# wasiahmad/context_attentive_ir

Measured on AMD Instinct MI355X. Metric: ranked (query,doc) pairs/sec, higher is better.
Workload: dtype f32; 1 GPU; cars, batch=16 sessions x session_len 7 x 10 candidates, q_len=4, doc_len=64, emb_dim=300, vocab=100000, f32, full-length Zipf ids; macro_batch=8, lanes=4, batches_in_flight=32, hipgraph=True, parallelism=single GPU, world_size=1

## Files before the change

### context_attentive_ir_amd/csrc/cars_session.hip

```cpp
#include "split2.hpp"
#include <algorithm>
#include <mutex>

namespace nir {

int launch_linear(const float* a, int64_t lda, const int64_t* ids, const float* table, int E, int64_t rows_per_seq,
                  int64_t seq_stride, const float* w, int64_t ldw, const float* bias, const float* bias2, float* c,
                  int64_t ldc, int64_t M, int N, int K, int act, hipStream_t st);
int launch_linear_ex(const float* a, int64_t lda, const int64_t* ids, const float* table, int E, int64_t rows_per_seq,
                     int64_t seq_stride, const float* w, int64_t ldw, const float* bias, const float* bias2, float* c,
                     int64_t ldc, int64_t M, int N, int K, int act, const float* add, int64_t ldadd, hipStream_t st);
constexpr int ACT_MAXOUT2 = 16;
constexpr int ACT_BOUNDED = 0x100;
constexpr int ACT_TANH_ROWDOT16 = 17;


__global__ __launch_bounds__(256) void click_pool2_kernel(const float* __restrict__ docs, const float* __restrict__ epart, int NP,
                                                          const float* __restrict__ b3, const float* __restrict__ labels,
                                                          const float* __restrict__ labels_all, int rows_all,
                                                          const int* __restrict__ mg, int rpg,
                                                          int rows, int N, int D, float* __restrict__ clicks) {
    __shared__ int part[4];
    const int lane = threadIdx.x & 63, wave = threadIdx.x >> 6;
    if (!mg) {
        int best = 0;
        for (int r0 = wave; r0 < rows_all; r0 += 4 * 16) {
            float lv[16];
#pragma unroll
            for (int j = 0; j < 16; ++j) {
                const int r = r0 + 4 * j;
                lv[j] = labels_all[(int64_t)(r < rows_all ? r : 0) * N + (lane < N ? lane : 0)];
            }
#pragma unroll
            for (int j = 0; j < 16; ++j) best = max(best, (int)__popcll(__ballot(lv[j] != 0.f && lane < N && r0 + 4 * j < rows_all)));
        }
        if (lane == 0) part[wave] = best;
    }
    __syncthreads();
    const int r = blockIdx.x * 4 + wave;
    if (r >= rows) return;
    const int m = mg ? mg[r / rpg] : max(max(part[0], part[1]), max(part[2], part[3]));
    const float lab = lane < N ? labels[(int64_t)r * N + lane] : -INFINITY;
    int rank = 0;
#pragma unroll 8
    for (int k = 0; k < N; ++k) {
        const float lk = __uint_as_float(__builtin_amdgcn_readlane(__float_as_uint(lab), k));
        rank += (lk > lab) || (lk == lab && k < lane);
    }
    const int count = (int)wave_sum((lane < N && lab != 0.f) ? 1.f : 0.f);
    const bool keep = lane < N && (rank < count || rank >= m);
    float lg = -INFINITY;
    if (keep) {
        const float* lp = epart + ((int64_t)r * N + lane) * NP;
        float s = b3[0];
        for (int j = 0; j < NP; j += 4) {
            const float4 v = *reinterpret_cast<const float4*>(lp + j);
            s += (v.x + v.y) + (v.z + v.w);
        }
        lg = s;
    }
    const float mx = wave_max(lg);
    const float ex = keep ? expf(lg - mx) : 0.f;
    const float p = ex / wave_sum(ex);
    const int nch = D >> 2;
    for (int c0 = 0; c0 < nch; c0 += 64) {
        const int c = c0 + lane < nch ? c0 + lane : 0;
        float4 acc = make_float4(0.f, 0.f, 0.f, 0.f);
#pragma unroll 8
        for (int k = 0; k < N; ++k) {
            const float pk = __uint_as_float(__builtin_amdgcn_readlane(__float_as_uint(p), k));
            const float4 v = *reinterpret_cast<const float4*>(docs + ((int64_t)r * N + k) * D + 4 * c);
            acc.x = fmaf(pk, v.x, acc.x); acc.y = fmaf(pk, v.y, acc.y); acc.z = fmaf(pk, v.z, acc.z); acc.w = fmaf(pk, v.w, acc.w);
        }
        if (c0 + lane < nch) *reinterpret_cast<float4*>(clicks + (int64_t)r * D + 4 * c) = acc;
    }
}

__global__ __launch_bounds__(256) void click_max_kernel(const float* __restrict__ labels, int rows, int N, int* __restrict__ out) {
    __shared__ int part[4];
    const int lane = threadIdx.x & 63, wave = threadIdx.x >> 6;
    const float* lg = labels + (int64_t)blockIdx.x * rows * N;
    int best = 0;
    if (N <= 64) {
        for (int r0 = 0; r0 < rows; r0 += 256) {
            const int r = r0 + (int)threadIdx.x;
            const float* row = lg + (int64_t)(r < rows ? r : rows - 1) * N;
            int c = 0;
#pragma unroll 8
            for (int k = 0; k < N; ++k) c += row[k] != 0.f ? 1 : 0;
            best = max(best, r < rows ? c : 0);
        }
        best = (int)wave_max((float)best);
    } else {
        for (int r = wave; r < rows; r += 4) {
            float c = 0.f;
            for (int k = lane; k < N; k += 64) c += lg[(int64_t)r * N + k] != 0.f ? 1.f : 0.f;
            best = max(best, (int)wave_sum(c));
        }
    }
    if (lane == 0) part[wave] = best;
    __syncthreads();
    if (threadIdx.x == 0) out[blockIdx.x] = max(max(part[0], part[1]), max(part[2], part[3]));
}

__global__ __launch_bounds__(256) void click_pool_big_kernel(const float* __restrict__ docs, const float* __restrict__ epart, int NP,
                                                             const float* __restrict__ b3, const float* __restrict__ labels,
                                                             const float* __restrict__ labels_all, int rows_all,
                                                             const int* __restrict__ mg, int rpg, int rows, int N, int D,
                                                             float* __restrict__ clicks) {
    extern __shared__ float csm[];
    __shared__ int part[4];
    const int lane = threadIdx.x & 63, wave = threadIdx.x >> 6;
    if (!mg) {
        int best = 0;
        for (int r = wave; r < rows_all; r += 4) {
            float c = 0.f;
            for (int k = lane; k < N; k += 64) c += labels_all[(int64_t)r * N + k] != 0.f ? 1.f : 0.f;
            best = max(best, (int)wave_sum(c));
        }
        if (lane == 0) part[wave] = best;
    }
    __syncthreads();
    const int r = blockIdx.x * 4 + wave;
    if (r >= rows) return;
    const int m = mg ? mg[r / rpg] : max(max(part[0], part[1]), max(part[2], part[3]));
    float* lab = csm + (size_t)wave * 2 * N;
    float* pw = lab + N;
    float cnt = 0.f;
    for (int k = lane; k < N; k += 64) {
        const float v = labels[(int64_t)r * N + k];
        lab[k] = v;
        cnt += v != 0.f ? 1.f : 0.f;
    }
    const int count = (int)wave_sum(cnt);
    __builtin_amdgcn_wave_barrier();
    float mx = -INFINITY;
    for (int c0 = 0; c0 < N; c0 += 64) {
        const int c = c0 + lane;
        const float lc = c < N ? lab[c] : -INFINITY;
        int rank = 0;
        for (int k = 0; k < N; ++k) {
            const float lk = lab[k];
            rank += (lk > lc) || (lk == lc && k < c);
        }
        const bool keep = c < N && (rank < count || rank >= m);
        float lg = -INFINITY;
        if (keep) {
            const float* lp = epart + ((int64_t)r * N + c) * NP;
            float sacc = b3[0];
            for (int j = 0; j < NP; j += 4) {
                const float4 v = *reinterpret_cast<const float4*>(lp + j);
                sacc += (v.x + v.y) + (v.z + v.w);
            }
            lg = sacc;
        }
        if (c < N) pw[c] = lg;
        mx = fmaxf(mx, lg);
    }
    mx = wave_max(mx);
    float den = 0.f;
    for (int c = lane; c < N; c += 64) {
        const float lg = pw[c];
        const float ex = lg == -INFINITY ? 0.f : expf(lg - mx);
        pw[c] = ex;
        den += ex;
    }
    den = wave_sum(den);
    __builtin_amdgcn_wave_barrier();
    const int nch = D >> 2;
    for (int c = lane; c < nch; c += 64) {
        float4 acc = make_float4(0.f, 0.f, 0.f, 0.f);
#pragma unroll 4
        for (int k = 0; k < N; ++k) {
            const float pk = pw[k] / den;
            const float4 v = *reinterpret_cast<const float4*>(docs + ((int64_t)r * N + k) * D + 4 * c);
            acc.x = fmaf(pk, v.x, acc.x); acc.y = fmaf(pk, v.y, acc.y); acc.z = fmaf(pk, v.z, acc.z); acc.w = fmaf(pk, v.w, acc.w);
        }
        *reinterpret_cast<float4*>(clicks + (int64_t)r * D + 4 * c) = acc;
    }
}


template <int NB, int UG = 1>
__global__ __launch_bounds__(256) void lstm_step_kernel(LstmStepArgs p) {
    __shared__ float red[4][UG * NB][256];
    const int tid = threadIdx.x, lane = tid & 63, wave = tid >> 6;
    const int i = lane & 15, g = lane >> 4;
    const int ch = blockIdx.y + p.chain0;
    const int u0 = blockIdx.x * 4 * UG;
    const int I = p.I, H = p.H;
    const float* wi[UG];
    const float* wh[UG];
#pragma unroll
    for (int ug = 0; ug < UG; ++ug) {
        const int ua = u0 + 4 * ug + (i >> 2);
        const int arow = (i & 3) * H + (ua < H ? ua : H - 1);
        wi[ug] = p.wih[ch] + (int64_t)arow * I;
        wh[ug] = p.whh[ch] + (int64_t)arow * H;
    }
    const float* hprev = p.hprev[ch];
    const float* cprev = p.cprev[ch];
    const float* gxp = p.gx[ch];
    const int nq1 = gxp ? 0 : ((I + 15) >> 4), nq2 = hprev ? ((H + 15) >> 4) : 0;
    float bias[UG][4];
#pragma unroll
    for (int ug = 0; ug < UG; ++ug) {
        const int ud = u0 + 4 * ug + g;
#pragma unroll
        for (int r = 0; r < 4; ++r) bias[ug][r] = (ud < H && !gxp) ? p.bih[ch][r * H + ud] + p.bhh[ch][r * H + ud] : 0.f;
    }
    for (int b0 = blockIdx.z * 16 * NB; b0 < p.B; b0 += gridDim.z * 16 * NB) {
        const float* xr[NB];
        const float* hr[NB];
        float bm[NB];
#pragma unroll
        for (int t = 0; t < NB; ++t) {
            const int b = b0 + 16 * t + i;
            const bool bv = b < p.B;
            bm[t] = bv ? 1.f : 0.f;
            const int bc = bv ? b : p.B - 1;
            const int64_t xr_i = p.xid[ch] ? p.xid[ch][bc] : (int64_t)bc;
            xr[t] = p.x[ch] + xr_i * p.xstride[ch];
            hr[t] = hprev ? hprev + (int64_t)bc * H : nullptr;
        }
        f32x4 acc[UG][NB];
#pragma unroll
        for (int ug = 0; ug < UG; ++ug)
#pragma unroll
            for (int t = 0; t < NB; ++t) acc[ug][t] = (f32x4){0.f, 0.f, 0.f, 0.f};
        constexpr int CH = NB == 1 ? 12 : (NB == 2 ? 8 : (UG == 1 ? 6 : 4));
        const int nqt = nq1 + nq2;
        for (int q0 = wave; q0 < nqt; q0 += 4 * CH) {
            float4 a4[CH][UG], b4[CH][NB];
#pragma unroll
            for (int c = 0; c < CH; ++c) {
                const int q = q0 + 4 * c;
                const bool second = q >= nq1;
                const int K = second ? H : I;
                const int k = 16 * (second ? q - nq1 : q) + 4 * g;
                const float km = (q < nqt && k < K) ? 1.f : 0.f;
                const int kc = (q < nqt && k < K) ? k : 0;
#pragma unroll
                for (int ug = 0; ug < UG; ++ug) {
                    a4[c][ug] = *reinterpret_cast<const float4*>((second ? wh[ug] : wi[ug]) + kc);
                    a4[c][ug].x *= km; a4[c][ug].y *= km; a4[c][ug].z *= km; a4[c][ug].w *= km;
                }
#pragma unroll
                for (int t = 0; t < NB; ++t) {
                    b4[c][t] = *reinterpret_cast<const float4*>(((second && hr[t]) ? hr[t] : xr[t]) + kc);
                    b4[c][t].x *= bm[t]; b4[c][t].y *= bm[t]; b4[c][t].z *= bm[t]; b4[c][t].w *= bm[t];
                }
            }
            __builtin_amdgcn_sched_barrier(0);
#pragma unroll
            for (int c = 0; c < CH; ++c)
#pragma unroll
                for (int ug = 0; ug < UG; ++ug)
#pragma unroll
                    for (int t = 0; t < NB; ++t) {
                        acc[ug][t] = __builtin_amdgcn_mfma_f32_16x16x4f32(a4[c][ug].x, b4[c][t].x, acc[ug][t], 0, 0, 0);
                        acc[ug][t] = __builtin_amdgcn_mfma_f32_16x16x4f32(a4[c][ug].y, b4[c][t].y, acc[ug][t], 0, 0, 0);
// ... 232 lines not shown
                                                              const float* __restrict__ Ds, const float* __restrict__ q,
                                                              int B, int S, int D, int HS, int q_on, int d_on,
                                                              float* __restrict__ xcat) {
    extern __shared__ float lgs[];
    float* lg[2] = {lgs, lgs + S};
    const int bt = blockIdx.x, b = bt / S, t = bt % S;
    const int lane = threadIdx.x & 63, wave = threadIdx.x >> 6;
    const int nch = q_on + d_on;
    const int HSQ = q_on ? HS : 0;
    const float* ur = U + (int64_t)bt * NU;
    const float* qv = q + (int64_t)bt * D;
    float* orow = xcat + (int64_t)bt * (D + nch * HS);
    for (int e = wave; e < nch * t; e += 4) {
        const int c = e / t, k = e % t + 1;
        const float* st = (c == 0 && q_on) ? Qs : Ds;
        const float* sv = st + ((int64_t)k * B + b) * HS;
        const float* uv = ur + c * HS;
        float sacc = 0.f;
        for (int f = 4 * lane; f < HS; f += 256) {
            const float4 a = *reinterpret_cast<const float4*>(sv + f), w = *reinterpret_cast<const float4*>(uv + f);
            sacc += (a.x * w.x + a.y * w.y) + (a.z * w.z + a.w * w.w);
        }
        sacc = wave_sum(sacc);
        if (lane == 0) lg[c][k] = sacc + ur[nch * HS + c];
    }
    if (threadIdx.x < nch) lg[threadIdx.x][0] = ur[nch * HS + threadIdx.x];
    for (int f = threadIdx.x; f < D; f += 256) orow[f] = qv[f];
    __syncthreads();
    for (int c = 0; c < nch; ++c) {
        const float* st = (c == 0 && q_on) ? Qs : Ds;
        float mx = -INFINITY;
        for (int k = 0; k <= t; ++k) mx = fmaxf(mx, lg[c][k]);
        float den = 0.f;
        for (int k = 0; k <= t; ++k) den += expf(lg[c][k] - mx);
        for (int f = threadIdx.x; f < HS; f += 256) {
            float acc = 0.f;
            for (int k = 1; k <= t; ++k) acc = fmaf(expf(lg[c][k] - mx) / den, st[((int64_t)k * B + b) * HS + f], acc);
            orow[D + c * HS + f] = acc;
        }
    }
    (void)HSQ;
}

__global__ void session_pack_kernel(const float* wq, const float* wshared, const float* wpriv, const float* sqw, const float* sqb,
                                    const float* sdw, const float* sdb, int D, int HS, int q_on, int d_on, float* wrank, float* ut) {
    const int nch = q_on + d_on, KS = nch * HS, KR = D + KS;
    const int64_t i = (int64_t)blockIdx.x * blockDim.x + threadIdx.x;
    if (i < (int64_t)D * KR) {
        const int o = (int)(i / KR), k = (int)(i % KR);
        float v;
        if (k < D) v = wq[(int64_t)o * D + k];
        else v = wshared[(int64_t)o * KS + (k - D)] + wpriv[(int64_t)o * KS + (k - D)];
        wrank[i] = v;
    }
    if (i < (int64_t)(KS + nch) * D) {
        const int j = (int)(i / D), f = (int)(i % D);
        float v;
        if (j < KS) {
            const int c = j / HS, jj = j % HS;
            const float* w = (c == 0 && q_on) ? sqw : sdw;
            v = w[(int64_t)f * HS + jj];
        } else {
            const int c = j - KS;
            v = ((c == 0 && q_on) ? sqb : sdb)[f];
        }
        ut[i] = v;
    }
}

__global__ void rank_feats_kernel(const float* qp, const float* docs, int N, int D, int64_t rows, float* feats) {
    const int64_t i = ((int64_t)blockIdx.x * blockDim.x + threadIdx.x) * 4;
    if (i < rows * D) {
        const int64_t r = i / D;
        const int f = (int)(i % D);
        const float4 q = *reinterpret_cast<const float4*>(qp + (r / N) * D + f), d = *reinterpret_cast<const float4*>(docs + r * D + f);
        float* o = feats + r * 4 * D + f;
        *reinterpret_cast<float4*>(o) = q;
        *reinterpret_cast<float4*>(o + D) = d;
        *reinterpret_cast<float4*>(o + 2 * D) = make_float4(fabsf(q.x - d.x), fabsf(q.y - d.y), fabsf(q.z - d.z), fabsf(q.w - d.w));
        *reinterpret_cast<float4*>(o + 3 * D) = make_float4(q.x * d.x, q.y * d.y, q.z * d.z, q.w * d.w);
    }
}

__global__ __launch_bounds__(256) void session_inner_pool_kernel(const float* __restrict__ states, const float* __restrict__ lpart,
                                                                 int NP, const float* __restrict__ b3, int B, int S, int HS,
                                                                 float* __restrict__ out ) {
    extern __shared__ float lg[];
    const int bt = blockIdx.x, b = bt / S, t = bt % S;
    const int n = t + 1;
    for (int k = threadIdx.x; k < n; k += 256) {
        const float* lp = lpart + ((int64_t)k * B + b) * NP;
        float s = b3[0];
        for (int j = 0; j < NP; ++j) s += lp[j];
        lg[k] = s;
    }
    __syncthreads();
    float mx = -INFINITY;
    for (int k = 0; k < n; ++k) mx = fmaxf(mx, lg[k]);
    float den = 0.f;
    for (int k = 0; k < n; ++k) den += expf(lg[k] - mx);
    for (int f = threadIdx.x; f < HS; f += 256) {
        float acc = 0.f;
        for (int k = 0; k < n; ++k) acc = fmaf(expf(lg[k] - mx) / den, states[((int64_t)k * B + b) * HS + f], acc);
        out[(int64_t)bt * HS + f] = acc;
    }
}

__global__ void session_cat_states_kernel(const float* a, const float* b2, int rows, int HSa, int HSb, float* out) {
    const int64_t i = (int64_t)blockIdx.x * blockDim.x + threadIdx.x;
    const int W = HSa + HSb;
    if (i < (int64_t)rows * W) {
        const int r = (int)(i / W), f = (int)(i % W);
        out[i] = f < HSa ? a[(int64_t)r * HSa + f] : b2[(int64_t)r * HSb + (f - HSa)];
    }
}

struct SessPlan {
    float *epart, *clicks, *Qs, *Ds, *Cq, *Cd, *U, *xcat, *qp, *feats, *y0, *y1, *lin, *cat, *gx, *Qs16, *Ds16;
    size_t bytes;
};
static SessPlan sess_plan(void* ws, size_t cap, int B, int S, int N, int D, int HS, int nch, bool rank_on, bool want_states) {
    Workspace a(ws, cap);
    SessPlan p;
    const size_t R = (size_t)B * S * N, BS = (size_t)B * S;
    p.epart = a.take<float>(R * (D / 16));
    p.clicks = a.take<float>(BS * D);
    p.Qs = a.take<float>((size_t)(S + 1) * B * HS);
    p.Ds = a.take<float>((size_t)(S + 1) * B * HS);
    p.Cq = a.take<float>((size_t)(S + 1) * B * HS);
    p.Cd = a.take<float>((size_t)(S + 1) * B * HS);
    p.U = a.take<float>(BS * (size_t)(nch * HS + nch + 4));
    p.xcat = a.take<float>(BS * (size_t)(D + nch * HS));
    p.qp = a.take<float>(BS * D);
    p.feats = a.take<float>(rank_on ? R * 4 * D : 0);
    p.y0 = a.take<float>(rank_on ? R * 256 : 0);
    p.y1 = a.take<float>(rank_on ? R * 128 : 0);
    p.lin = a.take<float>(want_states ? (size_t)(S + 1) * B * (HS / 16) : 0);
    p.cat = a.take<float>(want_states ? (size_t)S * B * nch * HS : 0);
    p.gx = a.take<float>((size_t)nch * BS * 4 * HS);
    p.Qs16 = a.take<float>((size_t)(S + 1) * B * HS);
    p.Ds16 = a.take<float>((size_t)(S + 1) * B * HS);
    p.bytes = align_up(a.off, 256);
    return p;
}

}

extern "C" size_t nir_lstm_step_whh_frag_bytes(int H) { return (H > 0 && H % 32 == 0) ? (size_t)4 * H * H * 2 * sizeof(_Float16) : 0; }

extern "C" int nir_lstm_step_pack_whh_frag(const float* w_hh, int H, void* frag, int* err_flag, nir_stream_t stream) {
    using namespace nir;
    NIR_REQUIRE(w_hh && frag && H > 0 && H % 32 == 0, "lstm_step_pack_whh_frag: H must be a positive multiple of 32");
    hipLaunchKernelGGL(lstm_step_whh_frag_kernel, dim3((unsigned)(H / 4), (unsigned)(H / 32)), dim3(64), 0, (hipStream_t)stream, w_hh, H, (_Float16*)frag, err_flag);
    NIR_CHECK_LAUNCH("lstm_step_whh_frag_kernel");
    return 0;
}

extern "C" size_t nir_cars_session_pack_floats(const nir_cars_session_weights* w, size_t* wrank_floats, size_t* ut_floats) {
    if (!w) return 0;
    const int nch = (w->q_on ? 1 : 0) + (w->d_on ? 1 : 0);
    const size_t a = (size_t)w->D * (w->D + nch * w->HS), b = (size_t)(nch * w->HS + nch) * w->D;
    if (wrank_floats) *wrank_floats = a;
    if (ut_floats) *ut_floats = b;
    return a + b;
}

extern "C" int nir_cars_session_pack(const nir_cars_session_weights* w, float* wrank, float* ut, nir_stream_t stream) {
    using namespace nir;
    NIR_REQUIRE(w && wrank && ut, "cars_session_pack: null pointer");
    const int q_on = w->q_on ? 1 : 0, d_on = w->d_on ? 1 : 0, nch = q_on + d_on;
    NIR_REQUIRE(w->qproj_w, "cars_session_pack: q_projection missing (ranker off?)");
    NIR_REQUIRE(nch == 0 || (w->shared_w && w->priv1_w), "cars_session_pack: session projectors missing");
    const int64_t n = std::max((int64_t)w->D * (w->D + nch * w->HS), (int64_t)(nch * w->HS + nch) * w->D);
    hipLaunchKernelGGL(session_pack_kernel, g1(n), dim3(256), 0, (hipStream_t)stream, w->qproj_w, w->shared_w, w->priv1_w, w->sq_attn_w,
                       w->sq_attn_b, w->sd_attn_w, w->sd_attn_b, w->D, w->HS, q_on, d_on, wrank, ut);
    NIR_CHECK_LAUNCH("session_pack_kernel");
    return 0;
}

extern "C" size_t nir_cars_session_workspace_bytes(int B, int S, int N, const nir_cars_session_weights* w) {
    if (!w || B < 0 || S <= 0 || N <= 0) return 0;
    const int nch = (w->q_on ? 1 : 0) + (w->d_on ? 1 : 0);
    return nir::sess_plan(nullptr, 0, B, S, N, w->D, w->HS, nch, true, true).bytes;
}

extern "C" int nir_cars_rank_session(const float* pooled_q, const float* pooled_docs, const float* labels, int B, int S, int N,
                                     const nir_cars_session_weights* w, void* workspace, size_t workspace_bytes,
                                     float* click_scores, float* clicks_out, const nir_cars_session_outputs* extra,
                                     nir_stream_t stream) {
    return nir_cars_rank_session_rows(pooled_q, pooled_docs, labels, B, S, N, w, workspace, workspace_bytes, click_scores, clicks_out, extra,
                                      nullptr, 0, nullptr, 0, nullptr, 0, stream);
}

extern "C" int nir_cars_rank_session_shard(const float* pooled_q, const float* pooled_docs, const float* labels, int B, int S, int N,
                                           const nir_cars_session_weights* w, void* workspace, size_t workspace_bytes,
                                           float* click_scores, float* clicks_out, const nir_cars_session_outputs* extra,
                                           const float* rank_docs, int NR, nir_stream_t stream) {
    return nir_cars_rank_session_rows(pooled_q, pooled_docs, labels, B, S, N, w, workspace, workspace_bytes, click_scores, clicks_out, extra,
                                      rank_docs, NR, nullptr, 0, nullptr, 0, stream);
}

extern "C" int nir_cars_click_max(const float* labels, int groups, int rows, int N, int* m_out, nir_stream_t stream) {
    using namespace nir;
    NIR_REQUIRE(labels && m_out && groups > 0 && rows > 0 && N > 0, "cars_click_max: bad args");
    hipLaunchKernelGGL(click_max_kernel, dim3((unsigned)groups), dim3(256), 0, (hipStream_t)stream, labels, rows, N, m_out);
    NIR_CHECK_LAUNCH("click_max_kernel");
    return 0;
}

extern "C" int nir_cars_rank_session_rows(const float* pooled_q, const float* pooled_docs, const float* labels, int B, int S, int N,
                                          const nir_cars_session_weights* w, void* workspace, size_t workspace_bytes,
                                          float* click_scores, float* clicks_out, const nir_cars_session_outputs* extra,
                                          const float* rank_docs, int NR, const float* labels_all, int64_t rows_all, const int* m_groups,
                                          int sessions_per_group, nir_stream_t stream) {
    return nir_cars_rank_session_pre(pooled_q, pooled_docs, labels, B, S, N, w, workspace, workspace_bytes, click_scores, clicks_out, extra, rank_docs, NR,
                                     labels_all, rows_all, m_groups, sessions_per_group, nullptr, nullptr, stream);
}

extern "C" int nir_cars_session_query_side(const float* pooled_q, int B, int S, const nir_cars_session_weights* w, float* U, float* gq,
                                           nir_stream_t stream) {
    using namespace nir;
    hipStream_t st = (hipStream_t)stream;
    NIR_REQUIRE(pooled_q && w && B >= 0 && S > 0, "cars_session_query_side: bad arguments");
    if (B == 0) return 0;
    const bool q_on = w->q_on != 0, d_on = w->d_on != 0, rank_on = w->rank_on != 0;
    const int nch = (q_on ? 1 : 0) + (d_on ? 1 : 0), D = w->D, HS = w->HS, NU = nch * HS + nch;
    const int64_t BS = (int64_t)B * S;
    const int bnd = (w->rank_bounded & 8) ? ACT_BOUNDED : 0;
    NIR_REQUIRE(!(nch && rank_on) || (U && w->attn_ut), "cars_session_query_side: U / packed attention weights missing");
    NIR_REQUIRE(!(nch && q_on) || gq, "cars_session_query_side: gq missing");
    if (nch && rank_on)
        NIR_PROPAGATE(launch_linear(pooled_q, D, nullptr, nullptr, 0, 0, 0, w->attn_ut, D, nullptr, nullptr, U, NU, BS, NU, D, NIR_ACT_NONE, st));
    if (nch && q_on)
        NIR_PROPAGATE(launch_linear_ex(pooled_q, D, nullptr, nullptr, 0, 0, 0, w->sq_wih, D, w->sq_bih, w->sq_bhh, gq, 4 * HS, BS, 4 * HS, D, NIR_ACT_NONE | bnd, nullptr, 0, st));
    return 0;
}

extern "C" int nir_cars_rank_session_pre(const float* pooled_q, const float* pooled_docs, const float* labels, int B, int S, int N,
                                         const nir_cars_session_weights* w, void* workspace, size_t workspace_bytes,
                                         float* click_scores, float* clicks_out, const nir_cars_session_outputs* extra,
                                         const float* rank_docs, int NR, const float* labels_all, int64_t rows_all, const int* m_groups,
                                         int sessions_per_group, const float* pre_U, const float* pre_gq, nir_stream_t stream) {
    using namespace nir;
    hipStream_t st = (hipStream_t)stream;
    NIR_REQUIRE(pooled_q && w, "cars_rank_session: null pointer");
    const bool q_on = w->q_on != 0, d_on = w->d_on != 0, rank_on = w->rank_on != 0;
    const int nch = (q_on ? 1 : 0) + (d_on ? 1 : 0);
    NIR_REQUIRE(!rank_on || (pooled_docs && click_scores && w->wrank), "cars_rank_session: ranker on needs documents, scores and packed weights");
    NIR_REQUIRE(!d_on || (pooled_docs && labels), "cars_rank_session: the document session needs documents and labels");
    NIR_REQUIRE(nch == 0 || !rank_on || w->attn_ut, "cars_rank_session: packed attention weights missing (nir_cars_session_pack)");
    NIR_REQUIRE(B >= 0 && S > 0 && N > 0, "cars_rank_session: bad dims");
    NIR_REQUIRE(N <= 2048, "cars_rank_session: %d candidates > 2048 unsupported", N);
    NIR_REQUIRE(!labels_all || (rows_all >= (int64_t)B * S && rows_all < (1 << 30)), "cars_rank_session: labels_all must hold at least the B*S rows of this call");
    NIR_REQUIRE(!rank_docs || (NR > 0 && NR <= N), "cars_rank_session: the ranked candidate slice must hold 1..N candidates (got %d)", NR);
    NIR_REQUIRE(S <= 4096, "cars_rank_session: session length %d > 4096 unsupported", S);
    NIR_REQUIRE(!m_groups || (sessions_per_group > 0 && !labels_all), "cars_rank_session: m_groups needs sessions_per_group > 0 and excludes labels_all");
    NIR_REQUIRE(!m_groups || B % sessions_per_group == 0, "cars_rank_session: B = %d is not a whole number of blocks of %d sessions", B, sessions_per_group);
    NIR_REQUIRE(!extra || nch > 0, "cars_rank_session: decoder states need at least one session encoder");
    NIR_REQUIRE(w->D % 64 == 0 && w->HS % 16 == 0 && w->D % 16 == 0, "cars_rank_session: D %% 64 / HS %% 16 required");
    if (B == 0) return 0;
    const int D = w->D, HS = w->HS, NP = D / 16;
    const bool want_states = extra != nullptr;
    SessPlan p = sess_plan(workspace, workspace_bytes, B, S, N, D, HS, nch, rank_on, want_states);
    if (!workspace || p.bytes > workspace_bytes) {
        set_error("cars_rank_session: workspace too small (%zu < %zu)", workspace_bytes, p.bytes);
        return NIR_ERR_WORKSPACE;
    }
    const int64_t BS = (int64_t)B * S, R = BS * N;
    float* clicks = clicks_out ? clicks_out : p.clicks;
    const int NU = nch * HS + nch;
    const float* gq = (pre_gq && q_on) ? pre_gq : p.gx;
    float* gd = p.gx + (q_on ? BS * 4 * (int64_t)HS : 0);
    const float* Uq = (pre_U && nch && rank_on) ? pre_U : p.U;
    const int bnd = (w->rank_bounded & 8) ? ACT_BOUNDED : 0;
    {
        hipStream_t sq_ = st;
        if (nch && rank_on && Uq == p.U)
            NIR_PROPAGATE(launch_linear(pooled_q, D, nullptr, nullptr, 0, 0, 0, w->attn_ut, D, nullptr, nullptr, p.U, NU, BS, NU, D, NIR_ACT_NONE, sq_));
        if (nch && q_on && gq == p.gx) NIR_PROPAGATE(launch_linear_ex(pooled_q, D, nullptr, nullptr, 0, 0, 0, w->sq_wih, D, w->sq_bih, w->sq_bhh, p.gx, 4 * HS, BS, 4 * HS, D, NIR_ACT_NONE | bnd, nullptr, 0, sq_));
    }
    if (d_on) {
        NIR_PROPAGATE(launch_linear_ex(pooled_docs, D, nullptr, nullptr, 0, 0, 0, w->click0_w, D, w->click0_b, nullptr, p.epart, NP, R, D, D,
                                       ACT_TANH_ROWDOT16 | ((w->rank_bounded & 4) ? ACT_BOUNDED : 0), w->click3_w, 0, st));
        {
            ProfScope ps("click_pool2_kernel", st);
            const float* lall = labels_all ? labels_all : labels;
            const int rall = labels_all ? (int)rows_all : (int)BS;
            if (N <= 64)
                hipLaunchKernelGGL(click_pool2_kernel, dim3((unsigned)((BS + 3) / 4)), dim3(256), 0, st, pooled_docs, p.epart, NP, w->click3_b, labels,
                                   lall, rall, m_groups, sessions_per_group * S, (int)BS, N, D, clicks);
            else {
                static std::once_flag once;
                std::call_once(once, [] { (void)hipFuncSetAttribute((const void*)click_pool_big_kernel, hipFuncAttributeMaxDynamicSharedMemorySize, 4 * 2 * 2048 * (int)sizeof(float)); });
                hipLaunchKernelGGL(click_pool_big_kernel, dim3((unsigned)((BS + 3) / 4)), dim3(256), (size_t)4 * 2 * N * sizeof(float), st, pooled_docs,
                                   p.epart, NP, w->click3_b, labels, lall, rall, m_groups, sessions_per_group * S, (int)BS, N, D, clicks);
            }
        }
        NIR_CHECK_LAUNCH("click_pool2_kernel");
    }
    const int nsteps = want_states ? S : S - 1;
    if (nch) {
        LstmStepArgs a;
        a.wih[0] = w->sq_wih; a.whh[0] = w->sq_whh; a.bih[0] = w->sq_bih; a.bhh[0] = w->sq_bhh;
        a.wih[1] = w->sd_wih; a.whh[1] = w->sd_whh; a.bih[1] = w->sd_bih; a.bhh[1] = w->sd_bhh;
        a.xid[0] = a.xid[1] = nullptr;
        a.xstride[0] = a.xstride[1] = (int64_t)S * D;
        a.chain0 = q_on ? 0 : 1;
        a.B = B; a.I = D; a.H = HS;
        {
            if (d_on) NIR_PROPAGATE(launch_linear_ex(clicks, D, nullptr, nullptr, 0, 0, 0, w->sd_wih, D, w->sd_bih, w->sd_bhh, gd, 4 * HS, BS, 4 * HS, D, NIR_ACT_NONE | bnd, nullptr, 0, st));
            a.gx[0] = gq; a.gx[1] = gd;
            a.gxstride = (int64_t)S * 4 * HS;
            a.whh_frag[0] = w->sq_whh_frag; a.whh_frag[1] = w->sd_whh_frag;
        }
        const float* gx0[2] = {a.gx[0], a.gx[1]};
        const int64_t slot = (int64_t)B * HS;
        for (int t = 0; t < nsteps; ++t) {
            a.gx[0] = gx0[0] + (int64_t)t * 4 * HS; a.gx[1] = gx0[1] + (int64_t)t * 4 * HS;
            a.x[0] = pooled_q + (int64_t)t * D; a.x[1] = clicks + (int64_t)t * D;
            a.hprev[0] = t ? p.Qs + t * slot : nullptr; a.cprev[0] = t ? p.Cq + t * slot : nullptr;
            a.hprev[1] = t ? p.Ds + t * slot : nullptr; a.cprev[1] = t ? p.Cd + t * slot : nullptr;
            a.hnext[0] = p.Qs + (t + 1) * slot; a.cnext[0] = p.Cq + (t + 1) * slot;
            a.hnext[1] = p.Ds + (t + 1) * slot; a.cnext[1] = p.Cd + (t + 1) * slot;
            a.h16prev[0] = t ? reinterpret_cast<const _Float16*>(p.Qs16 + t * slot) : nullptr;
            a.h16prev[1] = t ? reinterpret_cast<const _Float16*>(p.Ds16 + t * slot) : nullptr;
            a.h16next[0] = reinterpret_cast<_Float16*>(p.Qs16 + (t + 1) * slot);
            a.h16next[1] = reinterpret_cast<_Float16*>(p.Ds16 + (t + 1) * slot);
            NIR_PROPAGATE(launch_lstm_step(a, nch, st));
        }
    }
    if (rank_on) {
        const int KR = D + nch * HS;
        const float* xrows = pooled_q;
        if (nch) {
            {
                ProfScope ps("session_attend2_kernel", st);
                hipLaunchKernelGGL(session_attend2_kernel, dim3((unsigned)BS), dim3(256), 2 * S * sizeof(float), st, Uq, NU, p.Qs, p.Ds, pooled_q, B, S, D, HS,
                                   (int)q_on, (int)d_on, p.xcat);
            }
            NIR_CHECK_LAUNCH("session_attend2_kernel");
            xrows = p.xcat;
        }
        NIR_PROPAGATE(launch_linear(xrows, KR, nullptr, nullptr, 0, 0, 0, w->wrank, KR, w->qproj_b, nullptr, p.qp, D, BS, D, KR, NIR_ACT_NONE, st));
        const float* rdocs = rank_docs ? rank_docs : pooled_docs;
        const int Nr = rank_docs ? NR : N;
        const int64_t Rr = BS * Nr;
        {
            ProfScope ps("rank_feats_kernel", st);
            hipLaunchKernelGGL(rank_feats_kernel, g1(Rr * D / 4), dim3(256), 0, st, p.qp, rdocs, Nr, D, Rr, p.feats);
        }
        NIR_CHECK_LAUNCH("rank_feats_kernel");
        NIR_PROPAGATE(launch_linear_ex(p.feats, 4 * D, nullptr, nullptr, 0, 0, 0, w->mo0_w, 4 * D, w->mo0_b, nullptr, p.y0, 256, Rr, 512, 4 * D,
                                       ACT_MAXOUT2 | ((w->rank_bounded & 1) ? ACT_BOUNDED : 0), nullptr, 0, st));
        NIR_PROPAGATE(launch_linear_ex(p.y0, 256, nullptr, nullptr, 0, 0, 0, w->mo1_w, 256, w->mo1_b, nullptr, p.y1, 128, Rr, 256, 256,
                                       ACT_MAXOUT2 | ((w->rank_bounded & 2) ? ACT_BOUNDED : 0), nullptr, 0, st));
        NIR_PROPAGATE(launch_linear_ex(p.y1, 128, nullptr, nullptr, 0, 0, 0, w->mo2_w, 128, w->mo2_b, nullptr, click_scores, 1, Rr, 2, 128, ACT_MAXOUT2, nullptr, 0, st));
    }
    if (want_states) {
        const float* st_a = q_on ? p.Qs : p.Ds;
        const float* st_b = (q_on && d_on) ? p.Ds : nullptr;
        const float* c_a = q_on ? p.Cq : p.Cd;
        const float* c_b = (q_on && d_on) ? p.Cd : nullptr;
        const int HSb = st_b ? HS : 0, W = HS + HSb;
        const int rows = (S - 1) * B;
        if (extra->inner_q && q_on) {
            NIR_PROPAGATE(launch_linear_ex(p.Qs + (int64_t)B * HS, HS, nullptr, nullptr, 0, 0, 0, w->sq_inner0_w, HS, w->sq_inner0_b, nullptr, p.lin, HS / 16,
                                           (int64_t)S * B, HS, HS, ACT_TANH_ROWDOT16, w->sq_inner3_w, 0, st));
            hipLaunchKernelGGL(session_inner_pool_kernel, dim3((unsigned)BS), dim3(256), S * sizeof(float), st, p.Qs + (int64_t)B * HS, p.lin, HS / 16, w->sq_inner3_b, B, S, HS, extra->inner_q);
        }
        if (extra->inner_d && d_on) {
            NIR_PROPAGATE(launch_linear_ex(p.Ds + (int64_t)B * HS, HS, nullptr, nullptr, 0, 0, 0, w->sd_inner0_w, HS, w->sd_inner0_b, nullptr, p.lin, HS / 16,
                                           (int64_t)S * B, HS, HS, ACT_TANH_ROWDOT16, w->sd_inner3_w, 0, st));
            hipLaunchKernelGGL(session_inner_pool_kernel, dim3((unsigned)BS), dim3(256), S * sizeof(float), st, p.Ds + (int64_t)B * HS, p.lin, HS / 16, w->sd_inner3_b, B, S, HS, extra->inner_d);
        }
        NIR_CHECK_LAUNCH("session_inner_pool_kernel");
        if (rows > 0 && extra->dec_h && w->th_w) {
            hipLaunchKernelGGL(session_cat_states_kernel, g1((int64_t)rows * W), dim3(256), 0, st, st_a + (int64_t)B * HS,
                               st_b ? st_b + (int64_t)B * HS : nullptr, rows, HS, HSb, p.cat);
            NIR_PROPAGATE(launch_linear(p.cat, W, nullptr, nullptr, 0, 0, 0, w->th_w, W, w->th_b, nullptr, extra->dec_h, w->HDEC, rows, w->HDEC, W, NIR_ACT_NONE, st));
        }
        if (rows > 0 && extra->dec_c && w->tc_w) {
            hipLaunchKernelGGL(session_cat_states_kernel, g1((int64_t)rows * W), dim3(256), 0, st, c_a + (int64_t)B * HS,
                               c_b ? c_b + (int64_t)B * HS : nullptr, rows, HS, HSb, p.cat);
            NIR_PROPAGATE(launch_linear(p.cat, W, nullptr, nullptr, 0, 0, 0, w->tc_w, W, w->tc_b, nullptr, extra->dec_c, w->HDEC, rows, w->HDEC, W, NIR_ACT_NONE, st));
        }
        NIR_CHECK_LAUNCH("session_cat_states_kernel");
    }
    return 0;
}
```

### context_attentive_ir_amd/csrc/gemm.hip

```cpp
#include "split2.hpp"
#include <algorithm>
#include <mutex>
#include <stdlib.h>

namespace nir {


struct GemmArgs {
    const float* a;
    int64_t lda;
    const int64_t* ids;
    const float* table;
    int E;
    int64_t rows_per_seq, seq_stride;
    const float* w;
    int64_t ldw;
    const float* bias;
    const float* bias2;
    float* c;
    int64_t ldc;
    int64_t M;
    int N, K, act;
    const float* add;
    int64_t ldadd;
};

constexpr int ACT_MAXOUT2 = 16;
constexpr int ACT_TANH_ROWDOT16 = 17;
constexpr int ACT_BOUNDED = 0x100;

__device__ __forceinline__ void gemm_store(const GemmArgs& p, int64_t m, int n, float v, float bsum) {
    v += bsum;
    if (p.act == ACT_TANH_ROWDOT16) {
        v = n < p.N ? fast_tanh(v) * p.add[n] : 0.f;
        v += dpp_mov<0xB1>(v);
        v += dpp_mov<0x4E>(v);
        v += dpp_mov<0x141>(v);
        v += dpp_mov<0x140>(v);
        if (m < p.M && n < p.N && !(n & 15)) p.c[m * p.ldc + (n >> 4)] = v;
        return;
    }
    if (p.add && m < p.M && n < p.N) v += p.add[m * p.ldadd + n];
    if (p.act == NIR_ACT_TANH) v = fast_tanh(v);
    else if (p.act == NIR_ACT_RELU) v = fmaxf(v, 0.f);
    if (p.act == ACT_MAXOUT2) {
        const float other = dpp_mov<0xB1>(v);
        v = fmaxf(v, other);
        if (m < p.M && n < p.N && !(n & 1)) p.c[m * p.ldc + (n >> 1)] = v;
    } else if (m < p.M && n < p.N) {
        p.c[m * p.ldc + n] = v;
    }
}

#ifndef NIR_GEMM_BK
#define NIR_GEMM_BK 32
#endif
constexpr int BM = 64, BN = 64, BK = NIR_GEMM_BK, LDS_LD = BK + 4;
constexpr int TPR = BK / 4, RPP = 256 / TPR;
constexpr int LPT = BM * BK / 4 / 256;

template <bool VEC>
__global__ __launch_bounds__(256) void gemm_kernel(GemmArgs p) {
    extern __shared__ __attribute__((aligned(16))) float smem[];
    float* As = smem;
    float* Ws = smem + 2 * BM * LDS_LD;
    const int tid = threadIdx.x, lane = tid & 63, wave = tid >> 6;
    const int wm = wave >> 1, wn = wave & 1;
    const int nb = (p.N + BN - 1) / BN;
    const int64_t mb = (p.M + BM - 1) / BM;
    const int64_t bid = blockIdx.x;
    const int64_t tq = bid >> 3;
    const int64_t mblk = (tq / nb) * 8 + (bid & 7);
    if (mblk >= mb) return;
    const int64_t m0 = mblk * BM;
    const int n0 = (int)(tq % nb) * BN;
    const int lr = tid / TPR, lk = (tid % TPR) * 4;

    const float* arow[LPT];
    int64_t aidx[LPT];
    bool aval[LPT];
    const float* wrow[LPT];
    bool wval[LPT];
    const bool taps3 = p.ids && p.K > p.E && p.K <= 3 * p.E;
    const float* arow1[LPT];
    const float* arow2[LPT];
#pragma unroll
    for (int i = 0; i < LPT; ++i) {
        int64_t m = m0 + lr + RPP * i;
        aval[i] = m < p.M;
        arow[i] = arow1[i] = arow2[i] = nullptr;
        aidx[i] = 0;
        if (aval[i]) {
            if (p.ids) {
                aidx[i] = (m / p.rows_per_seq) * p.seq_stride + (m % p.rows_per_seq);
                if (p.K <= p.E) arow[i] = p.table + p.ids[aidx[i]] * (int64_t)p.E;
                if (taps3) {
                    arow[i] = p.table + p.ids[aidx[i]] * (int64_t)p.E;
                    arow1[i] = p.table + p.ids[aidx[i] + 1] * (int64_t)p.E - p.E;
                    arow2[i] = p.K > 2 * p.E ? p.table + p.ids[aidx[i] + 2] * (int64_t)p.E - 2 * p.E : arow1[i];
                }
            } else {
                arow[i] = p.a + m * p.lda;
            }
        }
        int n = n0 + lr + RPP * i;
        wval[i] = n < p.N;
        wrow[i] = p.w + (int64_t)(wval[i] ? n : 0) * p.ldw;
    }

    float4 ra[LPT], rw[LPT];
    auto load_tile = [&](int k0) {
        const int k = k0 + lk;
#pragma unroll
        for (int i = 0; i < LPT; ++i) {
            ra[i] = make_float4(0.f, 0.f, 0.f, 0.f);
            rw[i] = make_float4(0.f, 0.f, 0.f, 0.f);
            if (VEC) {
                if (k < p.K) {
                    if (aval[i]) {
                        const float* src;
                        if (taps3) {
                            src = (k < p.E ? arow[i] : (k < 2 * p.E ? arow1[i] : arow2[i])) + k;
                        } else if (p.ids && p.K > p.E) {
                            int seg = k / p.E;
                            src = p.table + p.ids[aidx[i] + seg] * (int64_t)p.E + (k - seg * p.E);
                        } else {
                            src = arow[i] + k;
                        }
                        ra[i] = *reinterpret_cast<const float4*>(src);
                    }
                    if (wval[i]) rw[i] = *reinterpret_cast<const float4*>(wrow[i] + k);
                }
            } else {
                float ta[4] = {0.f, 0.f, 0.f, 0.f}, tw[4] = {0.f, 0.f, 0.f, 0.f};
// ... 546 lines not shown
            G3_TERM(2, 0) G3_TERM(1, 1) G3_TERM(0, 2) G3_TERM(1, 0) G3_TERM(0, 1) G3_TERM(0, 0)
#undef G3_TERM
        }
      }
    };
#ifdef NIR_G3_NOLOAD
#define G3_LOAD(...)
#else
#define G3_LOAD(...) load_tile(__VA_ARGS__)
#endif
#ifdef NIR_G3_NOMMA
#define G3_MMA(b)
#else
#define G3_MMA(b) mma_tile(b)
#endif
#ifdef NIR_G3_NOSTORE
#define G3_STORE(...)
#else
#define G3_STORE(...) store_tile(__VA_ARGS__)
#endif
    int kt = 0;
    for (; kt + 4 < nk; kt += 2) {
        G3_LOAD(R0, (kt + 2) * KSTEP, false);
        __builtin_amdgcn_sched_barrier(0);
        G3_MMA(0);
        __builtin_amdgcn_sched_barrier(0);
        G3_STORE(R1, 1);
        lds_barrier();
        G3_LOAD(R1, (kt + 3) * KSTEP, false);
        __builtin_amdgcn_sched_barrier(0);
        G3_MMA(1);
        __builtin_amdgcn_sched_barrier(0);
        G3_STORE(R0, 0);
        lds_barrier();
    }
#undef G3_LOAD
#undef G3_MMA
#undef G3_STORE
    for (; kt < nk; ++kt) {
        const bool odd = (kt & 1) != 0;
        if (kt + 2 < nk) {
            if (odd) load_tile(R1, (kt + 2) * KSTEP, (kt + 2 == nk - 1) && ktail);
            else load_tile(R0, (kt + 2) * KSTEP, (kt + 2 == nk - 1) && ktail);
        }
        __builtin_amdgcn_sched_barrier(0);
        mma_tile(kt & 1);
        __builtin_amdgcn_sched_barrier(0);
        if (kt + 1 < nk) {
            if (odd) store_tile(R0, 0);
            else store_tile(R1, 1);
            lds_barrier();
        }
    }
#pragma unroll
    for (int b = 0; b < 2; ++b) {
        const int n = n0 + wn * 64 + b * 32 + (lane & 31);
        float bsum = 0.f;
        if (n < p.N) {
            if (p.bias) bsum += p.bias[n];
            if (p.bias2) bsum += p.bias2[n];
        }
#pragma unroll
        for (int a = 0; a < 2; ++a)
#pragma unroll
            for (int r = 0; r < 16; ++r) {
                const int64_t m = m0 + wm * 64 + a * 32 + (r & 3) + 8 * (r >> 2) + 4 * (lane >> 5);
                float v = acc[a][b][r];
                if (H2) v = split2_combine(v, acx[a][b][r]);
                gemm_store(p, m, n, v, bsum);
            }
    }
}

struct GemmPlaneArgs {
    const _Float16 *a1, *a2;
    int64_t lda;
    const int64_t* ids;
    int64_t rows_per_seq, seq_stride;
    int EP, taps;
    const _Float16 *w1, *w2;
    int64_t ldw;
    GemmArgs ep;
    int K;
};
constexpr int GP_BK = 32;
constexpr int GP_CHUNK = 128 * 8 + 32;
constexpr int GP_PLANE = 4 * GP_CHUNK;

template <int MODE>
__global__ __launch_bounds__(256, 2) void gemm_h2p_kernel(GemmPlaneArgs q) {
    extern __shared__ __attribute__((aligned(16))) unsigned short smemp[];
    unsigned short* As = smemp;
    unsigned short* Ws = smemp + 2 * 2 * GP_PLANE;
    const GemmArgs& p = q.ep;
    const int tid = threadIdx.x, lane = tid & 63, wave = tid >> 6;
    const int wm = wave >> 1, wn = wave & 1;
    const int nb = (p.N + G3_BN - 1) / G3_BN;
    const int64_t mb = (p.M + G3_BM - 1) / G3_BM;
    const int64_t bid = blockIdx.x;
    const int64_t tq = bid >> 3;
    const int64_t mblk = (tq / nb) * 8 + (bid & 7);
    if (mblk >= mb) return;
    const int64_t m0 = mblk * G3_BM;
    const int n0 = (int)(tq % nb) * G3_BN;
    const int lr = tid >> 1, hs = tid & 1;

    int64_t m = m0 + lr;
    m = m < p.M ? m : p.M - 1;
    int64_t arow[3] = {0, 0, 0};
    if (MODE == 0) {
        arow[0] = m * q.lda;
    } else {
        const int64_t ai = (m / q.rows_per_seq) * q.seq_stride + (m % q.rows_per_seq);
#pragma unroll
        for (int t = 0; t < 3; ++t) arow[t] = (t < q.taps ? q.ids[ai + t] : q.ids[ai]) * q.lda - (int64_t)t * q.EP;
    }
    int n = n0 + lr;
    n = n < p.N ? n : p.N - 1;
    const int64_t wrow = (int64_t)n * q.ldw;

    uint4 ra[2][2], rw[2][2];
    auto load_tile = [&](int k0, bool tail) {
        int k = k0 + 16 * hs;
        bool kv = true, kv2 = true;
        if (tail) {
            kv = k < q.K;
            k = kv ? k : 0;
            kv2 = kv && k + 8 < q.K;
        }
        int64_t ao = arow[0];
        if (MODE == 2) ao = k < q.EP ? arow[0] : (k < 2 * q.EP ? arow[1] : arow[2]);
        const int k2 = kv2 ? k + 8 : k;
        int64_t ao2 = ao;
        if (MODE == 2) ao2 = k2 < q.EP ? arow[0] : (k2 < 2 * q.EP ? arow[1] : arow[2]);
        ra[0][0] = *reinterpret_cast<const uint4*>(q.a1 + ao + k);
        ra[1][0] = *reinterpret_cast<const uint4*>(q.a2 + ao + k);
        ra[0][1] = *reinterpret_cast<const uint4*>(q.a1 + ao2 + k2);
        ra[1][1] = *reinterpret_cast<const uint4*>(q.a2 + ao2 + k2);
        rw[0][0] = *reinterpret_cast<const uint4*>(q.w1 + wrow + k);
        rw[1][0] = *reinterpret_cast<const uint4*>(q.w2 + wrow + k);
        rw[0][1] = *reinterpret_cast<const uint4*>(q.w1 + wrow + k2);
        rw[1][1] = *reinterpret_cast<const uint4*>(q.w2 + wrow + k2);
        if (tail) {
            const uint4 z = make_uint4(0u, 0u, 0u, 0u);
            if (!kv) { ra[0][0] = z; ra[1][0] = z; rw[0][0] = z; rw[1][0] = z; }
            if (!kv2) { ra[0][1] = z; ra[1][1] = z; rw[0][1] = z; rw[1][1] = z; }
        }
    };
    auto store_tile = [&](int buf) {
#pragma unroll
        for (int t = 0; t < 2; ++t)
#pragma unroll
            for (int c = 0; c < 2; ++c) {
                const int off = (buf * 2 + t) * GP_PLANE + (hs * 2 + c) * GP_CHUNK + lr * 8;
                *reinterpret_cast<uint4*>(As + off) = ra[t][c];
                *reinterpret_cast<uint4*>(Ws + off) = rw[t][c];
            }
    };
    f32x16 acc[2][2], acx[2][2];
#pragma unroll
    for (int a = 0; a < 2; ++a)
#pragma unroll
        for (int b = 0; b < 2; ++b)
#pragma unroll
            for (int r = 0; r < 16; ++r) { acc[a][b][r] = 0.0f; acx[a][b][r] = 0.0f; }

    const int nk = (q.K + GP_BK - 1) / GP_BK;
    const bool ktail = (q.K % GP_BK) != 0;
    if (nk == 1 && ktail) load_tile(0, true);
    else load_tile(0, false);
    store_tile(0);
    __syncthreads();
    const int foff_a = (lane >> 5) * GP_CHUNK + (wm * 64 + (lane & 31)) * 8;
    const int foff_w = (lane >> 5) * GP_CHUNK + (wn * 64 + (lane & 31)) * 8;
    auto mma_tile = [&](int buf) {
#pragma unroll
        for (int kb = 0; kb < 2; ++kb) {
            const unsigned short* ab = As + buf * 2 * GP_PLANE + kb * 2 * GP_CHUNK + foff_a;
            const unsigned short* wb = Ws + buf * 2 * GP_PLANE + kb * 2 * GP_CHUNK + foff_w;
            f16x8 af[2][2], wf[2][2];
#pragma unroll
            for (int t = 0; t < 2; ++t)
#pragma unroll
                for (int i = 0; i < 2; ++i) {
                    af[i][t] = *reinterpret_cast<const f16x8*>(ab + t * GP_PLANE + i * 32 * 8);
                    wf[i][t] = *reinterpret_cast<const f16x8*>(wb + t * GP_PLANE + i * 32 * 8);
                }
#define GP_T(ACC, TA, TW)                                                                                        \
            ACC[0][0] = __builtin_amdgcn_mfma_f32_32x32x16_f16(af[0][TA], wf[0][TW], ACC[0][0], 0, 0, 0);        \
            ACC[0][1] = __builtin_amdgcn_mfma_f32_32x32x16_f16(af[0][TA], wf[1][TW], ACC[0][1], 0, 0, 0);        \
            ACC[1][0] = __builtin_amdgcn_mfma_f32_32x32x16_f16(af[1][TA], wf[0][TW], ACC[1][0], 0, 0, 0);        \
            ACC[1][1] = __builtin_amdgcn_mfma_f32_32x32x16_f16(af[1][TA], wf[1][TW], ACC[1][1], 0, 0, 0);
            GP_T(acx, 1, 0) GP_T(acx, 0, 1) GP_T(acc, 0, 0)
#undef GP_T
        }
    };
    for (int kt = 0; kt + 2 < nk; ++kt) {
        load_tile((kt + 1) * GP_BK, false);
        __builtin_amdgcn_sched_barrier(0);
        mma_tile(kt & 1);
        __builtin_amdgcn_sched_barrier(0);
        store_tile((kt & 1) ^ 1);
        __syncthreads();
    }
    if (nk >= 2) {
        const int kt = nk - 2;
        if (ktail) load_tile((kt + 1) * GP_BK, true);
        else load_tile((kt + 1) * GP_BK, false);
        __builtin_amdgcn_sched_barrier(0);
        mma_tile(kt & 1);
        __builtin_amdgcn_sched_barrier(0);
        store_tile((kt & 1) ^ 1);
        __syncthreads();
    }
    mma_tile((nk - 1) & 1);
#pragma unroll
    for (int b = 0; b < 2; ++b) {
        const int nn = n0 + wn * 64 + b * 32 + (lane & 31);
        float bsum = 0.f;
        if (nn < p.N) {
            if (p.bias) bsum += p.bias[nn];
            if (p.bias2) bsum += p.bias2[nn];
        }
#pragma unroll
        for (int a = 0; a < 2; ++a)
#pragma unroll
            for (int r = 0; r < 16; ++r) {
                const int64_t mm = m0 + wm * 64 + a * 32 + (r & 3) + 8 * (r >> 2) + 4 * (lane >> 5);
                gemm_store(p, mm, nn, split2_combine(acc[a][b][r], acx[a][b][r]), bsum);
            }
    }
}

__global__ void split_f16x2_kernel(const float* __restrict__ x, int64_t rows, int cols, int64_t ld, int cols_pad, _Float16* __restrict__ p1,
                                   _Float16* __restrict__ p2) {
    const int64_t i = (int64_t)blockIdx.x * blockDim.x + threadIdx.x;
    if (i >= rows * cols_pad) return;
    const int64_t r = i / cols_pad;
    const int c = (int)(i % cols_pad);
    const float v = c < cols ? x[r * ld + c] : 0.f;
    const _Float16 a = split2_hi1_rtz(v);
    p1[i] = a;
    p2[i] = split2_lo1(v, a);
}

int launch_split_f16x2(const float* x, int64_t rows, int cols, int64_t ld, int cols_pad, void* p1, void* p2, hipStream_t st) {
    NIR_REQUIRE(x && p1 && p2 && rows >= 0 && cols > 0 && cols_pad >= cols && cols_pad % 8 == 0, "split_f16x2: bad args (cols_pad %% 8 == 0)");
    if (rows == 0) return 0;
    const int64_t n = rows * cols_pad;
    hipLaunchKernelGGL(split_f16x2_kernel, dim3((unsigned)((n + 255) / 256)), dim3(256), 0, st, x, rows, cols, ld, cols_pad, (_Float16*)p1, (_Float16*)p2);
    NIR_CHECK_LAUNCH("split_f16x2_kernel");
    return 0;
}

int launch_linear_planes(const void* a1, const void* a2, int64_t lda, const int64_t* ids, int64_t rows_per_seq, int64_t seq_stride, int EP,
                         int taps, const void* w1, const void* w2, int64_t ldw, const float* bias, float* c, int64_t ldc, int64_t M, int N, int K,
                         int act, const float* add, int64_t ldadd, hipStream_t st) {
    NIR_REQUIRE(a1 && a2 && w1 && w2 && c && M >= 0 && N > 0 && K > 0, "linear_planes: bad args");
    NIR_REQUIRE(K % 8 == 0 && lda % 8 == 0 && ldw % 8 == 0, "linear_planes: K and the row strides must be multiples of 8");
    NIR_REQUIRE(!ids || (taps >= 1 && taps <= 3 && EP % 8 == 0 && K == taps * EP), "linear_planes: gathered A needs K == taps*EP, EP %% 8 == 0");
    if (M == 0) return 0;
    GemmPlaneArgs q;
    q.a1 = (const _Float16*)a1; q.a2 = (const _Float16*)a2; q.lda = lda; q.ids = ids; q.rows_per_seq = rows_per_seq; q.seq_stride = seq_stride;
    q.EP = EP; q.taps = taps; q.w1 = (const _Float16*)w1; q.w2 = (const _Float16*)w2; q.ldw = ldw; q.K = K;
    q.ep = GemmArgs{nullptr, 0, nullptr, nullptr, 0, 0, 0, nullptr, 0, bias, nullptr, c, ldc, M, N, K, act, add, ldadd};
    const int64_t mb3 = (M + G3_BM - 1) / G3_BM;
    const int nb3 = (N + G3_BN - 1) / G3_BN;
    constexpr size_t lds = (size_t)2 * 2 * 2 * GP_PLANE * 2;
    static std::once_flag once;
    std::call_once(once, [] {
        (void)hipFuncSetAttribute((const void*)gemm_h2p_kernel<0>, hipFuncAttributeMaxDynamicSharedMemorySize, (int)lds);
        (void)hipFuncSetAttribute((const void*)gemm_h2p_kernel<2>, hipFuncAttributeMaxDynamicSharedMemorySize, (int)lds);
    });
    ProfScope ps(prof_shape_name(ids ? "gemm_h2p_kernel[gather]" : "gemm_h2p_kernel", M, N, K), st);
    dim3 grid((unsigned)(8 * nb3 * ((mb3 + 7) / 8)));
    if (ids) hipLaunchKernelGGL(gemm_h2p_kernel<2>, grid, dim3(256), lds, st, q);
    else hipLaunchKernelGGL(gemm_h2p_kernel<0>, grid, dim3(256), lds, st, q);
    NIR_CHECK_LAUNCH("gemm_h2p_kernel");
    return 0;
}

template <int NT>
static void launch_skinny(const GemmArgs& p, int G, size_t lds, hipStream_t st) {
    static std::once_flag once;
    std::call_once(once, [] { (void)hipFuncSetAttribute((const void*)gemm_skinny_kernel<NT>, hipFuncAttributeMaxDynamicSharedMemorySize, 128 * 1024); });
    const int64_t ntiles = (p.M + 15) / 16;
    const unsigned grid = (unsigned)std::min<int64_t>((ntiles + SK_WAVES - 1) / SK_WAVES, 512);
    hipLaunchKernelGGL(gemm_skinny_kernel<NT>, dim3(grid), dim3(64 * SK_WAVES), lds, st, p, G);
}

__global__ __launch_bounds__(256) void rowdot_kernel(const float* x, int64_t ldx, const float* w, const float* b,
                                                     float* out, int64_t M, int K, int act) {
    const int lane = threadIdx.x & 63;
    const int64_t m = (int64_t)blockIdx.x * 4 + (threadIdx.x >> 6);
    if (m >= M) return;
    const float* xr = x + m * ldx;
    float s = 0.f;
    for (int k = lane; k < K; k += 64) s += xr[k] * w[k];
    s = wave_sum(s);
    if (lane == 0) {
        float v = s + (b ? b[0] : 0.f);
        if (act == NIR_ACT_TANH) v = fast_tanh(v);
        else if (act == NIR_ACT_RELU) v = fmaxf(v, 0.f);
        out[m] = v;
    }
}

int launch_linear_ex(const float* a, int64_t lda, const int64_t* ids, const float* table, int E, int64_t rows_per_seq,
                     int64_t seq_stride, const float* w, int64_t ldw, const float* bias, const float* bias2, float* c,
                     int64_t ldc, int64_t M, int N, int K, int act, const float* add, int64_t ldadd, hipStream_t st) {
    const bool bounded = (act & ACT_BOUNDED) != 0;
    act &= ~ACT_BOUNDED;
    NIR_REQUIRE(M >= 0 && N > 0 && K > 0, "linear: bad dims M=%lld N=%d K=%d", (long long)M, N, K);
    NIR_REQUIRE(w && c, "linear: null weight/output");
    NIR_REQUIRE(ids ? (table != nullptr && E > 0 && rows_per_seq > 0) : (a != nullptr), "linear: null A operand");
    if (M == 0) return 0;
    NIR_REQUIRE(act != ACT_MAXOUT2 || (N % 2 == 0), "linear: maxout epilogue needs an even N");
    NIR_REQUIRE(act != ACT_TANH_ROWDOT16 || (N % 16 == 0 && add != nullptr), "linear: tanh-rowdot epilogue needs N %% 16 == 0 and the weight row");
    GemmArgs p{a, lda, ids, table, E, rows_per_seq, seq_stride, w, ldw, bias, bias2, c, ldc, M, N, K, act, add, ldadd};
    bool vec = (K % 4 == 0) && (ldw % 4 == 0) && (((uintptr_t)w & 15) == 0);
    if (ids) vec = vec && (E % 4 == 0) && (((uintptr_t)table & 15) == 0);
    else vec = vec && (lda % 4 == 0) && (((uintptr_t)a & 15) == 0);
    const int64_t mb = (M + BM - 1) / BM;
    const int nb = (N + BN - 1) / BN;
    const int skG = (K + 15) / 16, skNT = (N + 15) / 16;
    const size_t sk_lds = (size_t)16 * skNT * (skG * 16 + 4) * 4;
    const bool exact_f32 = tun(g_tun.exact_f32) != 0;
    const int64_t mb3 = (M + G3_BM - 1) / G3_BM;
    const int nb3 = (N + G3_BN - 1) / G3_BN;
    const int mode3 = !ids ? 0 : (K <= E ? 1 : (K <= 3 * E ? 2 : -1));
    if (vec && !exact_f32 && mode3 >= 0 && N >= 96 && K >= 32 && mb3 * nb3 >= 96) {
        ProfScope ps(prof_shape_name(bounded ? (ids ? "gemm3h_kernel[gather]" : "gemm3h_kernel") : (ids ? "gemm3_kernel[gather]" : "gemm3_kernel"), M, N, K), st);
        dim3 grid((unsigned)(8 * nb3 * ((mb3 + 7) / 8)));
        if (bounded && K >= 64) {
            constexpr size_t lds2 = (size_t)2 * 2 * 2 * 2 * G3_PLANE * 2;
            static std::once_flag once;
            std::call_once(once, [] {
                (void)hipFuncSetAttribute((const void*)gemm3_kernel<0, true, 2>, hipFuncAttributeMaxDynamicSharedMemorySize, (int)lds2);
                (void)hipFuncSetAttribute((const void*)gemm3_kernel<1, true, 2>, hipFuncAttributeMaxDynamicSharedMemorySize, (int)lds2);
            });
            if (mode3 == 0) { hipLaunchKernelGGL((gemm3_kernel<0, true, 2>), grid, dim3(256), lds2, st, p); NIR_CHECK_LAUNCH("gemm3h ks2"); return 0; }
            if (mode3 == 1) { hipLaunchKernelGGL((gemm3_kernel<1, true, 2>), grid, dim3(256), lds2, st, p); NIR_CHECK_LAUNCH("gemm3h ks2"); return 0; }
        }
        if (bounded) {
            constexpr size_t lds = (size_t)2 * 2 * 2 * G3_PLANE * 2;
            if (mode3 == 0) hipLaunchKernelGGL((gemm3_kernel<0, true>), grid, dim3(256), lds, st, p);
            else if (mode3 == 1) hipLaunchKernelGGL((gemm3_kernel<1, true>), grid, dim3(256), lds, st, p);
            else hipLaunchKernelGGL((gemm3_kernel<2, true>), grid, dim3(256), lds, st, p);
        } else {
            constexpr size_t lds = (size_t)2 * 2 * 3 * G3_PLANE * 2;
            if (mode3 == 0) hipLaunchKernelGGL((gemm3_kernel<0, false>), grid, dim3(256), lds, st, p);
            else if (mode3 == 1) hipLaunchKernelGGL((gemm3_kernel<1, false>), grid, dim3(256), lds, st, p);
            else hipLaunchKernelGGL((gemm3_kernel<2, false>), grid, dim3(256), lds, st, p);
        }
        NIR_CHECK_LAUNCH("nir_linear_f32[bf16x3]");
        return 0;
    }
    if (N <= 64 && vec && M >= 4096 && (!ids || K <= E) && sk_lds <= 128 * 1024 && act != ACT_MAXOUT2 && act != ACT_TANH_ROWDOT16) {
        ProfScope ps(prof_shape_name(ids ? "gemm_skinny_kernel[gather]" : "gemm_skinny_kernel", M, N, K), st);
        if (skNT == 1) launch_skinny<1>(p, skG, sk_lds, st);
// ... 18 lines not shown
        }
        const dim3 grid((unsigned)((M + 16 * best - 1) / (16 * best)), (unsigned)ncol);
        switch (best) {
            case 2: hipLaunchKernelGGL(gemm32_kernel<2>, grid, dim3(256), 0, st, p); break;
            case 3: hipLaunchKernelGGL(gemm32_kernel<3>, grid, dim3(256), 0, st, p); break;
            case 4: hipLaunchKernelGGL(gemm32_kernel<4>, grid, dim3(256), 0, st, p); break;
            case 5: hipLaunchKernelGGL(gemm32_kernel<5>, grid, dim3(256), 0, st, p); break;
            default: hipLaunchKernelGGL(gemm32_kernel<6>, grid, dim3(256), 0, st, p); break;
        }
    } else if (mb * nb < 160) {
        ProfScope ps(prof_shape_name(ids ? "gemm16_kernel[gather]" : "gemm16_kernel", M, N, K), st);
        dim3 grid((unsigned)((M + 15) / 16), (unsigned)((N + 15) / 16));
        if (vec) hipLaunchKernelGGL(gemm16_kernel<true>, grid, dim3(256), 0, st, p);
        else hipLaunchKernelGGL(gemm16_kernel<false>, grid, dim3(256), 0, st, p);
    } else {
        ProfScope ps(prof_shape_name(ids ? "gemm_kernel[gather]" : "gemm_kernel", M, N, K), st);
        constexpr size_t lds = (size_t)2 * (BM + BN) * LDS_LD * 4;
        static std::once_flag once;
        std::call_once(once, [] {
            (void)hipFuncSetAttribute((const void*)gemm_kernel<true>, hipFuncAttributeMaxDynamicSharedMemorySize, (int)lds);
            (void)hipFuncSetAttribute((const void*)gemm_kernel<false>, hipFuncAttributeMaxDynamicSharedMemorySize, (int)lds);
        });
        dim3 grid((unsigned)(8 * nb * ((mb + 7) / 8)));
        if (vec) hipLaunchKernelGGL(gemm_kernel<true>, grid, dim3(256), lds, st, p);
        else hipLaunchKernelGGL(gemm_kernel<false>, grid, dim3(256), lds, st, p);
    }
    NIR_CHECK_LAUNCH("nir_linear_f32");
    return 0;
}

int launch_linear(const float* a, int64_t lda, const int64_t* ids, const float* table, int E, int64_t rows_per_seq,
                  int64_t seq_stride, const float* w, int64_t ldw, const float* bias, const float* bias2, float* c,
                  int64_t ldc, int64_t M, int N, int K, int act, hipStream_t st) {
    return launch_linear_ex(a, lda, ids, table, E, rows_per_seq, seq_stride, w, ldw, bias, bias2, c, ldc, M, N, K, act,
                            nullptr, 0, st);
}

int launch_rowdot(const float* x, int64_t ldx, const float* w, const float* b, float* out, int64_t M, int K, int act,
                  hipStream_t st) {
    NIR_REQUIRE(x && w && out && K > 0, "rowdot: bad args");
    if (M == 0) return 0;
    {
        ProfScope ps("rowdot_kernel", st);
        hipLaunchKernelGGL(rowdot_kernel, dim3((unsigned)((M + 3) / 4)), dim3(256), 0, st, x, ldx, w, b, out, M, K, act);
    }
    NIR_CHECK_LAUNCH("nir_rowdot_f32");
    return 0;
}

}

extern "C" int nir_linear_f32(const float* a, int64_t lda, const int64_t* ids, const float* table, int E,
                              int64_t rows_per_seq, int64_t seq_stride, const float* w, int64_t ldw,
                              const float* bias, const float* bias2, float* c, int64_t ldc, int64_t M, int N, int K,
                              int act, nir_stream_t stream) {
    return nir::launch_linear(a, lda, ids, table, E, rows_per_seq, seq_stride, w, ldw, bias, bias2, c, ldc, M, N, K,
                              act, (hipStream_t)stream);
}

extern "C" int nir_linear_ex_f32(const float* a, int64_t lda, const int64_t* ids, const float* table, int E,
                                 int64_t rows_per_seq, int64_t seq_stride, const float* w, int64_t ldw,
                                 const float* bias, const float* bias2, float* c, int64_t ldc, int64_t M, int N, int K,
                                 int act, const float* add, int64_t ldadd, nir_stream_t stream) {
    return nir::launch_linear_ex(a, lda, ids, table, E, rows_per_seq, seq_stride, w, ldw, bias, bias2, c, ldc, M, N, K,
                                 act, add, ldadd, (hipStream_t)stream);
}

extern "C" int nir_rowdot_f32(const float* x, int64_t ldx, const float* w, const float* b, float* out, int64_t M,
                              int K, int act, nir_stream_t stream) {
    return nir::launch_rowdot(x, ldx, w, b, out, M, K, act, (hipStream_t)stream);
}

namespace nir { int launch_split_f16x2(const float* x, int64_t rows, int cols, int64_t ld, int cols_pad, void* p1, void* p2, hipStream_t st); }
extern "C" int nir_split_f16x2(const float* x, int64_t rows, int cols, int64_t ld, int cols_pad, void* p1, void* p2, nir_stream_t stream) {
    return nir::launch_split_f16x2(x, rows, cols, ld, cols_pad, p1, p2, (hipStream_t)stream);
}

extern "C" int nir_linear_planes_f32(const void* a1, const void* a2, int64_t lda, const int64_t* ids, int64_t rows_per_seq, int64_t seq_stride,
                                     int EP, int taps, const void* w1, const void* w2, int64_t ldw, const float* bias, float* c, int64_t ldc,
                                     int64_t M, int N, int K, int act, nir_stream_t stream) {
    return nir::launch_linear_planes(a1, a2, lda, ids, rows_per_seq, seq_stride, EP, taps, w1, w2, ldw, bias, c, ldc, M, N, K, act, nullptr, 0,
                                     (hipStream_t)stream);
}
```

### context_attentive_ir_amd/lib.py

```python
import ctypes as C
import os

import torch

_HERE = os.path.dirname(os.path.abspath(__file__))
LIB_PATH = os.path.join(_HERE, "libneuroir_hip.so")

c_fp = C.c_void_p
c_ip = C.c_void_p
c_st = C.c_void_p


def _struct(name, float_fields, int_fields=()):
    fields = [(f, c_fp) for f in float_fields] + [(f, C.c_int) for f in int_fields]
    return type(name, (C.Structure,), {"_fields_": fields})


DrmmWeights = _struct("nir_drmm_weights",
                      ["gate_w", "gate_b", "ffnn0_w", "ffnn0_b", "ffnn1_w", "ffnn1_b", "out_w", "out_b"], ["snap_one"])
DrmmWeights = type("nir_drmm_weights", (C.Structure,), {"_fields_": list(DrmmWeights._fields_) + [("self_bin", C.c_void_p)]})
MatchTensorWeights = _struct(
    "nir_matchtensor_weights",
    ["proj_w", "proj_b", "q_wih", "q_whh", "q_bih", "q_bhh", "d_wih", "d_whh", "d_bih", "d_bhh",
     "qproj_w", "qproj_b", "dproj_w", "dproj_b", "alpha", "conv1_w", "conv1_b", "conv2_w", "conv2_b",
     "conv3_w", "conv3_b", "conv_w", "conv_b", "out_w", "out_b"],
    ["F", "Hq", "Hd", "C", "NF", "MF", "bounded"])
MatchTensorWeights = type("nir_matchtensor_weights", (C.Structure,), {"_fields_": list(MatchTensorWeights._fields_) + [("dproj_frag", C.c_void_p)]})
DuetWeights = _struct(
    "nir_duet_weights",
    ["l_conv_w", "l_conv_b", "l_fc1_w", "l_fc1_b", "l_fc2_w", "l_fc2_b", "l_fc3_w", "l_fc3_b",
     "convq_w", "convq_b", "convd1_w", "convd1_b", "convd2_w", "convd2_b", "fc1_w", "fc1_b", "fc2_w", "fc2_b",
     "fc3_w", "fc3_b", "fc4_w", "fc4_b"],
    ["NF", "pool", "bounded"])
DuetWeights = type("nir_duet_weights", (C.Structure,), {"_fields_": list(DuetWeights._fields_) + [
    (f, C.c_void_p) for f in ("table_h1", "table_h2", "convd1_h1", "convd1_h2", "convd2_h1", "convd2_h2")] + [("EP", C.c_int)] + [
    ("fw1", C.c_void_p), ("fw2", C.c_void_p), ("K1P", C.c_int), ("ftable", C.c_void_p), ("fw1c", C.c_void_p), ("EPT", C.c_int)]})
DssmWeights = _struct("nir_dssm_weights", ["q_w1t", "q_b1", "q_w2t", "q_b2", "d_w1t", "d_b1", "d_w2t", "d_b2"], ["NH", "NO"])
CdssmWeights = _struct("nir_cdssm_weights", ["q_w5t", "q_b", "q_semt", "q_semb", "d_w5t", "d_b", "d_semt", "d_semb"], ["NH", "NO"])
CONV1D_SPLIT, CONV1D_FP32, ARCI_MAX_LAYERS = 0, 1, 8


class Conv1dLayer(C.Structure):
    _fields_ = [("planes", C.c_void_p), ("wt", c_fp), ("bias", c_fp)] + [(f, C.c_int) for f in ("C_in", "F", "k", "p", "path")]


class ArciWeights(C.Structure):
    _fields_ = [("q", Conv1dLayer * ARCI_MAX_LAYERS), ("d", Conv1dLayer * ARCI_MAX_LAYERS), ("head_wq", c_fp), ("head_wd", c_fp), ("head_b", c_fp),
                ("n_layers", C.c_int), ("q_feats", C.c_int), ("d_feats", C.c_int)]


ARCII_MAX_LAYERS = 8


class Conv2dLayer(C.Structure):
    _fields_ = [("planes", C.c_void_p), ("wt", c_fp), ("bias", c_fp)] + [(f, C.c_int) for f in ("C_in", "F", "kh", "kw", "ph", "pw", "path")]


class ArciiWeights(C.Structure):
    _fields_ = [("q", Conv1dLayer), ("d", Conv1dLayer), ("l", Conv2dLayer * ARCII_MAX_LAYERS), ("head_w", c_fp), ("head_b", c_fp),
                ("n_layers", C.c_int), ("feats", C.c_int)]


CarsEncoderWeights = _struct(
    "nir_cars_encoder_weights",
    ["wih", "whh", "bih", "bhh", "attn0_w", "attn0_b", "attn3_w", "attn3_b"], ["H", "bounded"])
CarsEncoderWeights = type("nir_cars_encoder_weights", (C.Structure,), {"_fields_": list(CarsEncoderWeights._fields_) + [("attn_frag", C.c_void_p),
                                                                                                   ("whh_frag", C.c_void_p)]})
CarsSessionWeights = _struct(
    "nir_cars_session_weights",
    ["click0_w", "click0_b", "click3_w", "click3_b", "sq_attn_w", "sq_attn_b", "sd_attn_w", "sd_attn_b",
     "sq_wih", "sq_whh", "sq_bih", "sq_bhh", "sd_wih", "sd_whh", "sd_bih", "sd_bhh", "qproj_w", "qproj_b",
     "shared_w", "priv1_w", "mo0_w", "mo0_b", "mo1_w", "mo1_b", "mo2_w", "mo2_b", "wrank", "attn_ut",
     "sq_inner0_w", "sq_inner0_b", "sq_inner3_w", "sq_inner3_b", "sd_inner0_w", "sd_inner0_b", "sd_inner3_w", "sd_inner3_b",
     "th_w", "th_b", "tc_w", "tc_b"],
    ["D", "HS", "HDEC", "q_on", "d_on", "rank_on", "rank_bounded"])
CarsSessionWeights = type("nir_cars_session_weights", (C.Structure,), {"_fields_": list(CarsSessionWeights._fields_) + [("sq_whh_frag", C.c_void_p),
                                                                                                   ("sd_whh_frag", C.c_void_p)]})
class CarsDecoderWeights(C.Structure):
    _fields_ = [(f, c_fp) for f in ("rnn_wih", "rnn_whh", "rnn_bih", "rnn_bhh", "attn_in_w", "attn_out_w", "dec_attn_w", "pred1_w",
                                    "pred2_w", "sess_w")] + [(f, C.c_int) for f in ("HD", "DQ", "P", "KS")] + [("VT", C.c_int64), ("pred2_frag", C.c_void_p), ("rnn_gate_fold", C.c_void_p),
                                                                                                           ("rnn_whh_frag", C.c_void_p), ("attn_q_w", C.c_void_p)]


S2S_ATTN = {"general": 0, "dot": 1, "mlp": 2}


class Seq2seqDecoderWeights(C.Structure):
    _fields_ = [(f, c_fp) for f in ("rnn_wih", "rnn_whh", "rnn_bih", "rnn_bhh", "attn_in_wt", "attn_ctx_w", "attn_query_w", "attn_query_b", "attn_v",
                                    "attn_out_w", "attn_out_b", "gen_w", "gen_b")] + [("H", C.c_int), ("attn_type", C.c_int), ("VT", C.c_int64),
                                                                                     ("rnn_gate_fold", C.c_void_p), ("rnn_whh_frag", C.c_void_p),
                                                                                     ("gen_frag", C.c_void_p)]


class AcgCopyWeights(C.Structure):
    _fields_ = [("copy_w", c_fp), ("copy_b", c_fp), ("reuse_copy_attn", C.c_int)] + [(f, c_fp) for f in ("attn_in_wt", "attn_ctx_w", "attn_query_w",
                                                                                                    "attn_query_b", "attn_v")]


class HredqsDecoderWeights(C.Structure):
    _fields_ = [(f, c_fp) for f in ("rnn_wih", "rnn_whh", "rnn_bih", "rnn_bhh", "gen_w", "gen_b")] + [("H", C.c_int), ("VT", C.c_int64),
                                                                                                     ("rnn_gate_fold", C.c_void_p),
                                                                                                     ("rnn_whh_frag", C.c_void_p),
                                                                                                     ("gen_frag", C.c_void_p)]


CarsSessionOutputs = _struct("nir_cars_session_outputs", ["inner_q", "inner_d", "dec_h", "dec_c"])

MnsrfWeights = _struct(
    "nir_mnsrf_weights",
    ["q_wih", "q_whh", "q_bih", "q_bhh", "d_wih", "d_whh", "d_bih", "d_bhh", "s_wih", "s_whh", "s_bih", "s_bhh",
     "proj_w", "proj_b"], ["Hq", "Hd", "HS"])
MnsrfWeights = type("nir_mnsrf_weights", (C.Structure,), {"_fields_": list(MnsrfWeights._fields_) + [
    ("q_fold", C.c_void_p), ("d_fold", C.c_void_p), ("q_whh_frag", C.c_void_p), ("d_whh_frag", C.c_void_p), ("s_whh_frag", C.c_void_p), ("err", C.c_void_p)]})

_i, _l, _z = C.c_int, C.c_int64, C.c_size_t
SIGNATURES = {
    "nir_version": (_i, []),
    "nir_last_error_string": (C.c_char_p, []),
    "nir_debug_clock_probe": (_i, [C.c_void_p, _i, _i, C.c_void_p, c_st]),
    "nir_debug_set_buffer": (_i, [C.c_void_p]),
    "nir_set_stream_batches_in_flight": (_i, [c_st, _i]),
    "nir_debug_set_tunable": (_i, [C.c_char_p, _i]),
    "nir_profile_enable": (_i, [_i]),
    "nir_profile_report": (_i, [C.c_char_p, _z]),
    "nir_split_f16x2": (_i, [c_fp, _l, _i, _l, _i, C.c_void_p, C.c_void_p, c_st]),
    "nir_linear_planes_f32": (_i, [C.c_void_p, C.c_void_p, _l, c_ip, _l, _l, _i, _i, C.c_void_p, C.c_void_p, _l, c_fp, c_fp, _l, _l, _i, _i, _i, c_st]),
    "nir_sanitize_ids": (_i, [c_ip, _l, c_ip, _l, _l, c_ip, c_ip, C.c_void_p, c_st]),
    "nir_flag_publish": (_i, [C.c_void_p, C.c_void_p, c_st]),
    "nir_gather_fields": (_i, [C.c_void_p, _i, C.c_void_p, _l, c_st]),
    "nir_host_device_pointer": (_i, [C.c_void_p, C.POINTER(C.c_void_p)]),
    "nir_softmax_rows_publish": (_i, [c_fp, c_fp, _l, _i, C.c_void_p, C.c_void_p, c_st]),
    "nir_host_rank_metric": (C.c_double, [_i, C.c_void_p, C.c_void_p, _i, _l, _i, _i]),
    "nir_widen_ids_i32": (_i, [C.c_void_p, C.c_void_p, _l, c_st]),
    "nir_linear_f32": (_i, [c_fp, _l, c_ip, c_fp, _i, _l, _l, c_fp, _l, c_fp, c_fp, c_fp, _l, _l, _i, _i, _i, c_st]),
    "nir_linear_ex_f32": (_i, [c_fp, _l, c_ip, c_fp, _i, _l, _l, c_fp, _l, c_fp, c_fp, c_fp, _l, _l, _i, _i, _i, c_fp, _l, c_st]),
    "nir_rowdot_f32": (_i, [c_fp, _l, c_fp, c_fp, c_fp, _l, _i, _i, c_st]),
    "nir_attn_pool_workspace_bytes": (_z, [_l, _i, _i]),
    "nir_attn_pool_f32": (_i, [C.c_void_p, _i, C.POINTER(CarsEncoderWeights), c_ip, _l, _i, _i, _i, C.c_void_p, _z, c_fp, c_st]),
    "nir_bilstm_fwd": (_i, [c_fp, c_ip, c_fp, c_fp, c_fp, c_fp, c_fp, c_fp, _l, _i, _i, _i, c_st]),
    "nir_bilstm_supported": (_i, [_i]),
    "nir_bilstm_fused_fwd": (_i, [c_fp, _i, c_fp, c_fp, c_fp, c_ip, c_fp, c_fp, c_fp, c_fp, c_fp, c_fp, _l, _i, _i, _i, c_st]),
    "nir_bilstm_steps_workspace_bytes": (_z, [_l, _i]),
    "nir_bilstm_steps_fwd": (_i, [c_fp, c_ip, c_fp, c_fp, c_fp, c_fp, c_fp, c_fp, _l, _i, _i, _i, C.c_void_p, _z, c_st]),
    "nir_birnn_steps_fwd": (_i, [_i, c_fp, c_ip, c_fp, c_fp, c_fp, c_fp, c_fp, c_fp, c_fp, c_fp, _l, _i, _i, _i, C.c_void_p, _z, c_st]),
    "nir_maxpool_time_f32": (_i, [c_fp, _l, _i, _i, c_fp, c_st]),
    "nir_lstm256_whh_frag_bytes": (_z, [_i]),
    "nir_lstm256_pack_whh_frag": (_i, [c_fp, _i, C.c_void_p, C.c_void_p, c_st]),
    "nir_lstm256_workspace_bytes": (_z, [_l, _i]),
    "nir_lstm256_rows_fwd": (_i, [c_fp, c_ip, c_ip, C.c_void_p, c_fp, _i, C.c_void_p, _l, _l, _i, _i, C.c_void_p, _z, c_st]),
    "nir_lstm256_train_fwd": (_i, [c_fp, c_ip, C.c_void_p, c_fp, c_fp, c_fp, C.c_void_p, _l, _i, _i, C.c_void_p, C.c_size_t, c_st]),
    "nir_lstm256_bptt_workspace_bytes": (_z, [_l, _i]),
    "nir_lstm256_bptt": (_i, [c_fp, c_fp, c_fp, c_ip, c_fp, c_fp, _l, _i, _i, C.c_void_p, C.c_size_t, c_st]),
    "nir_decode_greedy_plain_workspace_bytes": (_z, [_l, _i, _l]),
    "nir_decode_greedy_plain": (_i, [c_fp, c_fp, _l, _i, c_fp, _l, _i, c_fp, c_fp, c_fp, c_fp, c_fp, c_fp, _l, c_ip, _l, _i, C.c_void_p, _z, c_ip,
                                     c_st]),
    "nir_decode_greedy_plain_folded": (_i, [c_fp, c_fp, _l, _i, c_fp, _l, _i, c_fp, c_fp, c_fp, c_fp, c_fp, c_fp, _l, c_ip, _l, _i, c_fp, C.c_void_p,
                                            C.c_void_p, _z, c_ip, c_st]),
    "nir_mnsrf_workspace_bytes": (_z, [_l, _i, _i, _i, _i, C.POINTER(MnsrfWeights)]),
    "nir_mnsrf_encode": (_i, [c_ip, c_ip, _l, _i, _i, c_fp, _l, _i, C.POINTER(MnsrfWeights), C.c_void_p, _z, c_fp, c_fp, c_st]),
    "nir_mnsrf_encode_states": (_i, [c_ip, c_ip, _l, _i, _i, c_fp, _l, _i, C.POINTER(MnsrfWeights), C.c_void_p, _z, c_fp, c_fp, c_fp, c_fp, c_st]),
    "nir_mnsrf_rank": (_i, [c_fp, c_fp, c_ip, c_ip, _l, _i, _i, _i, c_fp, _l, _i, C.POINTER(MnsrfWeights), C.c_void_p, _z, c_fp, c_st]),
    "nir_mnsrf_score": (_i, [c_ip, c_ip, c_ip, c_ip, _l, _i, _i, _i, _i, c_fp, _l, _i, C.POINTER(MnsrfWeights), C.c_void_p, _z,
                            c_fp, c_st]),
    "nir_softmax_rows": (_i, [c_fp, c_fp, _l, _i, c_st]),
    "nir_softmax_gathered": (_i, [c_fp, c_fp, c_fp, _i, _l, _i, _i, c_st]),
    "nir_rank_loss_bce": (_i, [c_fp, c_fp, _l, _i, c_fp, c_st]),
    "nir_rank_loss_softmax_nll": (_i, [c_fp, c_fp, _l, _i, c_fp, c_st]),
    "nir_esm_score": (_i, [c_ip, c_ip, _i, _i, _i, _i, c_fp, _l, _i, c_fp, c_st]),
    "nir_drmm_score": (_i, [c_ip, c_ip, _i, _i, _i, _i, c_fp, _l, _i, C.POINTER(DrmmWeights), c_fp, c_fp, c_st]),
    "nir_matchtensor_workspace_bytes": (_z, [_i, _i, _i, _i, C.POINTER(MatchTensorWeights)]),
    "nir_matchtensor_score": (_i, [c_ip, c_ip, c_ip, c_ip, _i, _i, _i, _i, c_fp, _l, _i,
                                   C.POINTER(MatchTensorWeights), C.c_void_p, _z, c_fp, c_fp, c_fp, c_fp, c_fp, c_st]),
    "nir_matchtensor_score_encoded": (_i, [c_ip, c_ip, c_fp, c_fp, _i, _i, _i, _i, C.POINTER(MatchTensorWeights), C.c_void_p, _z, c_fp, c_fp, c_fp,
                                           c_st]),
    "nir_matchtensor_score_folded": (_i, [c_ip, c_ip, c_ip, c_ip, _i, _i, _i, _i, C.c_void_p, C.c_void_p, _i, _l,
                                          C.POINTER(MatchTensorWeights), C.c_void_p, _z, c_fp, c_fp, c_fp, c_fp, c_fp, C.c_void_p, c_st]),
    "nir_duet_workspace_bytes": (_z, [_i, _i, _i, _i, _i, C.POINTER(DuetWeights)]),
    "nir_duet_score": (_i, [c_ip, c_ip, _i, _i, _i, _i, c_fp, _l, _i, C.POINTER(DuetWeights), C.c_void_p, _z,
                            c_fp, c_fp, c_fp, c_st]),
    "nir_dssm_workspace_bytes": (_z, [_i, _i, _i]),
    "nir_dssm_score": (_i, [c_ip, c_ip, _i, _i, _i, _i, c_fp, _l, _i, _l, C.POINTER(DssmWeights), C.c_void_p, _z, c_fp, c_fp, c_fp, c_st]),
    "nir_cdssm_workspace_bytes": (_z, [_i, _i, _i, _i, _i]),
    "nir_cdssm_score": (_i, [c_ip, c_ip, _i, _i, _i, _i, c_fp, _l, _i, _l, C.POINTER(CdssmWeights), C.c_void_p, _z, c_fp, c_fp, c_fp, c_st]),
    "nir_conv1d_planes_bytes": (_z, [_i, _i, _i]),
    "nir_conv1d_pack": (_i, [c_fp, _i, _i, _i, C.c_void_p, c_fp, C.c_void_p, c_st]),
    "nir_conv1d_pool_out_floats": (_z, [_l, _i, _i, _i, _i]),
    "nir_conv1d_pool_f32": (_i, [c_ip, c_fp, _l, _i, C.POINTER(Conv1dLayer), _i, c_fp, c_fp, c_st]),
    "nir_arci_workspace_bytes": (_z, [_i, _i, _i, _i, C.POINTER(ArciWeights)]),
    "nir_arci_score": (_i, [c_ip, c_ip, _i, _i, _i, _i, c_fp, _l, _i, C.POINTER(ArciWeights), C.c_void_p, _z, c_fp, c_st]),
    "nir_conv2d_planes_bytes": (_z, [_i, _i, _i, _i]),
    "nir_conv2d_pack": (_i, [c_fp, _i, _i, _i, _i, C.c_void_p, c_fp, C.c_void_p, c_st]),
    "nir_conv2d_pool_out_floats": (_z, [_l, _i, _i, _i, _i, _i, _i]),
    "nir_conv2d_pool_f32": (_i, [c_fp, c_fp, c_fp, _l, _i, _i, _i, C.POINTER(Conv2dLayer), _i, c_fp, c_fp, c_st]),
    "nir_arcii_workspace_bytes": (_z, [_i, _i, _i, _i, C.POINTER(ArciiWeights)]),
    "nir_arcii_score": (_i, [c_ip, c_ip, _i, _i, _i, _i, c_fp, _l, _i, C.POINTER(ArciiWeights), C.c_void_p, _z, c_fp, c_st]),
    "nir_maxpool_arg_f32": (_i, [c_fp, _l, _i, _i, c_fp, C.c_void_p, c_st]),
    "nir_maxpool_arg_bwd_f32": (_i, [c_fp, C.c_void_p, _l, _i, _i, c_fp, c_st]),
    "nir_cosine_bcast_f32": (_i, [c_fp, c_fp, _l, _i, _i, c_fp, c_st]),
    "nir_cosine_bcast_bwd_f32": (_i, [c_fp, c_fp, c_fp, _l, _i, _i, c_fp, c_fp, c_st]),
    "nir_rank_loss_softmax_nll_bwd": (_i, [c_fp, c_fp, c_fp, _l, _i, c_fp, c_st]),
    "nir_cars_encode_workspace_bytes": (_z, [_l, _i, _i, C.POINTER(CarsEncoderWeights)]),
    "nir_cars_encode": (_i, [c_ip, c_ip, _l, _i, c_fp, _l, _i, C.POINTER(CarsEncoderWeights), C.c_void_p, _z,
                             c_fp, c_fp, c_st]),
    "nir_lstm_whh_frag_bytes": (_z, [_i, _i]),
    "nir_lstm_pack_whh_frag": (_i, [c_fp, _i, _i, C.c_void_p, C.c_void_p, c_st]),
    "nir_lstm_fold_table_bytes": (_z, [_l, _i, _i, _i]),
    "nir_lstm_fold_table_workspace_bytes": (_z, [_l, _i, _i, _i, _i]),
    "nir_lstm_fold_table": (_i, [c_fp, _l, _i, c_fp, c_fp, c_fp, _i, _i, C.c_void_p, _i, C.c_void_p, _z, c_st]),
    "nir_bilstm_folded_fwd": (_i, [C.c_void_p, _i, c_ip, c_ip, c_fp, c_fp, C.c_void_p, _l, _l, _i, _i, _i, c_st]),
    "nir_cars_encode_folded_workspace_bytes": (_z, [_l, _i, C.POINTER(CarsEncoderWeights)]),
    "nir_cars_encode_folded": (_i, [c_ip, c_ip, _l, _i, C.c_void_p, _i, _l, C.POINTER(CarsEncoderWeights), C.c_void_p, _z,
                                    c_fp, c_fp, C.c_void_p, c_st]),
    "nir_cars_session_workspace_bytes": (_z, [_i, _i, _i, C.POINTER(CarsSessionWeights)]),
    "nir_linear_wgrad_f32": (_i, [c_fp, _l, c_fp, _l, c_ip, c_fp, _i, c_fp, _l, _l, _i, _i, c_st]),
    "nir_colsum_f32": (_i, [c_fp, _l, _l, _i, c_fp, c_st]),
    "nir_linear_wgrad_set_f32": (_i, [c_fp, _l, c_fp, _l, c_ip, c_fp, _i, c_fp, _l, _l, _i, _i, c_st]),
    "nir_linear_wgrad_bias_f32": (_i, [c_fp, _l, c_fp, _l, c_ip, c_fp, _i, c_fp, _l, c_fp, _l, _i, _i, c_st]),
    "nir_linear_wgrad_group_f32": (_i, [_i] + [C.c_void_p] * 10 + [c_st]),
    "nir_linear_wgrad_bias_set_f32": (_i, [c_fp, _l, c_fp, _l, c_ip, c_fp, _i, c_fp, _l, c_fp, _l, _i, _i, c_st]),
    "nir_colsum_set_f32": (_i, [c_fp, _l, _l, _i, c_fp, c_st]),
    "nir_seq_rows": (_i, [c_ip, _l, _i, _i, C.c_void_p, C.c_void_p, c_st]),
    "nir_linear_wgrad_rows_set_f32": (_i, [c_fp, _l, _l, c_fp, _l, _l, C.c_void_p, C.c_void_p, _l, _i, _i, c_fp, _l, c_fp, _i, _i, c_st]),
    "nir_transpose_f32": (_i, [c_fp, _i, _i, c_fp, c_st]),
    "nir_transpose_group_f32": (_i, [_i, C.c_void_p, C.c_void_p, C.c_void_p, C.c_void_p, c_st]),
    "nir_lstm_train_fwd": (_i, [c_fp, c_ip, c_fp, c_fp, c_fp, c_fp, c_fp, c_fp, c_fp, c_fp, _l, _i, _i, _i, c_st]),
    "nir_lstm_perm_weights": (_i, [c_fp, c_fp, c_fp, c_fp, c_fp, c_fp, _i, _i, _i, c_fp, c_fp, c_st]),
    "nir_lstm_train_fwd_split": (_i, [c_fp, c_ip, c_ip, c_fp, c_fp, c_fp, c_fp, C.c_void_p, _l, _i, _i, _i, c_st]),
    "nir_lstm_train_bwd": (_i, [c_fp, c_fp, c_fp, c_fp, c_fp, c_fp, c_fp, c_ip, c_fp, c_fp, c_fp, c_fp, _l, _i, _i, _i, c_st]),
    "nir_lstm_cell_fwd": (_i, [c_fp, c_fp, c_fp, c_fp, c_fp, _l, _i, c_st]),
    "nir_lstm_cell_bwd": (_i, [c_fp, c_fp, c_fp, c_fp, c_fp, c_fp, c_fp, _l, _i, c_st]),
    "nir_lstm_cell_seq_fwd": (_i, [c_fp, _l, c_fp, c_fp, c_fp, _l, c_fp, _l, c_fp, _l, c_fp, _l, _l, _i, c_st]),
    "nir_lstm_cell_seq_bwd": (_i, [c_fp, _l, c_fp, c_fp, _l, c_fp, c_fp, _l, c_fp, _l, c_fp, _l, c_fp, _l, c_fp, _l, _i, c_st]),
    "nir_gru_train_mfma_supported": (_i, [_i]),
    "nir_gru_train_fwd": (_i, [c_fp, c_ip, c_fp, c_fp, c_fp, c_fp, c_fp, _l, _i, _i, _i, c_st]),
    "nir_gru_train_bwd": (_i, [c_fp, c_fp, c_fp, c_fp, c_ip, c_fp, c_fp, c_fp, _l, _i, _i, _i, _i, c_st]),
    "nir_gru_cell_seq_fwd": (_i, [c_fp, _l, c_fp, c_fp, c_fp, _l, c_fp, _l, c_fp, _l, _l, _i, c_st]),
    "nir_gru_cell_seq_bwd": (_i, [c_fp, _l, c_fp, c_fp, c_fp, _l, c_fp, _l, c_fp, _l, c_fp, _l, c_fp, _l, _i, c_st]),
    "nir_dropout_f32": (_i, [c_fp, c_fp, C.c_void_p, _l, C.c_float, C.c_uint64, c_st]),
    "nir_dropout_dev_f32": (_i, [c_fp, c_fp, C.c_void_p, _l, C.c_float, C.c_void_p, C.c_uint64, c_st]),
    "nir_mask_scale_f32": (_i, [c_fp, C.c_void_p, C.c_float, c_fp, _l, c_st]),
    "nir_act_bwd_f32": (_i, [c_fp, c_fp, c_fp, _l, _i, c_st]),
    "nir_im2col_rows_f32": (_i, [c_fp, _l, _i, _i, _i, _i, _i, _i, _i, c_fp, c_st]),
    "nir_mt_conv3_supported": (_i, [_i, _i, _i, _i]),
    "nir_mt_conv3_fwd": (_i, [c_fp, c_fp, c_fp, c_fp, c_fp, c_fp, c_fp, _l, _i, _i, _i, _i, c_fp, c_st]),
    "nir_mt_conv3_wt_floats": (C.c_size_t, [_i, _i]),
    "nir_mt_conv3_partial_floats": (C.c_size_t, [_l, _i, _i]),
    "nir_mt_conv3_bwd": (_i, [c_fp, c_fp, c_fp, c_fp, c_fp, _l, _i, _i, _i, _i, c_fp, c_fp, c_fp, c_st]),
    "nir_col2im_rows_f32": (_i, [c_fp, _l, _i, _i, _i, _i, _i, _i, _i, c_fp, c_st]),
    "nir_rank_loss_bce_bwd": (_i, [c_fp, c_fp, c_fp, c_fp, _l, c_st]),
    "nir_softmax_nll_ent_fwd": (_i, [c_fp, _l, c_ip, _l, _l, _i, c_fp, c_fp, c_fp, C.c_void_p, c_st]),
    "nir_softmax_nll_ent_bwd": (_i, [c_fp, _l, c_ip, _l, c_fp, c_fp, c_fp, c_fp, _l, _i, c_fp, c_st]),
    "nir_softmax_pool_fwd": (_i, [c_fp, C.c_void_p, _l, _l, c_fp, _l, _i, _i, _i, c_fp, c_fp, c_st]),
    "nir_softmax_pool_bwd": (_i, [c_fp, c_fp, c_fp, _l, _i, _i, _i, c_fp, c_fp, c_st]),
    "nir_embed_f32": (_i, [c_ip, c_fp, _l, _i, _l, c_fp, C.c_void_p, c_st]),
    "nir_embed_bwd_f32": (_i, [c_ip, c_fp, _l, _i, _l, c_fp, _l, c_st]),
    "nir_add_f32": (_i, [c_fp, c_fp, c_fp, _l, c_st]),
    "nir_cars_decode_workspace_bytes": (_z, [_l, _l, _i, C.POINTER(CarsDecoderWeights)]),
    "nir_cars_decode_greedy": (_i, [c_fp, c_fp, c_fp, c_ip, _l, _i, c_ip, _l, c_fp, c_fp, _l, _i, c_ip, _l, _i,
                                    C.POINTER(CarsDecoderWeights), C.c_void_p, _z, c_ip, c_st]),
    "nir_cars_session_pack_floats": (_z, [C.POINTER(CarsSessionWeights), C.POINTER(_z), C.POINTER(_z)]),
    "nir_cars_session_pack": (_i, [C.POINTER(CarsSessionWeights), c_fp, c_fp, c_st]),
    "nir_cars_rank_session": (_i, [c_fp, c_fp, c_fp, _i, _i, _i, C.POINTER(CarsSessionWeights), C.c_void_p, _z,
                                   c_fp, c_fp, C.POINTER(CarsSessionOutputs), c_st]),
    "nir_cars_rank_session_shard": (_i, [c_fp, c_fp, c_fp, _i, _i, _i, C.POINTER(CarsSessionWeights), C.c_void_p, _z,
                                         c_fp, c_fp, C.POINTER(CarsSessionOutputs), c_fp, _i, c_st]),
    "nir_cars_rank_session_rows": (_i, [c_fp, c_fp, c_fp, _i, _i, _i, C.POINTER(CarsSessionWeights), C.c_void_p, _z,
                                        c_fp, c_fp, C.POINTER(CarsSessionOutputs), c_fp, _i, c_fp, _l, C.c_void_p, _i, c_st]),
    "nir_cars_session_query_side": (_i, [c_fp, _i, _i, C.POINTER(CarsSessionWeights), c_fp, c_fp, c_st]),
    "nir_cars_rank_session_pre": (_i, [c_fp, c_fp, c_fp, _i, _i, _i, C.POINTER(CarsSessionWeights), C.c_void_p, _z,
                                       c_fp, c_fp, C.POINTER(CarsSessionOutputs), c_fp, _i, c_fp, _l, C.c_void_p, _i, c_fp, c_fp, c_st]),
    "nir_cars_click_max": (_i, [c_fp, _i, _i, _i, C.c_void_p, c_st]),
    "nir_lstm_step_whh_frag_bytes": (_z, [_i]),
    "nir_lstm_step_pack_whh_frag": (_i, [c_fp, _i, C.c_void_p, C.c_void_p, c_st]),
    "nir_seq2seq_gen_frag_bytes": (_z, [_l, _i]),
    "nir_seq2seq_pack_gen_frag": (_i, [c_fp, _l, _i, C.c_void_p, C.c_void_p, c_st]),
    "nir_seq2seq_gen_argmax_workspace_bytes": (_z, [_l, _i, _l, _i]),
    "nir_seq2seq_gen_argmax": (_i, [c_fp, _l, _i, c_fp, c_fp, C.c_void_p, _l, c_ip, _l, C.c_void_p, _z, c_ip, _l, c_ip, c_st]),
    "nir_seq2seq_attend": (_i, [c_fp, c_fp, c_fp, c_fp, c_fp, c_ip, _l, _i, _i, _i, c_fp, c_fp, _l, c_st]),
    "nir_seq2seq_decode_workspace_bytes": (_z, [_l, _i, C.POINTER(Seq2seqDecoderWeights)]),
    "nir_seq2seq_decode_greedy": (_i, [c_fp, c_fp, c_fp, c_ip, _l, _i, c_fp, _l, _i, c_ip, _l, _i, C.POINTER(Seq2seqDecoderWeights), C.c_void_p, _z,
                                       c_ip, c_fp, c_st]),
    "nir_hredqs_gen_argmax_workspace_bytes": (_z, [_l]),
    "nir_hredqs_gen_argmax": (_i, [C.c_void_p, _l, _i, c_fp, C.c_void_p, _l, c_ip, _l, C.c_void_p, _z, c_ip, _l, c_ip, c_st]),
    "nir_hredqs_decode_workspace_bytes": (_z, [_l, _l, _i, C.POINTER(HredqsDecoderWeights)]),
    "nir_hredqs_decode_greedy": (_i, [c_fp, c_fp, _l, _l, c_fp, _l, _i, c_ip, _l, _i, C.POINTER(HredqsDecoderWeights), C.c_void_p, _z, c_ip, c_st]),
    "nir_acg_gen_select_workspace_bytes": (_z, [_l, _i, _l, _i]),
    "nir_acg_gen_select": (_i, [c_fp, _l, _i, c_fp, c_fp, C.c_void_p, _l, c_fp, c_fp, c_fp, _l, c_ip, _i, c_ip, c_ip, c_ip, _i, c_ip, _l, C.c_void_p, _z,
                                c_ip, _l, c_ip, c_fp, c_fp, c_ip, c_st]),
    "nir_acg_decode_workspace_bytes": (_z, [_l, _i, _i, C.POINTER(Seq2seqDecoderWeights), C.POINTER(AcgCopyWeights)]),
    "nir_acg_decode_greedy": (_i, [c_fp, c_fp, c_fp, c_ip, _l, _i, c_fp, _l, _i, c_ip, _l, _i, C.POINTER(Seq2seqDecoderWeights),
                                   C.POINTER(AcgCopyWeights), c_ip, c_ip, c_ip, _i, C.c_void_p, _z, c_ip, c_fp, c_st]),
    "nir_acg_copy_loss_fwd": (_i, [c_fp, _l, c_fp, c_fp, c_ip, c_ip, _i, _l, _i, c_fp, c_fp, C.c_void_p, c_st]),
    "nir_acg_copy_loss_bwd": (_i, [c_fp, _l, c_fp, c_fp, c_ip, c_ip, _i, c_fp, c_fp, _l, _i, c_fp, c_fp, c_fp, c_st]),
}

# ... 386 lines not shown
```

### context_attentive_ir_amd/multitask/cars.py

```python
from collections import OrderedDict

import torch
import torch.nn as nn

from .. import autograd as A
from .. import lib
from ..constants import BOS, PAD
from ..encoders.rnn_encoder import lstm_cat_weights
from ..modules import Maxout
from . import suggest
from .layers import Embedder, Encoder


def _attn_mlp(n, p):
    return nn.Sequential(nn.Linear(n, n), nn.Tanh(), nn.Dropout(p=p), nn.Linear(n, 1))


def _projector(i, o, p, bias):
    return nn.Sequential(OrderedDict([("dropout", nn.Dropout(p=p)), ("linear", nn.Linear(i, o, bias=bias))]))


class _RNNDecoderParams(nn.Module):

    def __init__(self, emsize, nhid):
        super().__init__()
        self.rnn = nn.LSTM(emsize, nhid, 1, batch_first=True)
        self.attn = nn.Module()
        self.attn.linear_in = nn.Linear(nhid, nhid, bias=False)
        self.attn.linear_out = nn.Linear(2 * nhid, nhid, bias=False)


def _wsum(x, w):
    return (x * w.unsqueeze(2)).sum(1)


class CARS(nn.Module, lib.IdCheck):
    def __init__(self, args):
        super().__init__()
        if args.rnn_type != "LSTM" or not args.bidirection or args.nlayers != 1 or args.pool_type != "attn":
            raise NotImplementedError("HIP CARS supports the reference configuration (hyparam.py:197-225): LSTM, bidirectional, 1 layer, "
                                      "pool_type='attn' (GRU / stacked layers fail in the reference's own session loop too)")
        if getattr(args, "attn_type", "general") != "general":
            raise NotImplementedError("HIP CARS decoder supports attn_type='general' (hyparam.py:206)")
        p = args.dropout
        self.no_ranker = bool(args.turn_ranker_off)
        self.no_recommender = bool(args.turn_recommender_off)
        self.no_query_session_encoding = bool(args.query_session_off)
        self.no_document_session_encoding = bool(args.doc_session_off)
        q_on, d_on = not self.no_query_session_encoding, not self.no_document_session_encoding
        need_docs = not (self.no_ranker and self.no_document_session_encoding)
        if (q_on and d_on and args.nhid_session_query != args.nhid_session_document) or args.nhid_query != args.nhid_document:
            raise NotImplementedError("HIP CARS expects nhid_query == nhid_document and equal session sizes")
        self.embedder = Embedder(args.emsize, args.src_vocab_size, args.dropout_emb)
        self.query_encoder = Encoder(args.rnn_type, args.emsize, True, 1, args.nhid_query, args.dropout_rnn)
        self.q_attn = _attn_mlp(args.nhid_query, p)
        if need_docs:
            self.document_encoder = Encoder(args.rnn_type, args.emsize, True, 1, args.nhid_document, args.dropout_rnn)
            self.d_attn = _attn_mlp(args.nhid_document, p)
        sess = 0
        if q_on:
            self.nhid_session_query = args.nhid_session_query
            self.session_query_encoder = Encoder(args.rnn_type, args.nhid_query, False, 1, args.nhid_session_query, args.dropout_rnn)
            self.session_query_attn = nn.Linear(args.nhid_session_query, args.nhid_query)
            self.session_query_inner_attn = _attn_mlp(args.nhid_session_query, p)
            sess += args.nhid_session_query
        if d_on:
            self.click_attn = _attn_mlp(args.nhid_document, p)
            self.nhid_session_document = args.nhid_session_document
            self.session_doc_encoder = Encoder(args.rnn_type, args.nhid_document, False, 1, args.nhid_session_document, args.dropout_rnn)
            self.session_doc_attn = nn.Linear(args.nhid_session_document, args.nhid_document)
            self.session_doc_inner_attn = _attn_mlp(args.nhid_session_document, p)
            sess += args.nhid_session_document
        self.session_rep_size = sess
        if sess > 0:
            self.shared_session_projector = _projector(sess, args.nhid_document, p, False)
        if not self.no_ranker:
            self.q_projection = _projector(args.nhid_query, args.nhid_document, p, True)
            if sess > 0:
                self.private_session_projector1 = _projector(sess, args.nhid_document, p, False)
            self.ranknet = Maxout(args.nhid_document * 4, 3, [256, 128, 1], [2, 2, 2])
        if not self.no_recommender:
            if sess == 0:
                raise ValueError("Both session-level RNNs cannot be off!")
            self.private_session_projector2 = _projector(sess, args.nhid_document, p, False)
            self.transform_hid = _projector(sess, args.nhid_decoder, p, True)
            self.transform_cell = _projector(sess, args.nhid_decoder, p, True)
            self.decoder = nn.Module()
            self.decoder.decoder = _RNNDecoderParams(args.emsize, args.nhid_decoder)
            self.dec_attn = nn.Linear(args.nhid_query, args.nhid_decoder, bias=False)
            pred_in = args.nhid_document if need_docs else args.emsize
            self.token_prob_predictor1 = nn.Linear(args.nhid_decoder, pred_in, bias=False)
            self.token_prob_predictor2 = nn.Linear(pred_in, args.tgt_vocab_size, bias=False)
        self.dropout = nn.Dropout(args.dropout)
        self.dec_dropout_p = float(args.dropout_rnn)
        self.regularize_coeff = args.regularize_coeff
        self.pool_type = args.pool_type
        self.lambda1, self.lambda2 = args.lambda1, args.lambda2
        hs = args.nhid_session_query if q_on else args.nhid_session_document
        self._dims = dict(D=args.nhid_document, HS=hs, HDEC=args.nhid_decoder, q_on=int(q_on), d_on=int(d_on),
                          rank_on=int(not self.no_ranker))
        self._pq, self._pd, self._ps, self._pdec = lib.PackCache(), lib.PackCache(), lib.PackCache(), lib.PackCache()
        self.fold_embeddings = getattr(args, "fold_embeddings", True)
        self.fuse_attention_pooling = True
        self.fuse_generator_topk = True
        self.fuse_decoder_argmax = True
        self.fold_decoder_step = True
        self.fold_decoder_query = True
        self.fold_budget_bytes = 64 << 30
        self.compute_dtype = getattr(args, "compute_dtype", "f32")
        self._fq, self._fd = lib.PackCache(retain=1), lib.PackCache(retain=1)

    def _enc_weights(self, which):
        enc = (self.query_encoder if which == "q" else self.document_encoder).encoder
        attn = self.q_attn if which == "q" else self.d_attn
        cache = self._pq if which == "q" else self._pd

        def build():
            wih, whh, bih, bhh = lstm_cat_weights(enc.rnns[0])
            bounded = float(attn[0].weight.detach().abs().max()) < 32768.0
            table = self.embedder.word_embeddings.table
            gb = float(table.detach().abs().max()) < 32768.0 and float(wih.detach().abs().max()) < 32768.0
            rec_ok = float(whh.detach().abs().max()) < 32768.0
            pk = lib.Packed(lib.CarsEncoderWeights,
                            dict(wih=wih, whh=whh, bih=bih, bhh=bhh, attn0_w=attn[0].weight, attn0_b=attn[0].bias,
                                 attn3_w=attn[3].weight, attn3_b=attn[3].bias),
                            dict(H=enc.hidden, bounded=int(bounded) | (int(gb) << 1) | (int(rec_ok) << 2)))
            pk.rec_ok = rec_ok
            L = lib.load()
            nb = L.nir_lstm_whh_frag_bytes(enc.hidden, 2)
            if nb and pk.rec_ok and whh.is_cuda:
                pk.keep["whh_frag"] = torch.empty(nb, dtype=torch.uint8, device=whh.device)
                lib.check(L.nir_lstm_pack_whh_frag(lib.ptr(pk.keep["whh"]), enc.hidden, 2, lib.ptr(pk.keep["whh_frag"]), None, lib.stream()),
                          "nir_lstm_pack_whh_frag")
                pk.struct.whh_frag = pk.keep["whh_frag"].data_ptr()
            if bounded and 2 * enc.hidden == 256 and self.fuse_attention_pooling and attn[0].weight.is_cuda:
                planes = torch.stack(lib.split_f16x2(pk.keep["attn0_w"], 256))
                pk.keep["attn_frag"] = planes.view(2, 16, 16, 8, 4, 8).permute(3, 1, 0, 4, 2, 5).contiguous()
                pk.struct.attn_frag = pk.keep["attn_frag"].data_ptr()
            return pk
        return cache.get(list(enc.parameters()) + list(attn.parameters()) + [self.embedder.word_embeddings.table], build)

    def _session_modules(self):
        names = ["click_attn", "session_query_attn", "session_doc_attn", "session_query_encoder", "session_doc_encoder",
                 "q_projection", "shared_session_projector", "private_session_projector1", "ranknet",
                 "session_query_inner_attn", "session_doc_inner_attn", "transform_hid", "transform_cell"]
        return [getattr(self, n) for n in names if hasattr(self, n)]

    def _session_weights(self):
        def build():
            t = {}
            if hasattr(self, "click_attn"):
                sd = self.session_doc_encoder.encoder.rnns[0]
                t.update(click0_w=self.click_attn[0].weight, click0_b=self.click_attn[0].bias,
                         click3_w=self.click_attn[3].weight, click3_b=self.click_attn[3].bias,
                         sd_attn_w=self.session_doc_attn.weight, sd_attn_b=self.session_doc_attn.bias,
                         sd_wih=sd.weight_ih_l0, sd_whh=sd.weight_hh_l0, sd_bih=sd.bias_ih_l0, sd_bhh=sd.bias_hh_l0,
                         sd_inner0_w=self.session_doc_inner_attn[0].weight, sd_inner0_b=self.session_doc_inner_attn[0].bias,
                         sd_inner3_w=self.session_doc_inner_attn[3].weight, sd_inner3_b=self.session_doc_inner_attn[3].bias)
            if hasattr(self, "session_query_encoder"):
                sq = self.session_query_encoder.encoder.rnns[0]
                t.update(sq_attn_w=self.session_query_attn.weight, sq_attn_b=self.session_query_attn.bias,
                         sq_wih=sq.weight_ih_l0, sq_whh=sq.weight_hh_l0, sq_bih=sq.bias_ih_l0, sq_bhh=sq.bias_hh_l0,
                         sq_inner0_w=self.session_query_inner_attn[0].weight, sq_inner0_b=self.session_query_inner_attn[0].bias,
                         sq_inner3_w=self.session_query_inner_attn[3].weight, sq_inner3_b=self.session_query_inner_attn[3].bias)
            if not self.no_ranker:
                mo = self.ranknet._linear_layers
                t.update(qproj_w=self.q_projection.linear.weight, qproj_b=self.q_projection.linear.bias,
                         mo0_w=mo[0].weight, mo0_b=mo[0].bias, mo1_w=mo[1].weight, mo1_b=mo[1].bias,
                         mo2_w=mo[2].weight, mo2_b=mo[2].bias)
                if self.session_rep_size:
                    t.update(shared_w=self.shared_session_projector.linear.weight,
                             priv1_w=self.private_session_projector1.linear.weight)
            if not self.no_recommender:
                t.update(th_w=self.transform_hid.linear.weight, th_b=self.transform_hid.linear.bias,
                         tc_w=self.transform_cell.linear.weight, tc_b=self.transform_cell.linear.bias)
            pk = lib.Packed(lib.CarsSessionWeights, t, self._dims)
            L = lib.load()
            HS_ = self._dims["HS"]
            nb = L.nir_lstm_step_whh_frag_bytes(HS_)
            for key in ("sq", "sd"):
                if nb and (key + "_whh") in pk.keep:
                    dev = pk.keep[key + "_whh"].device
                    frag, flag = torch.empty(nb, dtype=torch.uint8, device=dev), torch.zeros(1, dtype=torch.int32, device=dev)
                    lib.check(L.nir_lstm_step_pack_whh_frag(lib.ptr(pk.keep[key + "_whh"]), HS_, lib.ptr(frag), lib.ptr(flag), lib.stream()),
                              "nir_lstm_step_pack_whh_frag")
                    if int(flag.item()) == 0:
                        pk.keep[key + "_whh_frag"] = frag
                        setattr(pk.struct, key + "_whh_frag", frag.data_ptr())
            b3 = int(all(float(pk.keep[k].abs().max()) < 32768.0 for k in ("sq_wih", "sd_wih") if k in pk.keep))
            pk.struct.rank_bounded = b3 << 3
            if not self.no_ranker:
                L = lib.load()
                na, nb = lib.C.c_size_t(0), lib.C.c_size_t(0)
                L.nir_cars_session_pack_floats(pk.ref(), lib.C.byref(na), lib.C.byref(nb))
                dev = self.q_projection.linear.weight.device
                pk.keep["wrank"] = torch.empty(max(na.value, 1), device=dev)
                pk.keep["attn_ut"] = torch.empty(max(nb.value, 1), device=dev)
                lib.check(L.nir_cars_session_pack(pk.ref(), lib.ptr(pk.keep["wrank"]), lib.ptr(pk.keep["attn_ut"]), lib.stream()),
                          "nir_cars_session_pack")
                pk.struct.wrank = pk.keep["wrank"].data_ptr()
                pk.struct.attn_ut = pk.keep["attn_ut"].data_ptr()
                D_ = self._dims["D"]
                kr = na.value // D_ if D_ else 0
                qb = float((pk.keep["wrank"][:D_ * kr].view(D_, kr).abs().sum(1) + pk.keep["qproj_b"].abs()).max()) if kr else 0.0
                b0 = int(qb + 1.0 < 32768.0 and float(pk.keep["mo0_w"].abs().max()) < 32768.0)
                y0 = (qb + 1.0) * float(pk.keep["mo0_w"].abs().sum(1).max()) + float(pk.keep["mo0_b"].abs().max())
                b1 = int(b0 and y0 < 32768.0 and float(pk.keep["mo1_w"].abs().max()) < 32768.0)
                b2 = int("click0_w" in pk.keep and float(pk.keep["click0_w"].abs().max()) < 32768.0)
                pk.struct.rank_bounded = b0 | (b1 << 1) | (b2 << 2) | (b3 << 3)
            return pk
        return self._ps.get([p for m in self._session_modules() for p in m.parameters()], build)

    def _decoder_weights(self):
        def build():
            rnn, att = self.decoder.decoder.rnn, self.decoder.decoder.attn
            t = dict(rnn_wih=rnn.weight_ih_l0, rnn_whh=rnn.weight_hh_l0, rnn_bih=rnn.bias_ih_l0, rnn_bhh=rnn.bias_hh_l0,
                     attn_in_w=att.linear_in.weight, attn_out_w=att.linear_out.weight, dec_attn_w=self.dec_attn.weight,
                     pred1_w=self.token_prob_predictor1.weight, pred2_w=self.token_prob_predictor2.weight)
            ints = dict(HD=rnn.hidden_size, DQ=self.dec_attn.weight.shape[1], P=self.token_prob_predictor1.weight.shape[0],
                        KS=self.session_rep_size, VT=self.token_prob_predictor2.weight.shape[0])
            pk = lib.Packed(lib.CarsDecoderWeights, t, ints)
            a = self.shared_session_projector.linear.weight.detach().float().contiguous()
            b = self.private_session_projector2.linear.weight.detach().float().contiguous()
            pk.keep["sess_w"] = torch.empty_like(a)
            lib.check(lib.load().nir_add_f32(lib.ptr(a), lib.ptr(b), lib.ptr(pk.keep["sess_w"]), a.numel(), lib.stream()), "nir_add_f32")
            pk.struct.sess_w = pk.keep["sess_w"].data_ptr()
            w2 = pk.keep["pred2_w"]
            VT, P = w2.shape
            if self.fuse_decoder_argmax and P == 256 and w2.is_cuda and float(w2.abs().max()) < 32768.0:
                vp = (VT + 15) // 16 * 16
                pad = torch.zeros(vp, P, device=w2.device, dtype=torch.float32)
                pad[:VT] = w2
                planes = torch.stack(lib.split_f16x2(pad, P))
                pk.keep["pred2_frag"] = planes.view(2, vp // 16, 16, P // 32, 4, 8).permute(1, 3, 0, 4, 2, 5).contiguous()
                pk.struct.pred2_frag = pk.keep["pred2_frag"].data_ptr()
            if self.fold_decoder_query and w2.is_cuda:
                HDa, DQ = self.dec_attn.weight.shape
                a_t = pk.keep["attn_in_w"].t().contiguous()
                d_t = pk.keep["dec_attn_w"].t().contiguous()
                wq = torch.empty(HDa, DQ, device=w2.device, dtype=torch.float32)
                lib.check(lib.load().nir_linear_f32(lib.ptr(a_t), HDa, None, None, 0, 0, 0, lib.ptr(d_t), HDa, None, None, lib.ptr(wq), DQ, HDa, DQ, HDa,
                                                    0, lib.stream()), "nir_linear_f32")
                pk.keep["attn_q_w"] = wq
                pk.struct.attn_q_w = wq.data_ptr()
            table = self.embedder.word_embeddings.table
            HD = int(rnn.hidden_size)
            nb = lib.load().nir_lstm_step_whh_frag_bytes(HD)
            if (self.fold_decoder_step and self.fold_embeddings and nb and table.is_cuda and table.shape[1] == rnn.input_size
                    and table.shape[0] * 4 * HD * 4 <= self.fold_budget_bytes):
                frag, flag = torch.empty(nb, dtype=torch.uint8, device=table.device), torch.zeros(1, dtype=torch.int32, device=table.device)
                lib.check(lib.load().nir_lstm_step_pack_whh_frag(lib.ptr(pk.keep["rnn_whh"]), HD, lib.ptr(frag), lib.ptr(flag), lib.stream()),
                          "nir_lstm_step_pack_whh_frag")
                if int(flag.item()) == 0:
                    pk.keep["rnn_whh_frag"] = frag
                    pk.keep["rnn_gate_fold"] = lib.fold_lstm_table(table, pk.keep["rnn_wih"], pk.keep["rnn_bih"], pk.keep["rnn_bhh"], HD, 1, "f32")
                    pk.struct.rnn_whh_frag = frag.data_ptr()
                    pk.struct.rnn_gate_fold = pk.keep["rnn_gate_fold"].data_ptr()
            return pk
        mods = [self.decoder, self.dec_attn, self.token_prob_predictor1, self.token_prob_predictor2,
                self.shared_session_projector, self.private_session_projector2]
        return self._pdec.get([p for m in mods for p in m.parameters()] + [self.embedder.word_embeddings.table, self.fold_decoder_step,
                                                                         self.fuse_decoder_argmax, self.fold_decoder_query], build)

    def _check_eval(self):
        if self.training:
            raise RuntimeError("CARS.encode / encode_document / rank_document / decode are the inference entry points: call them in "
                               "eval mode (the train-mode path is forward(), which runs the differentiable operators with dropout)")

    def _folded_table(self, which, w):
        table = self.embedder.word_embeddings.table
        enc = (self.query_encoder if which == "q" else self.document_encoder).encoder
        cache = self._fq if which == "q" else self._fd
        dt = "bf16" if self.compute_dtype == "bf16" else "f32"
        return cache.get([table] + list(enc.parameters()) + [dt],
                         lambda: lib.fold_lstm_table(table, w.keep["wih"], w.keep["bih"], w.keep["bhh"], w.struct.H, 2, dt))

    def _use_fold(self, table, H):
        if not self.fold_embeddings or self.training:
            return False
        per = table.shape[0] * 8 * H * (2 if self.compute_dtype == "bf16" else 4)
        return 2 * per <= self.fold_budget_bytes and H >= 8 and (2 * H) % 64 == 0

    def _encode_seqs(self, which, ids, lens, want_encoded):
        table = self.embedder.word_embeddings.table
        lib.require_device(ids, lens, table)
        L = lib.load()
        ids, lens = lib.ids64(ids), lib.ids64(lens)
        M, T = ids.shape
        w = self._enc_weights(which)
        H2 = 2 * w.struct.H
        dev = ids.device
        pooled = torch.empty(M, H2, device=dev, dtype=torch.float32)
        encoded = torch.empty(M, T, H2, device=dev, dtype=torch.float32) if want_encoded else None
        if self._use_fold(table, w.struct.H) and w.rec_ok:
# ... 480 lines not shown
```

### include/neuroir_hip.h

```cpp
#ifndef NEUROIR_HIP_H
#define NEUROIR_HIP_H

#include <stddef.h>
#include <stdint.h>

#ifdef __cplusplus
extern "C" {
#endif

typedef void* nir_stream_t;

#define NIR_ERR_BAD_ARG (-1)
#define NIR_ERR_UNSUPPORTED (-2)
#define NIR_ERR_WORKSPACE (-3)

#define NIR_DTYPE_F32 0
#define NIR_DTYPE_BF16 1
#define NIR_DTYPE_F32_SPLIT2 2

int nir_version(void);
const char* nir_last_error_string(void);

int nir_set_stream_batches_in_flight(nir_stream_t stream, int n);
int nir_debug_set_tunable(const char* name , int value);

int nir_debug_clock_probe(void* out , int iters, int blocks, void* sink , nir_stream_t stream);
int nir_debug_set_buffer(void* dev_u64);
int nir_profile_enable(int on);
int nir_profile_report(char* buf , size_t cap);

int nir_split_f16x2(const float* x, int64_t rows, int cols, int64_t ld, int cols_pad, void* p1, void* p2, nir_stream_t stream);

int nir_linear_planes_f32(const void* a1, const void* a2, int64_t lda, const int64_t* ids, int64_t rows_per_seq, int64_t seq_stride, int EP,
                          int taps, const void* w1, const void* w2, int64_t ldw, const float* bias, float* c, int64_t ldc, int64_t M, int N,
                          int K, int act, nir_stream_t stream);

int nir_sanitize_ids(const int64_t* a, int64_t na, const int64_t* b, int64_t nb, int64_t V, int64_t* out_a, int64_t* out_b,
                     int* err_flag, nir_stream_t stream);

int nir_flag_publish(const int* dev_flag, int* host_flag , nir_stream_t stream);

int nir_gather_fields(const int64_t* table , int n, void* dst , int64_t total_bytes, nir_stream_t stream);
int nir_host_device_pointer(const void* host, void** device_visible );

int nir_softmax_rows_publish(const float* scores, float* probs, int64_t rows, int n, const int* dev_flag, int* host_flag, nir_stream_t stream);

double nir_host_rank_metric(int what, const int64_t* predictions , const void* target , int label_dtype, int64_t rows, int n, int k);

int nir_widen_ids_i32(const int32_t* src, int64_t* dst, int64_t n, nir_stream_t stream);


#define NIR_ACT_NONE 0
#define NIR_ACT_TANH 1
#define NIR_ACT_RELU 2

int nir_linear_f32(const float* a, int64_t lda, const int64_t* ids, const float* table, int E,
                   int64_t rows_per_seq, int64_t seq_stride, const float* w, int64_t ldw, const float* bias,
                   const float* bias2, float* c, int64_t ldc, int64_t M, int N, int K, int act,
                   nir_stream_t stream);

#define NIR_ACT_MAXOUT2 16
#define NIR_ACT_TANH_ROWDOT16 17
#define NIR_ACT_BOUNDED 0x100
int nir_linear_ex_f32(const float* a, int64_t lda, const int64_t* ids, const float* table, int E,
                      int64_t rows_per_seq, int64_t seq_stride, const float* w, int64_t ldw, const float* bias,
                      const float* bias2, float* c, int64_t ldc, int64_t M, int N, int K, int act,
                      const float* add, int64_t ldadd, nir_stream_t stream);

int nir_rowdot_f32(const float* x, int64_t ldx, const float* w, const float* b, float* out, int64_t M, int K,
                   int act, nir_stream_t stream);

int nir_bilstm_fwd(const float* gates_in, const int64_t* lengths, const float* w_hh, const float* h0,
                   const float* c0, float* out, float* hn, float* cn, int64_t M, int T, int H, int ndir,
                   nir_stream_t stream);
int nir_bilstm_supported(int H);
int nir_bilstm_fused_fwd(const float* x, int I, const float* w_ih, const float* b_ih, const float* b_hh,
                         const int64_t* lengths, const float* w_hh, const float* h0, const float* c0, float* out,
                         float* hn, float* cn, int64_t M, int T, int H, int ndir, nir_stream_t stream);

int nir_softmax_rows(const float* in, float* out, int64_t rows, int n, nir_stream_t stream);
int nir_softmax_gathered(const float* gathered, float* probs, float* scores, int world, int64_t B, int per, int N,
                         nir_stream_t stream);
int nir_rank_loss_bce(const float* scores, const float* labels, int64_t rows, int n, float* loss,
                      nir_stream_t stream);
int nir_rank_loss_softmax_nll(const float* scores, const float* labels, int64_t rows, int n, float* loss,
                              nir_stream_t stream);

int nir_esm_score(const int64_t* q_ids, const int64_t* d_ids, int B, int N, int QL, int DL,
                  const float* table, int64_t V, int E, float* scores, nir_stream_t stream);

typedef struct {
    const float* gate_w;
    const float* gate_b;
    const float* ffnn0_w;
    const float* ffnn0_b;
    const float* ffnn1_w;
    const float* ffnn1_b;
    const float* out_w;
    const float* out_b;
    int snap_one;
    const signed char* self_bin;
} nir_drmm_weights;
int nir_drmm_score(const int64_t* q_ids, const int64_t* d_ids, int B, int N, int QL, int DL,
                   const float* table, int64_t V, int E, const nir_drmm_weights* w , float* scores,
                   float* hist_out, nir_stream_t stream);

typedef struct {
    const float *proj_w, *proj_b;
    const float *q_wih, *q_whh, *q_bih, *q_bhh;
    const float *d_wih, *d_whh, *d_bih, *d_bhh;
    const float *qproj_w, *qproj_b;
    const float *dproj_w, *dproj_b;
    const float* alpha;
    const float *conv1_w, *conv1_b;
    const float *conv2_w, *conv2_b;
    const float *conv3_w, *conv3_b;
    const float *conv_w, *conv_b;
    const float *out_w, *out_b;
// ... 86 lines not shown
size_t nir_conv1d_planes_bytes(int C_in, int F, int k);
int nir_conv1d_pack(const float* w, int C_in, int F, int k, void* planes, float* wt, int* flag, nir_stream_t stream);
size_t nir_conv1d_pool_out_floats(int64_t M, int L, int F, int p, int head);
int nir_conv1d_pool_f32(const int64_t* ids, const float* x, int64_t M, int L, const nir_conv1d_layer* layer , int act, const float* head_w,
                        float* out, nir_stream_t stream);
size_t nir_arci_workspace_bytes(int B, int N, int QL, int DL, const nir_arci_weights* w );
int nir_arci_score(const int64_t* q_ids, const int64_t* d_ids, int B, int N, int QL, int DL, const float* table, int64_t V, int E,
                   const nir_arci_weights* w , void* workspace, size_t workspace_bytes, float* scores, nir_stream_t stream);

#define NIR_ARCII_MAX_LAYERS 8
typedef struct {
    const void* planes;
    const float* wt;
    const float* bias;
    int C_in, F, kh, kw, ph, pw, path;
} nir_conv2d_layer;
typedef struct {
    nir_conv1d_layer q, d;
    nir_conv2d_layer l[NIR_ARCII_MAX_LAYERS];
    const float* head_w;
    const float* head_b;
    int n_layers, feats;
} nir_arcii_weights;
size_t nir_conv2d_planes_bytes(int C_in, int F, int kh, int kw);
int nir_conv2d_pack(const float* w, int C_in, int F, int kh, int kw, void* planes, float* wt, int* flag, nir_stream_t stream);
size_t nir_conv2d_pool_out_floats(int64_t M, int H, int W, int F, int ph, int pw, int head);
int nir_conv2d_pool_f32(const float* x, const float* pd, const float* pq, int64_t M, int N, int H, int W, const nir_conv2d_layer* layer ,
                        int act, const float* head_w, float* out, nir_stream_t stream);
size_t nir_arcii_workspace_bytes(int B, int N, int QL, int DL, const nir_arcii_weights* w );
int nir_arcii_score(const int64_t* q_ids, const int64_t* d_ids, int B, int N, int QL, int DL, const float* table, int64_t V, int E,
                    const nir_arcii_weights* w , void* workspace, size_t workspace_bytes, float* scores, nir_stream_t stream);

typedef struct {
    const float *wih, *whh, *bih, *bhh;
    const float *attn0_w, *attn0_b;
    const float *attn3_w, *attn3_b;
    int H;
    int bounded;
    const void* attn_frag;
    const void* whh_frag;
} nir_cars_encoder_weights;
size_t nir_cars_encode_workspace_bytes(int64_t M, int T, int E, const nir_cars_encoder_weights* w );
int nir_cars_encode(const int64_t* ids, const int64_t* lens, int64_t M, int T, const float* table, int64_t V, int E,
                    const nir_cars_encoder_weights* w , void* workspace, size_t workspace_bytes,
                    float* pooled, float* encoded, nir_stream_t stream);

size_t nir_lstm_fold_table_bytes(int64_t V, int H, int ndir, int dtype);
size_t nir_lstm_fold_table_workspace_bytes(int64_t V, int E, int H, int ndir, int dtype);
int nir_lstm_fold_table(const float* table, int64_t V, int E, const float* w_ih, const float* b_ih, const float* b_hh, int H,
                        int ndir, void* folded, int dtype, void* workspace, size_t workspace_bytes, nir_stream_t stream);
size_t nir_lstm_whh_frag_bytes(int H, int ndir);
int nir_lstm_pack_whh_frag(const float* w_hh, int H, int ndir, void* frag, int* err_flag, nir_stream_t stream);
int nir_bilstm_folded_fwd(const void* folded, int dtype, const int64_t* ids, const int64_t* lengths, const float* w_hh,
                          float* out, int* err_flag, int64_t M, int64_t V, int T, int H, int ndir, nir_stream_t stream);
size_t nir_cars_encode_folded_workspace_bytes(int64_t M, int T, const nir_cars_encoder_weights* w );
int nir_cars_encode_folded(const int64_t* ids, const int64_t* lens, int64_t M, int T, const void* folded, int dtype, int64_t V,
                           const nir_cars_encoder_weights* w , void* workspace, size_t workspace_bytes, float* pooled,
                           float* encoded, int* err_flag, nir_stream_t stream);

#define NIR_ATTN_POOL_ONE_TERM 1
#define NIR_ATTN_POOL_PLAIN 2
size_t nir_attn_pool_workspace_bytes(int64_t M, int T, int D);
int nir_attn_pool_f32(const void* rows, int row_format, const nir_cars_encoder_weights* w , const int64_t* lens, int64_t M, int T,
                      int D, int flags, void* workspace, size_t workspace_bytes, float* pooled, nir_stream_t stream);

typedef struct {
    const float *click0_w, *click0_b, *click3_w, *click3_b;
    const float *sq_attn_w, *sq_attn_b;
    const float *sd_attn_w, *sd_attn_b;
    const float *sq_wih, *sq_whh, *sq_bih, *sq_bhh;
    const float *sd_wih, *sd_whh, *sd_bih, *sd_bhh;
    const float *qproj_w, *qproj_b;
    const float *shared_w, *priv1_w;
    const float *mo0_w, *mo0_b, *mo1_w, *mo1_b, *mo2_w, *mo2_b;
    const float *wrank;
    const float *attn_ut;
    const float *sq_inner0_w, *sq_inner0_b, *sq_inner3_w, *sq_inner3_b;
    const float *sd_inner0_w, *sd_inner0_b, *sd_inner3_w, *sd_inner3_b;
    const float *th_w, *th_b, *tc_w, *tc_b;
    int D, HS, HDEC;
    int q_on, d_on, rank_on;
    int rank_bounded;
    const void *sq_whh_frag, *sd_whh_frag;
} nir_cars_session_weights;
typedef struct {
    float* inner_q;
    float* inner_d;
    float* dec_h;
    float* dec_c;
} nir_cars_session_outputs;
size_t nir_lstm_step_whh_frag_bytes(int H);
int nir_lstm_step_pack_whh_frag(const float* w_hh, int H, void* frag, int* err_flag, nir_stream_t stream);
size_t nir_cars_session_pack_floats(const nir_cars_session_weights* w , size_t* wrank_floats , size_t* ut_floats );
int nir_cars_session_pack(const nir_cars_session_weights* w , float* wrank, float* attn_ut, nir_stream_t stream);
size_t nir_cars_session_workspace_bytes(int B, int S, int N, const nir_cars_session_weights* w );
int nir_cars_rank_session(const float* pooled_q, const float* pooled_docs, const float* labels, int B, int S, int N,
                          const nir_cars_session_weights* w , void* workspace, size_t workspace_bytes,
                          float* click_scores, float* clicks_out, const nir_cars_session_outputs* extra ,
                          nir_stream_t stream);
int nir_cars_rank_session_shard(const float* pooled_q, const float* pooled_docs, const float* labels, int B, int S, int N,
                                const nir_cars_session_weights* w , void* workspace, size_t workspace_bytes,
                                float* click_scores, float* clicks_out, const nir_cars_session_outputs* extra ,
                                const float* rank_docs, int NR, nir_stream_t stream);
int nir_cars_rank_session_rows(const float* pooled_q, const float* pooled_docs, const float* labels, int B, int S, int N,
                               const nir_cars_session_weights* w , void* workspace, size_t workspace_bytes,
                               float* click_scores, float* clicks_out, const nir_cars_session_outputs* extra ,
                               const float* rank_docs, int NR, const float* labels_all, int64_t rows_all, const int* m_groups,
                               int sessions_per_group, nir_stream_t stream);
int nir_cars_session_query_side(const float* pooled_q, int B, int S, const nir_cars_session_weights* w , float* U, float* gq,
                                nir_stream_t stream);
int nir_cars_rank_session_pre(const float* pooled_q, const float* pooled_docs, const float* labels, int B, int S, int N,
                              const nir_cars_session_weights* w , void* workspace, size_t workspace_bytes,
                              float* click_scores, float* clicks_out, const nir_cars_session_outputs* extra ,
                              const float* rank_docs, int NR, const float* labels_all, int64_t rows_all, const int* m_groups,
                              int sessions_per_group, const float* pre_U, const float* pre_gq, nir_stream_t stream);
int nir_cars_click_max(const float* labels, int groups, int rows, int N, int* m_out, nir_stream_t stream);

typedef struct {
    const float *rnn_wih, *rnn_whh, *rnn_bih, *rnn_bhh;
    const float *attn_in_w;
    const float *attn_out_w;
    const float *dec_attn_w;
    const float *pred1_w;
    const float *pred2_w;
    const float *sess_w;
    int HD, DQ, P, KS;
    int64_t VT;
    const void* pred2_frag;
    const float* rnn_gate_fold;
    const void* rnn_whh_frag;
    const float* attn_q_w;
} nir_cars_decoder_weights;
int nir_add_f32(const float* a, const float* b, float* out, int64_t n, nir_stream_t stream);
size_t nir_cars_decode_workspace_bytes(int64_t rows_src, int64_t Bd, int QL, const nir_cars_decoder_weights* w );
int nir_cars_decode_greedy(const float* dec_h, const float* dec_c, const float* encoded_source, const int64_t* source_len,
                           int64_t rows_src, int QL, const int64_t* rowmap, int64_t Bd, const float* session_cat,
                           const float* table, int64_t V, int E, const int64_t* tgt2src, int64_t bos, int max_len,
                           const nir_cars_decoder_weights* w , void* workspace, size_t workspace_bytes,
                           int64_t* predictions, nir_stream_t stream);

size_t nir_bilstm_steps_workspace_bytes(int64_t M, int H);
int nir_bilstm_steps_fwd(const float* gates_in, const int64_t* lengths, const float* w_hh, const float* h0, const float* c0,
                         float* out, float* hn, float* cn, int64_t M, int T, int H, int ndir, void* workspace,
                         size_t workspace_bytes, nir_stream_t stream);
size_t nir_lstm256_whh_frag_bytes(int ndir);
int nir_lstm256_pack_whh_frag(const float* w_hh, int ndir, void* frag, int* err_flag, nir_stream_t stream);
size_t nir_lstm256_workspace_bytes(int64_t M, int ndir);
int nir_lstm256_rows_fwd(const float* rows, const int64_t* ids, const int64_t* lengths, const void* whh_frag, float* out, int mode,
                         int* err_flag, int64_t M, int64_t R, int T, int ndir, void* workspace, size_t workspace_bytes, nir_stream_t stream);
int nir_lstm256_train_fwd(const float* gates_perm, const int64_t* lengths, const void* whh_frag, float* out, float* act, float* cst,
                          int* err_flag, int64_t M, int T, int ndir, void* workspace, size_t workspace_bytes, nir_stream_t stream);
size_t nir_lstm256_bptt_workspace_bytes(int64_t M, int ndir);
int nir_lstm256_bptt(const float* dout, const float* act, const float* cst, const int64_t* lengths, const float* w_hh, float* dgates,
                     int64_t M, int T, int ndir, void* workspace, size_t workspace_bytes, nir_stream_t stream);

#define NIR_CELL_LSTM 0
#define NIR_CELL_GRU 1
int nir_birnn_steps_fwd(int cell, const float* gates_in, const int64_t* lengths, const float* w_hh, const float* b_hh, const float* h0,
                        const float* c0, float* out, float* c_steps , float* hn,
                        float* cn, int64_t M, int T, int H, int ndir, void* workspace, size_t workspace_bytes, nir_stream_t stream);

int nir_maxpool_time_f32(const float* x, int64_t M, int T, int D, float* y, nir_stream_t stream);

size_t nir_decode_greedy_plain_workspace_bytes(int64_t Bd, int H, int64_t VT);
int nir_decode_greedy_plain(const float* dec_h, const float* dec_c, int64_t Bd, int H, const float* table, int64_t V, int E, const float* w_ih,
                            const float* w_hh, const float* b_ih, const float* b_hh, const float* gen_w, const float* gen_b, int64_t VT,
                            const int64_t* tgt2src, int64_t bos, int max_len, void* workspace, size_t workspace_bytes, int64_t* predictions,
                            nir_stream_t stream);
int nir_decode_greedy_plain_folded(const float* dec_h, const float* dec_c, int64_t Bd, int H, const float* table, int64_t V, int E,
                                   const float* w_ih, const float* w_hh, const float* b_ih, const float* b_hh, const float* gen_w,
                                   const float* gen_b, int64_t VT, const int64_t* tgt2src, int64_t bos, int max_len, const float* gate_fold,
                                   const void* whh_frag, void* workspace, size_t workspace_bytes, int64_t* predictions, nir_stream_t stream);

typedef struct {
    const float *q_wih, *q_whh, *q_bih, *q_bhh;
    const float *d_wih, *d_whh, *d_bih, *d_bhh;
    const float *s_wih, *s_whh, *s_bih, *s_bhh;
// ... 185 lines not shown
```

Before: 8.487 million pairs/s.

## Pre-split session GEMM weights into fp16 hi/lo planes and emit activation planes

Adds a one-time packing step that splits five session-model weight matrices (click0, sq/sd input projections, maxout layers) into two fp16 planes. The session GEMMs then run through a plane-based linear path that takes pre-split weights. Producer kernels (click pooling, rank feature construction, mo0 output) write fp16 hi/lo activation planes directly, so the consumer GEMMs skip the per-call f32-to-fp16 split. This aims to cut GEMM conversion and memory cost, at the price of extra plane writes, more workspace reuse, and dependence on the bounded-magnitude checks for accuracy.

Result: no change. 8.484 million pairs/s (-0.0%).

```diff
diff --git a/context_attentive_ir_amd/csrc/cars_session.hip b/context_attentive_ir_amd/csrc/cars_session.hip
--- a/context_attentive_ir_amd/csrc/cars_session.hip
+++ b/context_attentive_ir_amd/csrc/cars_session.hip
@@ -10,6 +10,11 @@
 int launch_linear_ex(const float* a, int64_t lda, const int64_t* ids, const float* table, int E, int64_t rows_per_seq,
                      int64_t seq_stride, const float* w, int64_t ldw, const float* bias, const float* bias2, float* c,
                      int64_t ldc, int64_t M, int N, int K, int act, const float* add, int64_t ldadd, hipStream_t st);
+int launch_linear_wplanes(const float* a, const void* a1, const void* a2, int64_t lda, const void* w1, const void* w2, int64_t ldw,
+                          const float* bias, const float* bias2, float* c, void* c1, void* c2, int64_t ldc, int64_t M, int N, int K, int act,
+                          const float* add, hipStream_t st);
+int launch_split_f16x2_rtz(const float* x, int64_t rows, int cols, int64_t ld, int cols_pad, void* p1, void* p2, int* err, hipStream_t st);
+bool linear_split_shape(const float* a, int64_t lda, int64_t M, int N, int K);
 constexpr int ACT_MAXOUT2 = 16;
 constexpr int ACT_BOUNDED = 0x100;
 constexpr int ACT_TANH_ROWDOT16 = 17;
@@ -19,7 +24,8 @@
                                                           const float* __restrict__ b3, const float* __restrict__ labels,
                                                           const float* __restrict__ labels_all, int rows_all,
                                                           const int* __restrict__ mg, int rpg,
-                                                          int rows, int N, int D, float* __restrict__ clicks) {
+                                                          int rows, int N, int D, float* __restrict__ clicks,
+                                                          _Float16* __restrict__ ch1, _Float16* __restrict__ ch2) {
     __shared__ int part[4];
     const int lane = threadIdx.x & 63, wave = threadIdx.x >> 6;
     if (!mg) {
@@ -72,7 +78,14 @@
             const float4 v = *reinterpret_cast<const float4*>(docs + ((int64_t)r * N + k) * D + 4 * c);
             acc.x = fmaf(pk, v.x, acc.x); acc.y = fmaf(pk, v.y, acc.y); acc.z = fmaf(pk, v.z, acc.z); acc.w = fmaf(pk, v.w, acc.w);
         }
-        if (c0 + lane < nch) *reinterpret_cast<float4*>(clicks + (int64_t)r * D + 4 * c) = acc;
+        if (c0 + lane < nch) {
+            *reinterpret_cast<float4*>(clicks + (int64_t)r * D + 4 * c) = acc;
+            if (ch1) {
+                const Split2x4 h = split2(acc);
+                *reinterpret_cast<uint2*>(ch1 + (int64_t)r * D + 4 * c) = h.hi;
+                *reinterpret_cast<uint2*>(ch2 + (int64_t)r * D + 4 * c) = h.lo;
+            }
+        }
     }
 }
 
@@ -107,7 +120,7 @@
                                                              const float* __restrict__ b3, const float* __restrict__ labels,
                                                              const float* __restrict__ labels_all, int rows_all,
                                                              const int* __restrict__ mg, int rpg, int rows, int N, int D,
-                                                             float* __restrict__ clicks) {
+                                                             float* __restrict__ clicks, _Float16* __restrict__ ch1, _Float16* __restrict__ ch2) {
     extern __shared__ float csm[];
     __shared__ int part[4];
     const int lane = threadIdx.x & 63, wave = threadIdx.x >> 6;
@@ -177,6 +190,11 @@
             acc.x = fmaf(pk, v.x, acc.x); acc.y = fmaf(pk, v.y, acc.y); acc.z = fmaf(pk, v.z, acc.z); acc.w = fmaf(pk, v.w, acc.w);
         }
         *reinterpret_cast<float4*>(clicks + (int64_t)r * D + 4 * c) = acc;
+        if (ch1) {
+            const Split2x4 h = split2(acc);
+            *reinterpret_cast<uint2*>(ch1 + (int64_t)r * D + 4 * c) = h.hi;
+            *reinterpret_cast<uint2*>(ch2 + (int64_t)r * D + 4 * c) = h.lo;
+        }
     }
 }
 
@@ -575,6 +593,25 @@
     }
 }
 
+__global__ void rank_feats_planes_kernel(const float* qp, const float* docs, int N, int D, int64_t rows, _Float16* f1, _Float16* f2) {
+    const int64_t i = ((int64_t)blockIdx.x * blockDim.x + threadIdx.x) * 4;
+    if (i < rows * D) {
+        const int64_t r = i / D;
+        const int f = (int)(i % D);
+        const float4 q = *reinterpret_cast<const float4*>(qp + (r / N) * D + f), d = *reinterpret_cast<const float4*>(docs + r * D + f);
+        const int64_t o = r * 4 * D + f;
+        const Split2x4 sq = split2(q), sd = split2(d);
+        const Split2x4 sa = split2(make_float4(fabsf(q.x - d.x), fabsf(q.y - d.y), fabsf(q.z - d.z), fabsf(q.w - d.w)));
+        float4 m = make_float4(q.x * d.x, q.y * d.y, q.z * d.z, q.w * d.w);
+        asm volatile("" : "+v"(m.x), "+v"(m.y), "+v"(m.z), "+v"(m.w));
+        const Split2x4 sm = split2(m);
+        *reinterpret_cast<uint2*>(f1 + o) = sq.hi;         *reinterpret_cast<uint2*>(f2 + o) = sq.lo;
+        *reinterpret_cast<uint2*>(f1 + o + D) = sd.hi;     *reinterpret_cast<uint2*>(f2 + o + D) = sd.lo;
+        *reinterpret_cast<uint2*>(f1 + o + 2 * D) = sa.hi; *reinterpret_cast<uint2*>(f2 + o + 2 * D) = sa.lo;
+        *reinterpret_cast<uint2*>(f1 + o + 3 * D) = sm.hi; *reinterpret_cast<uint2*>(f2 + o + 3 * D) = sm.lo;
+    }
+}
+
 __global__ __launch_bounds__(256) void session_inner_pool_kernel(const float* __restrict__ states, const float* __restrict__ lpart,
                                                                  int NP, const float* __restrict__ b3, int B, int S, int HS,
                                                                  float* __restrict__ out ) {
@@ -609,7 +646,7 @@
 }
 
 struct SessPlan {
-    float *epart, *clicks, *Qs, *Ds, *Cq, *Cd, *U, *xcat, *qp, *feats, *y0, *y1, *lin, *cat, *gx, *Qs16, *Ds16;
+    float *epart, *clicks, *Qs, *Ds, *Cq, *Cd, *U, *xcat, *qp, *feats, *y0, *y1, *lin, *cat, *gx, *Qs16, *Ds16, *clicks16;
     size_t bytes;
 };
 static SessPlan sess_plan(void* ws, size_t cap, int B, int S, int N, int D, int HS, int nch, bool rank_on, bool want_states) {
@@ -633,6 +670,7 @@
     p.gx = a.take<float>((size_t)nch * BS * 4 * HS);
     p.Qs16 = a.take<float>((size_t)(S + 1) * B * HS);
     p.Ds16 = a.take<float>((size_t)(S + 1) * B * HS);
+    p.clicks16 = a.take<float>(BS * D);
     p.bytes = align_up(a.off, 256);
     return p;
 }
@@ -671,6 +709,61 @@
     return 0;
 }
 
+namespace nir {
+struct SessPlaneLayer { const float* w; int64_t rows; int K; int bit; const void* p1; const void* p2; };
+static void sess_plane_layers(const nir_cars_session_weights* w, SessPlaneLayer (&l)[5]) {
+    const int D = w->D, HS = w->HS;
+    l[0] = {w->click0_w, D, D, 4, w->click0_w1, w->click0_w2};
+    l[1] = {w->sq_wih, 4 * (int64_t)HS, D, 8, w->sq_wih1, w->sq_wih2};
+    l[2] = {w->sd_wih, 4 * (int64_t)HS, D, 8, w->sd_wih1, w->sd_wih2};
+    l[3] = {w->mo0_w, 512, 4 * D, 1, w->mo0_w1, w->mo0_w2};
+    l[4] = {w->mo1_w, 256, 256, 2, w->mo1_w1, w->mo1_w2};
+}
+static bool sess_use_planes(const nir_cars_session_weights* w, int layer, const float* a, int64_t M) {
+    SessPlaneLayer l[5];
+    sess_plane_layers(w, l);
+    const SessPlaneLayer& y = l[layer];
+    return y.p1 && y.p2 && (w->rank_bounded & y.bit) && linear_split_shape(a, y.K, M, (int)y.rows, y.K);
+}
+static int sess_gemm(const nir_cars_session_weights* w, int layer, bool planes, const float* a, const void* a1, const void* a2, const float* bias,
+                     const float* bias2, float* c, void* c1, void* c2, int64_t ldc, int64_t M, int act, const float* add, hipStream_t st) {
+    SessPlaneLayer l[5];
+    sess_plane_layers(w, l);
+    const SessPlaneLayer& y = l[layer];
+    if (planes) return launch_linear_wplanes(a, a1, a2, y.K, y.p1, y.p2, (y.K + 7) / 8 * 8, bias, bias2, c, c1, c2, ldc, M, (int)y.rows, y.K, act, add, st);
+    return launch_linear_ex(a, y.K, nullptr, nullptr, 0, 0, 0, y.w, y.K, bias, bias2, c, ldc, M, (int)y.rows, y.K,
+                            act | ((w->rank_bounded & y.bit) ? ACT_BOUNDED : 0), add, 0, st);
+}
+}
+
+extern "C" size_t nir_cars_session_plane_bytes(const nir_cars_session_weights* w, size_t* offsets) {
+    if (!w || w->D <= 0 || w->HS <= 0) return 0;
+    nir::SessPlaneLayer l[5];
+    nir::sess_plane_layers(w, l);
+    size_t off = 0;
+    for (int i = 0; i < 5; ++i) {
+        if (offsets) offsets[i] = l[i].w ? off : (size_t)-1;
+        if (l[i].w) off = nir::align_up(off + (size_t)2 * l[i].rows * ((l[i].K + 7) / 8 * 8) * sizeof(_Float16), 256);
+    }
+    return off;
+}
+
+extern "C" int nir_cars_session_pack_planes(const nir_cars_session_weights* w, void* buffer, size_t buffer_bytes, int* err_flag, nir_stream_t stream) {
+    using namespace nir;
+    size_t offs[5];
+    const size_t need = nir_cars_session_plane_bytes(w, offs);
+    NIR_REQUIRE(w && buffer && need && buffer_bytes >= need && ((uintptr_t)buffer & 255) == 0, "cars_session_pack_planes: buffer missing, misaligned or too small");
+    SessPlaneLayer l[5];
+    sess_plane_layers(w, l);
+    for (int i = 0; i < 5; ++i) {
+        if (!l[i].w || !(w->rank_bounded & l[i].bit)) continue;
+        const int KP = (l[i].K + 7) / 8 * 8;
+        char* p1 = (char*)buffer + offs[i];
+        NIR_PROPAGATE(launch_split_f16x2_rtz(l[i].w, l[i].rows, l[i].K, l[i].K, KP, p1, p1 + (size_t)l[i].rows * KP * sizeof(_Float16), err_flag, (hipStream_t)stream));
+    }
+    return 0;
+}
+
 extern "C" size_t nir_cars_session_workspace_bytes(int B, int S, int N, const nir_cars_session_weights* w) {
     if (!w || B < 0 || S <= 0 || N <= 0) return 0;
     const int nch = (w->q_on ? 1 : 0) + (w->d_on ? 1 : 0);
@@ -719,13 +812,13 @@
     const bool q_on = w->q_on != 0, d_on = w->d_on != 0, rank_on = w->rank_on != 0;
     const int nch = (q_on ? 1 : 0) + (d_on ? 1 : 0), D = w->D, HS = w->HS, NU = nch * HS + nch;
     const int64_t BS = (int64_t)B * S;
-    const int bnd = (w->rank_bounded & 8) ? ACT_BOUNDED : 0;
     NIR_REQUIRE(!(nch && rank_on) || (U && w->attn_ut), "cars_session_query_side: U / packed attention weights missing");
     NIR_REQUIRE(!(nch && q_on) || gq, "cars_session_query_side: gq missing");
     if (nch && rank_on)
         NIR_PROPAGATE(launch_linear(pooled_q, D, nullptr, nullptr, 0, 0, 0, w->attn_ut, D, nullptr, nullptr, U, NU, BS, NU, D, NIR_ACT_NONE, st));
     if (nch && q_on)
-        NIR_PROPAGATE(launch_linear_ex(pooled_q, D, nullptr, nullptr, 0, 0, 0, w->sq_wih, D, w->sq_bih, w->sq_bhh, gq, 4 * HS, BS, 4 * HS, D, NIR_ACT_NONE | bnd, nullptr, 0, st));
+        NIR_PROPAGATE(sess_gemm(w, 1, sess_use_planes(w, 1, pooled_q, BS), pooled_q, nullptr, nullptr, w->sq_bih, w->sq_bhh, gq, nullptr, nullptr, 4 * HS, BS,
+                                NIR_ACT_NONE, nullptr, st));
     return 0;
 }
 
@@ -765,28 +858,32 @@
     const float* gq = (pre_gq && q_on) ? pre_gq : p.gx;
     float* gd = p.gx + (q_on ? BS * 4 * (int64_t)HS : 0);
     const float* Uq = (pre_U && nch && rank_on) ? pre_U : p.U;
-    const int bnd = (w->rank_bounded & 8) ? ACT_BOUNDED : 0;
+    const bool sd_planes = d_on && sess_use_planes(w, 2, clicks, BS);
+    _Float16* ch1 = sd_planes ? reinterpret_cast<_Float16*>(p.clicks16) : nullptr;
+    _Float16* ch2 = sd_planes ? ch1 + BS * D : nullptr;
     {
         hipStream_t sq_ = st;
         if (nch && rank_on && Uq == p.U)
             NIR_PROPAGATE(launch_linear(pooled_q, D, nullptr, nullptr, 0, 0, 0, w->attn_ut, D, nullptr, nullptr, p.U, NU, BS, NU, D, NIR_ACT_NONE, sq_));
-        if (nch && q_on && gq == p.gx) NIR_PROPAGATE(launch_linear_ex(pooled_q, D, nullptr, nullptr, 0, 0, 0, w->sq_wih, D, w->sq_bih, w->sq_bhh, p.gx, 4 * HS, BS, 4 * HS, D, NIR_ACT_NONE | bnd, nullptr, 0, sq_));
+        if (nch && q_on && gq == p.gx)
+            NIR_PROPAGATE(sess_gemm(w, 1, sess_use_planes(w, 1, pooled_q, BS), pooled_q, nullptr, nullptr, w->sq_bih, w->sq_bhh, p.gx, nullptr, nullptr, 4 * HS, BS,
+                                    NIR_ACT_NONE, nullptr, sq_));
     }
     if (d_on) {
-        NIR_PROPAGATE(launch_linear_ex(pooled_docs, D, nullptr, nullptr, 0, 0, 0, w->click0_w, D, w->click0_b, nullptr, p.epart, NP, R, D, D,
-                                       ACT_TANH_ROWDOT16 | ((w->rank_bounded & 4) ? ACT_BOUNDED : 0), w->click3_w, 0, st));
+        NIR_PROPAGATE(sess_gemm(w, 0, sess_use_planes(w, 0, pooled_docs, R), pooled_docs, nullptr, nullptr, w->click0_b, nullptr, p.epart, nullptr, nullptr, NP, R,
+                                ACT_TANH_ROWDOT16, w->click3_w, st));
         {
             ProfScope ps("click_pool2_kernel", st);
             const float* lall = labels_all ? labels_all : labels;
             const int rall = labels_all ? (int)rows_all : (int)BS;
             if (N <= 64)
                 hipLaunchKernelGGL(click_pool2_kernel, dim3((unsigned)((BS + 3) / 4)), dim3(256), 0, st, pooled_docs, p.epart, NP, w->click3_b, labels,
-                                   lall, rall, m_groups, sessions_per_group * S, (int)BS, N, D, clicks);
+                                   lall, rall, m_groups, sessions_per_group * S, (int)BS, N, D, clicks, ch1, ch2);
             else {
                 static std::once_flag once;
                 std::call_once(once, [] { (void)hipFuncSetAttribute((const void*)click_pool_big_kernel, hipFuncAttributeMaxDynamicSharedMemorySize, 4 * 2 * 2048 * (int)sizeof(float)); });
                 hipLaunchKernelGGL(click_pool_big_kernel, dim3((unsigned)((BS + 3) / 4)), dim3(256), (size_t)4 * 2 * N * sizeof(float), st, pooled_docs,
-                                   p.epart, NP, w->click3_b, labels, lall, rall, m_groups, sessions_per_group * S, (int)BS, N, D, clicks);
+                                   p.epart, NP, w->click3_b, labels, lall, rall, m_groups, sessions_per_group * S, (int)BS, N, D, clicks, ch1, ch2);
             }
         }
         NIR_CHECK_LAUNCH("click_pool2_kernel");
@@ -801,7 +898,7 @@
         a.chain0 = q_on ? 0 : 1;
         a.B = B; a.I = D; a.H = HS;
         {
-            if (d_on) NIR_PROPAGATE(launch_linear_ex(clicks, D, nullptr, nullptr, 0, 0, 0, w->sd_wih, D, w->sd_bih, w->sd_bhh, gd, 4 * HS, BS, 4 * HS, D, NIR_ACT_NONE | bnd, nullptr, 0, st));
+            if (d_on) NIR_PROPAGATE(sess_gemm(w, 2, sd_planes, clicks, ch1, ch2, w->sd_bih, w->sd_bhh, gd, nullptr, nullptr, 4 * HS, BS, NIR_ACT_NONE, nullptr, st));
             a.gx[0] = gq; a.gx[1] = gd;
             a.gxstride = (int64_t)S * 4 * HS;
             a.whh_frag[0] = w->sq_whh_frag; a.whh_frag[1] = w->sd_whh_frag;
@@ -838,15 +935,21 @@
         const float* rdocs = rank_docs ? rank_docs : pooled_docs;
         const int Nr = rank_docs ? NR : N;
         const int64_t Rr = BS * Nr;
+        const bool m0_planes = sess_use_planes(w, 3, p.feats, Rr), m1_planes = sess_use_planes(w, 4, p.y0, Rr);
+        _Float16* f1 = reinterpret_cast<_Float16*>(p.feats);
+        _Float16* f2 = f1 + Rr * 4 * D;
+        const bool y0_planes = m0_planes && m1_planes;
+        _Float16* y01 = y0_planes ? reinterpret_cast<_Float16*>(p.y0) : nullptr;
+        _Float16* y02 = y0_planes ? y01 + Rr * 256 : nullptr;
         {
             ProfScope ps("rank_feats_kernel", st);
-            hipLaunchKernelGGL(rank_feats_kernel, g1(Rr * D / 4), dim3(256), 0, st, p.qp, rdocs, Nr, D, Rr, p.feats);
+            if (m0_planes) hipLaunchKernelGGL(rank_feats_planes_kernel, g1(Rr * D / 4), dim3(256), 0, st, p.qp, rdocs, Nr, D, Rr, f1, f2);
+            else hipLaunchKernelGGL(rank_feats_kernel, g1(Rr * D / 4), dim3(256), 0, st, p.qp, rdocs, Nr, D, Rr, p.feats);
         }
         NIR_CHECK_LAUNCH("rank_feats_kernel");
-        NIR_PROPAGATE(launch_linear_ex(p.feats, 4 * D, nullptr, nullptr, 0, 0, 0, w->mo0_w, 4 * D, w->mo0_b, nullptr, p.y0, 256, Rr, 512, 4 * D,
-                                       ACT_MAXOUT2 | ((w->rank_bounded & 1) ? ACT_BOUNDED : 0), nullptr, 0, st));
-        NIR_PROPAGATE(launch_linear_ex(p.y0, 256, nullptr, nullptr, 0, 0, 0, w->mo1_w, 256, w->mo1_b, nullptr, p.y1, 128, Rr, 256, 256,
-                                       ACT_MAXOUT2 | ((w->rank_bounded & 2) ? ACT_BOUNDED : 0), nullptr, 0, st));
+        NIR_PROPAGATE(sess_gemm(w, 3, m0_planes, p.feats, m0_planes ? f1 : nullptr, f2, w->mo0_b, nullptr, y0_planes ? nullptr : p.y0, y01, y02, 256, Rr,
+                                ACT_MAXOUT2, nullptr, st));
+        NIR_PROPAGATE(sess_gemm(w, 4, m1_planes, p.y0, y01, y02, w->mo1_b, nullptr, p.y1, nullptr, nullptr, 128, Rr, ACT_MAXOUT2, nullptr, st));
         NIR_PROPAGATE(launch_linear_ex(p.y1, 128, nullptr, nullptr, 0, 0, 0, w->mo2_w, 128, w->mo2_b, nullptr, click_scores, 1, Rr, 2, 128, ACT_MAXOUT2, nullptr, 0, st));
     }
     if (want_states) {
diff --git a/context_attentive_ir_amd/csrc/gemm.hip b/context_attentive_ir_amd/csrc/gemm.hip
--- a/context_attentive_ir_amd/csrc/gemm.hip
+++ b/context_attentive_ir_amd/csrc/gemm.hip
@@ -23,33 +23,51 @@
     int N, K, act;
     const float* add;
     int64_t ldadd;
+    _Float16 *c1, *c2;
 };
 
 constexpr int ACT_MAXOUT2 = 16;
 constexpr int ACT_TANH_ROWDOT16 = 17;
 constexpr int ACT_BOUNDED = 0x100;
 
-__device__ __forceinline__ void gemm_store(const GemmArgs& p, int64_t m, int n, float v, float bsum) {
+template <bool CP>
+__device__ __forceinline__ void gemm_put(const GemmArgs& p, int64_t i, float v) {
+    if (CP) {
+        asm volatile("" : "+v"(v));
+        const _Float16 h = split2_hi1_rtz(v);
+        p.c1[i] = h;
+        p.c2[i] = split2_hi1_rtz(split2_res(v, h));
+    } else {
+        p.c[i] = v;
+    }
+}
+
+template <bool CP = false>
+__device__ __forceinline__ void gemm_store_a(const GemmArgs& p, const int act, const float addn, int64_t m, int n, float v, float bsum) {
     v += bsum;
-    if (p.act == ACT_TANH_ROWDOT16) {
-        v = n < p.N ? fast_tanh(v) * p.add[n] : 0.f;
+    if (act == ACT_TANH_ROWDOT16) {
+        v = n < p.N ? fast_tanh(v) * addn : 0.f;
         v += dpp_mov<0xB1>(v);
         v += dpp_mov<0x4E>(v);
         v += dpp_mov<0x141>(v);
         v += dpp_mov<0x140>(v);
-        if (m < p.M && n < p.N && !(n & 15)) p.c[m * p.ldc + (n >> 4)] = v;
+        if (m < p.M && n < p.N && !(n & 15)) gemm_put<CP>(p, m * p.ldc + (n >> 4), v);
         return;
     }
     if (p.add && m < p.M && n < p.N) v += p.add[m * p.ldadd + n];
-    if (p.act == NIR_ACT_TANH) v = fast_tanh(v);
-    else if (p.act == NIR_ACT_RELU) v = fmaxf(v, 0.f);
-    if (p.act == ACT_MAXOUT2) {
+    if (act == NIR_ACT_TANH) v = fast_tanh(v);
+    else if (act == NIR_ACT_RELU) v = fmaxf(v, 0.f);
+    if (act == ACT_MAXOUT2) {
         const float other = dpp_mov<0xB1>(v);
         v = fmaxf(v, other);
-        if (m < p.M && n < p.N && !(n & 1)) p.c[m * p.ldc + (n >> 1)] = v;
+        if (m < p.M && n < p.N && !(n & 1)) gemm_put<CP>(p, m * p.ldc + (n >> 1), v);
     } else if (m < p.M && n < p.N) {
-        p.c[m * p.ldc + n] = v;
-    }
+        gemm_put<CP>(p, m * p.ldc + n, v);
+    }
+}
+template <bool CP = false>
+__device__ __forceinline__ void gemm_store(const GemmArgs& p, int64_t m, int n, float v, float bsum) {
+    gemm_store_a<CP>(p, p.act, (p.act == ACT_TANH_ROWDOT16 && n < p.N) ? p.add[n] : 0.f, m, n, v, bsum);
 }
 
 #ifndef NIR_GEMM_BK
@@ -762,16 +780,28 @@
     int64_t ldw;
     GemmArgs ep;
     int K;
+    int KA;
+#ifdef NIR_GP_STAMP
+    unsigned long long* dbg;
+#endif
 };
+#ifdef NIR_GP_STAMP
+#define GP_STAMP(slot) do { if (q.dbg && threadIdx.x == 0 && blockIdx.x < 4096) q.dbg[blockIdx.x * 8 + (slot)] = wall_clock64(); } while (0)
+#define GP_STAMP_ARG(q) (q).dbg = g_debug_buf
+#else
+#define GP_STAMP(slot)
+#define GP_STAMP_ARG(q)
+#endif
 constexpr int GP_BK = 32;
 constexpr int GP_CHUNK = 128 * 8 + 32;
 constexpr int GP_PLANE = 4 * GP_CHUNK;
 
-template <int MODE>
+template <int MODE, bool AF32 = false, bool CP = false>
 __global__ __launch_bounds__(256, 2) void gemm_h2p_kernel(GemmPlaneArgs q) {
     extern __shared__ __attribute__((aligned(16))) unsigned short smemp[];
     unsigned short* As = smemp;
     unsigned short* Ws = smemp + 2 * 2 * GP_PLANE;
+    GP_STAMP(0);
     const GemmArgs& p = q.ep;
     const int tid = threadIdx.x, lane = tid & 63, wave = tid >> 6;
     const int wm = wave >> 1, wn = wave & 1;
@@ -788,7 +818,9 @@
     int64_t m = m0 + lr;
     m = m < p.M ? m : p.M - 1;
     int64_t arow[3] = {0, 0, 0};
-    if (MODE == 0) {
+    if (AF32) {
+        arow[0] = m * p.lda;
+    } else if (MODE == 0) {
         arow[0] = m * q.lda;
     } else {
         const int64_t ai = (m / q.rows_per_seq) * q.seq_stride + (m % q.rows_per_seq);
@@ -799,8 +831,12 @@
     n = n < p.N ? n : p.N - 1;
     const int64_t wrow = (int64_t)n * q.ldw;
 
-    uint4 ra[2][2], rw[2][2];
-    auto load_tile = [&](int k0, bool tail) {
+    struct TileRegs {
+        uint4 ra[2][2], rw[2][2];
+        float4 fa[4];
+    };
+    TileRegs R0;
+    auto load_tile = [&](TileRegs& R, int k0, bool tail) {
         int k = k0 + 16 * hs;
         bool kv = true, kv2 = true;
         if (tail) {
@@ -813,28 +849,46 @@
         const int k2 = kv2 ? k + 8 : k;
         int64_t ao2 = ao;
         if (MODE == 2) ao2 = k2 < q.EP ? arow[0] : (k2 < 2 * q.EP ? arow[1] : arow[2]);
-        ra[0][0] = *reinterpret_cast<const uint4*>(q.a1 + ao + k);
-        ra[1][0] = *reinterpret_cast<const uint4*>(q.a2 + ao + k);
-        ra[0][1] = *reinterpret_cast<const uint4*>(q.a1 + ao2 + k2);
-        ra[1][1] = *reinterpret_cast<const uint4*>(q.a2 + ao2 + k2);
-        rw[0][0] = *reinterpret_cast<const uint4*>(q.w1 + wrow + k);
-        rw[1][0] = *reinterpret_cast<const uint4*>(q.w2 + wrow + k);
-        rw[0][1] = *reinterpret_cast<const uint4*>(q.w1 + wrow + k2);
-        rw[1][1] = *reinterpret_cast<const uint4*>(q.w2 + wrow + k2);
+        if (AF32) {
+#pragma unroll
+            for (int j = 0; j < 4; ++j) {
+                const int kj = k0 + 16 * hs + 4 * j;
+                const bool v = !tail || kj < q.KA;
+                R.fa[j] = *reinterpret_cast<const float4*>(p.a + ao + (v ? kj : 0));
+                if (tail && !v) R.fa[j] = make_float4(0.f, 0.f, 0.f, 0.f);
+            }
+        } else {
+            R.ra[0][0] = *reinterpret_cast<const uint4*>(q.a1 + ao + k);
+            R.ra[1][0] = *reinterpret_cast<const uint4*>(q.a2 + ao + k);
+            R.ra[0][1] = *reinterpret_cast<const uint4*>(q.a1 + ao2 + k2);
+            R.ra[1][1] = *reinterpret_cast<const uint4*>(q.a2 + ao2 + k2);
+        }
+        R.rw[0][0] = *reinterpret_cast<const uint4*>(q.w1 + wrow + k);
+        R.rw[1][0] = *reinterpret_cast<const uint4*>(q.w2 + wrow + k);
+        R.rw[0][1] = *reinterpret_cast<const uint4*>(q.w1 + wrow + k2);
+        R.rw[1][1] = *reinterpret_cast<const uint4*>(q.w2 + wrow + k2);
         if (tail) {
             const uint4 z = make_uint4(0u, 0u, 0u, 0u);
-            if (!kv) { ra[0][0] = z; ra[1][0] = z; rw[0][0] = z; rw[1][0] = z; }
-            if (!kv2) { ra[0][1] = z; ra[1][1] = z; rw[0][1] = z; rw[1][1] = z; }
+            if (!kv) { R.rw[0][0] = z; R.rw[1][0] = z; if (!AF32) { R.ra[0][0] = z; R.ra[1][0] = z; } }
+            if (!kv2) { R.rw[0][1] = z; R.rw[1][1] = z; if (!AF32) { R.ra[0][1] = z; R.ra[1][1] = z; } }
         }
     };
-    auto store_tile = [&](int buf) {
+    auto store_tile = [&](TileRegs& R, int buf) {
+        if (AF32) {
+#pragma unroll
+            for (int c = 0; c < 2; ++c) {
+                const Split2x4 lo = split2(R.fa[2 * c]), hi = split2(R.fa[2 * c + 1]);
+                R.ra[0][c] = make_uint4(lo.hi.x, lo.hi.y, hi.hi.x, hi.hi.y);
+                R.ra[1][c] = make_uint4(lo.lo.x, lo.lo.y, hi.lo.x, hi.lo.y);
+            }
+        }
 #pragma unroll
         for (int t = 0; t < 2; ++t)
 #pragma unroll
             for (int c = 0; c < 2; ++c) {
                 const int off = (buf * 2 + t) * GP_PLANE + (hs * 2 + c) * GP_CHUNK + lr * 8;
-                *reinterpret_cast<uint4*>(As + off) = ra[t][c];
-                *reinterpret_cast<uint4*>(Ws + off) = rw[t][c];
+                *reinterpret_cast<uint4*>(As + off) = R.ra[t][c];
+                *reinterpret_cast<uint4*>(Ws + off) = R.rw[t][c];
             }
     };
     f32x16 acc[2][2], acx[2][2];
@@ -846,11 +900,25 @@
             for (int r = 0; r < 16; ++r) { acc[a][b][r] = 0.0f; acx[a][b][r] = 0.0f; }
 
     const int nk = (q.K + GP_BK - 1) / GP_BK;
-    const bool ktail = (q.K % GP_BK) != 0;
-    if (nk == 1 && ktail) load_tile(0, true);
-    else load_tile(0, false);
-    store_tile(0);
+    const bool ktail = ((AF32 ? q.KA : q.K) % GP_BK) != 0;
+    load_tile(R0, 0, nk == 1 && ktail);
+    GP_STAMP(1);
+    float bsum[2], addn[2];
+#pragma unroll
+    for (int b = 0; b < 2; ++b) {
+        const int nn = n0 + wn * 64 + b * 32 + (lane & 31);
+        bsum[b] = 0.f;
+        addn[b] = 0.f;
+        if (nn < p.N) {
+            if (p.bias) bsum[b] += p.bias[nn];
+            if (p.bias2) bsum[b] += p.bias2[nn];
+            if (p.act == ACT_TANH_ROWDOT16) addn[b] = p.add[nn];
+        }
+    }
+    store_tile(R0, 0);
+    GP_STAMP(2);
     __syncthreads();
+    GP_STAMP(3);
     const int foff_a = (lane >> 5) * GP_CHUNK + (wm * 64 + (lane & 31)) * 8;
     const int foff_w = (lane >> 5) * GP_CHUNK + (wn * 64 + (lane & 31)) * 8;
     auto mma_tile = [&](int buf) {
@@ -876,40 +944,42 @@
         }
     };
     for (int kt = 0; kt + 2 < nk; ++kt) {
-        load_tile((kt + 1) * GP_BK, false);
+        load_tile(R0, (kt + 1) * GP_BK, false);
         __builtin_amdgcn_sched_barrier(0);
         mma_tile(kt & 1);
         __builtin_amdgcn_sched_barrier(0);
-        store_tile((kt & 1) ^ 1);
+        store_tile(R0, (kt & 1) ^ 1);
         __syncthreads();
     }
     if (nk >= 2) {
         const int kt = nk - 2;
-        if (ktail) load_tile((kt + 1) * GP_BK, true);
-        else load_tile((kt + 1) * GP_BK, false);
+        load_tile(R0, (kt + 1) * GP_BK, ktail);
         __builtin_amdgcn_sched_barrier(0);
         mma_tile(kt & 1);
         __builtin_amdgcn_sched_barrier(0);
-        store_tile((kt & 1) ^ 1);
+        store_tile(R0, (kt & 1) ^ 1);
         __syncthreads();
     }
     mma_tile((nk - 1) & 1);
-#pragma unroll
-    for (int b = 0; b < 2; ++b) {
-        const int nn = n0 + wn * 64 + b * 32 + (lane & 31);
-        float bsum = 0.f;
-        if (nn < p.N) {
-            if (p.bias) bsum += p.bias[nn];
-            if (p.bias2) bsum += p.bias2[nn];
-        }
+    GP_STAMP(4);
+    auto epilogue = [&](const int act) __attribute__((always_inline)) {
 #pragma unroll
         for (int a = 0; a < 2; ++a)
 #pragma unroll
             for (int r = 0; r < 16; ++r) {
                 const int64_t mm = m0 + wm * 64 + a * 32 + (r & 3) + 8 * (r >> 2) + 4 * (lane >> 5);
-                gemm_store(p, mm, nn, split2_combine(acc[a][b][r], acx[a][b][r]), bsum);
-            }
-    }
+#pragma unroll
+                for (int b = 0; b < 2; ++b) {
+                    const int nn = n0 + wn * 64 + b * 32 + (lane & 31);
+                    gemm_store_a<CP>(p, act, addn[b], mm, nn, split2_combine(acc[a][b][r], acx[a][b][r]), bsum[b]);
+                }
+            }
+    };
+    if (p.act == ACT_MAXOUT2) epilogue(ACT_MAXOUT2);
+    else if (p.act == ACT_TANH_ROWDOT16) epilogue(ACT_TANH_ROWDOT16);
+    else if (p.act == NIR_ACT_NONE) epilogue(NIR_ACT_NONE);
+    else epilogue(p.act);
+    GP_STAMP(5);
 }
 
 __global__ void split_f16x2_kernel(const float* __restrict__ x, int64_t rows, int cols, int64_t ld, int cols_pad, _Float16* __restrict__ p1,
@@ -942,8 +1012,9 @@
     if (M == 0) return 0;
     GemmPlaneArgs q;
     q.a1 = (const _Float16*)a1; q.a2 = (const _Float16*)a2; q.lda = lda; q.ids = ids; q.rows_per_seq = rows_per_seq; q.seq_stride = seq_stride;
-    q.EP = EP; q.taps = taps; q.w1 = (const _Float16*)w1; q.w2 = (const _Float16*)w2; q.ldw = ldw; q.K = K;
-    q.ep = GemmArgs{nullptr, 0, nullptr, nullptr, 0, 0, 0, nullptr, 0, bias, nullptr, c, ldc, M, N, K, act, add, ldadd};
+    q.EP = EP; q.taps = taps; q.w1 = (const _Float16*)w1; q.w2 = (const _Float16*)w2; q.ldw = ldw; q.K = K; q.KA = K;
+    GP_STAMP_ARG(q);
+    q.ep = GemmArgs{nullptr, 0, nullptr, nullptr, 0, 0, 0, nullptr, 0, bias, nullptr, c, ldc, M, N, K, act, add, ldadd, nullptr, nullptr};
     const int64_t mb3 = (M + G3_BM - 1) / G3_BM;
     const int nb3 = (N + G3_BN - 1) / G3_BN;
     constexpr size_t lds = (size_t)2 * 2 * 2 * GP_PLANE * 2;
@@ -956,6 +1027,78 @@
     dim3 grid((unsigned)(8 * nb3 * ((mb3 + 7) / 8)));
     if (ids) hipLaunchKernelGGL(gemm_h2p_kernel<2>, grid, dim3(256), lds, st, q);
     else hipLaunchKernelGGL(gemm_h2p_kernel<0>, grid, dim3(256), lds, st, q);
+    NIR_CHECK_LAUNCH("gemm_h2p_kernel");
+    return 0;
+}
+
+__global__ void split_f16x2_rtz_kernel(const float* __restrict__ x, int64_t rows, int cols, int64_t ld, int cols_pad, _Float16* __restrict__ p1,
+                                       _Float16* __restrict__ p2, int* __restrict__ err) {
+    const int64_t i = (int64_t)blockIdx.x * blockDim.x + threadIdx.x;
+    if (i >= rows * cols_pad) return;
+    const int64_t r = i / cols_pad;
+    const int c = (int)(i % cols_pad);
+    const float v = c < cols ? x[r * ld + c] : 0.f;
+    if (!(fabsf(v) < 32768.f)) {
+        if (err) atomicOr(err, 2);
+        return;
+    }
+    const _Float16 a = split2_hi1_rtz(v);
+    p1[i] = a;
+    p2[i] = split2_hi1_rtz(split2_res(v, a));
+}
+
+int launch_split_f16x2_rtz(const float* x, int64_t rows, int cols, int64_t ld, int cols_pad, void* p1, void* p2, int* err, hipStream_t st) {
+    NIR_REQUIRE(x && p1 && p2 && rows >= 0 && cols > 0 && cols_pad >= cols && cols_pad % 8 == 0, "split_f16x2_rtz: bad args (cols_pad %% 8 == 0)");
+    if (rows == 0) return 0;
+    const int64_t n = rows * cols_pad;
+    hipLaunchKernelGGL(split_f16x2_rtz_kernel, dim3((unsigned)((n + 255) / 256)), dim3(256), 0, st, x, rows, cols, ld, cols_pad, (_Float16*)p1, (_Float16*)p2, err);
+    NIR_CHECK_LAUNCH("split_f16x2_rtz_kernel");
+    return 0;
+}
+
+bool linear_split_shape(const float* a, int64_t lda, int64_t M, int N, int K) {
+    const int64_t mb3 = (M + G3_BM - 1) / G3_BM;
+    const int nb3 = (N + G3_BN - 1) / G3_BN;
+    const bool vec = (K % 4 == 0) && (!a || ((lda % 4 == 0) && (((uintptr_t)a & 15) == 0)));
+    return vec && tun(g_tun.exact_f32) == 0 && N >= 96 && K >= 32 && mb3 * nb3 >= 96;
+}
+
+int launch_linear_wplanes(const float* a, const void* a1, const void* a2, int64_t lda, const void* w1, const void* w2, int64_t ldw,
+                          const float* bias, const float* bias2, float* c, void* c1, void* c2, int64_t ldc, int64_t M, int N, int K, int act,
+                          const float* add, hipStream_t st) {
+    const bool af32 = a1 == nullptr, cp = c == nullptr;
+    NIR_REQUIRE(w1 && w2 && M >= 0 && N > 0 && K > 0 && (af32 ? (a != nullptr) : (a2 != nullptr)) && (cp ? (c1 && c2) : true), "linear_wplanes: bad args");
+    const int KP = (K + 7) / 8 * 8;
+    NIR_REQUIRE(ldw % 8 == 0 && ldw >= KP, "linear_wplanes: the W planes' row stride must be a multiple of 8 and hold the padded K");
+    NIR_REQUIRE(af32 ? (K % 4 == 0 && lda % 4 == 0 && ((uintptr_t)a & 15) == 0) : (lda % 8 == 0 && lda >= KP && ((uintptr_t)a1 & 15) == 0 && ((uintptr_t)a2 & 15) == 0),
+                "linear_wplanes: fp32 A needs K %% 4 == 0 and 16-byte rows, plane A a row stride that is a multiple of 8 and holds the padded K");
+    NIR_REQUIRE((((uintptr_t)w1 | (uintptr_t)w2) & 15) == 0, "linear_wplanes: W planes must be 16-byte aligned");
+    NIR_REQUIRE(act == NIR_ACT_NONE || act == NIR_ACT_TANH || act == NIR_ACT_RELU || act == ACT_MAXOUT2 || act == ACT_TANH_ROWDOT16, "linear_wplanes: bad activation");
+    NIR_REQUIRE(act != ACT_MAXOUT2 || (N % 2 == 0), "linear_wplanes: maxout epilogue needs an even N");
+    NIR_REQUIRE(act != ACT_TANH_ROWDOT16 || (N % 16 == 0 && add != nullptr), "linear_wplanes: tanh-rowdot epilogue needs N %% 16 == 0 and the weight row");
+    if (M == 0) return 0;
+    GemmPlaneArgs q;
+    q.a1 = (const _Float16*)a1; q.a2 = (const _Float16*)a2; q.lda = lda; q.ids = nullptr; q.rows_per_seq = 0; q.seq_stride = 0;
+    q.EP = 0; q.taps = 0; q.w1 = (const _Float16*)w1; q.w2 = (const _Float16*)w2; q.ldw = ldw; q.K = KP; q.KA = K;
+    q.ep = GemmArgs{a, lda, nullptr, nullptr, 0, 0, 0, nullptr, 0, bias, bias2, c, ldc, M, N, KP, act, act == ACT_TANH_ROWDOT16 ? add : nullptr, 0,
+                    (_Float16*)c1, (_Float16*)c2};
+    GP_STAMP_ARG(q);
+    const int64_t mb3 = (M + G3_BM - 1) / G3_BM;
+    const int nb3 = (N + G3_BN - 1) / G3_BN;
+    constexpr size_t lds = (size_t)2 * 2 * 2 * GP_PLANE * 2;
+    static std::once_flag once;
+    std::call_once(once, [] {
+        (void)hipFuncSetAttribute((const void*)gemm_h2p_kernel<0, false, true>, hipFuncAttributeMaxDynamicSharedMemorySize, (int)lds);
+        (void)hipFuncSetAttribute((const void*)gemm_h2p_kernel<0, true, false>, hipFuncAttributeMaxDynamicSharedMemorySize, (int)lds);
+        (void)hipFuncSetAttribute((const void*)gemm_h2p_kernel<0, true, true>, hipFuncAttributeMaxDynamicSharedMemorySize, (int)lds);
+        (void)hipFuncSetAttribute((const void*)gemm_h2p_kernel<0, false, false>, hipFuncAttributeMaxDynamicSharedMemorySize, (int)lds);
+    });
+    ProfScope ps(prof_shape_name(af32 ? "gemm_h2p_kernel[a32]" : "gemm_h2p_kernel", M, N, K), st);
+    dim3 grid((unsigned)(8 * nb3 * ((mb3 + 7) / 8)));
+    if (af32 && cp) hipLaunchKernelGGL((gemm_h2p_kernel<0, true, true>), grid, dim3(256), lds, st, q);
+    else if (af32) hipLaunchKernelGGL((gemm_h2p_kernel<0, true, false>), grid, dim3(256), lds, st, q);
+    else if (cp) hipLaunchKernelGGL((gemm_h2p_kernel<0, false, true>), grid, dim3(256), lds, st, q);
+    else hipLaunchKernelGGL((gemm_h2p_kernel<0, false, false>), grid, dim3(256), lds, st, q);
     NIR_CHECK_LAUNCH("gemm_h2p_kernel");
     return 0;
 }
@@ -1140,3 +1283,20 @@
     return nir::launch_linear_planes(a1, a2, lda, ids, rows_per_seq, seq_stride, EP, taps, w1, w2, ldw, bias, c, ldc, M, N, K, act, nullptr, 0,
                                      (hipStream_t)stream);
 }
+
+namespace nir {
+int launch_split_f16x2_rtz(const float* x, int64_t rows, int cols, int64_t ld, int cols_pad, void* p1, void* p2, int* err, hipStream_t st);
+int launch_linear_wplanes(const float* a, const void* a1, const void* a2, int64_t lda, const void* w1, const void* w2, int64_t ldw,
+                          const float* bias, const float* bias2, float* c, void* c1, void* c2, int64_t ldc, int64_t M, int N, int K, int act,
+                          const float* add, hipStream_t st);
+}
+extern "C" int nir_split_f16x2_rtz(const float* x, int64_t rows, int cols, int64_t ld, int cols_pad, void* p1, void* p2, int* err_flag,
+                                   nir_stream_t stream) {
+    return nir::launch_split_f16x2_rtz(x, rows, cols, ld, cols_pad, p1, p2, err_flag, (hipStream_t)stream);
+}
+
+extern "C" int nir_linear_wplanes_f32(const float* a, const void* a1, const void* a2, int64_t lda, const void* w1, const void* w2, int64_t ldw,
+                                      const float* bias, const float* bias2, float* c, void* c1, void* c2, int64_t ldc, int64_t M, int N, int K,
+                                      int act, const float* add, nir_stream_t stream) {
+    return nir::launch_linear_wplanes(a, a1, a2, lda, w1, w2, ldw, bias, bias2, c, c1, c2, ldc, M, N, K, act, add, (hipStream_t)stream);
+}
diff --git a/context_attentive_ir_amd/lib.py b/context_attentive_ir_amd/lib.py
--- a/context_attentive_ir_amd/lib.py
+++ b/context_attentive_ir_amd/lib.py
@@ -1,3 +1,4 @@
+import collections
 import ctypes as C
 import os
 
@@ -66,6 +67,8 @@
     ["wih", "whh", "bih", "bhh", "attn0_w", "attn0_b", "attn3_w", "attn3_b"], ["H", "bounded"])
 CarsEncoderWeights = type("nir_cars_encoder_weights", (C.Structure,), {"_fields_": list(CarsEncoderWeights._fields_) + [("attn_frag", C.c_void_p),
                                                                                                    ("whh_frag", C.c_void_p)]})
+SESSION_PLANE_LAYERS = collections.OrderedDict((("click0_w", ("click0_w", 4)), ("sq_wih", ("sq_wih", 8)), ("sd_wih", ("sd_wih", 8)),
+                                                ("mo0_w", ("mo0_w", 1)), ("mo1_w", ("mo1_w", 2))))
 CarsSessionWeights = _struct(
     "nir_cars_session_weights",
     ["click0_w", "click0_b", "click3_w", "click3_b", "sq_attn_w", "sq_attn_b", "sd_attn_w", "sd_attn_b",
@@ -75,7 +78,8 @@
      "th_w", "th_b", "tc_w", "tc_b"],
     ["D", "HS", "HDEC", "q_on", "d_on", "rank_on", "rank_bounded"])
 CarsSessionWeights = type("nir_cars_session_weights", (C.Structure,), {"_fields_": list(CarsSessionWeights._fields_) + [("sq_whh_frag", C.c_void_p),
-                                                                                                   ("sd_whh_frag", C.c_void_p)]})
+                                                                                                   ("sd_whh_frag", C.c_void_p)] + [
+    (f + t, C.c_size_t) for f in SESSION_PLANE_LAYERS for t in ("1", "2")]})
 class CarsDecoderWeights(C.Structure):
     _fields_ = [(f, c_fp) for f in ("rnn_wih", "rnn_whh", "rnn_bih", "rnn_bhh", "attn_in_w", "attn_out_w", "dec_attn_w", "pred1_w",
                                     "pred2_w", "sess_w")] + [(f, C.c_int) for f in ("HD", "DQ", "P", "KS")] + [("VT", C.c_int64), ("pred2_frag", C.c_void_p), ("rnn_gate_fold", C.c_void_p),
@@ -124,6 +128,9 @@
     "nir_profile_enable": (_i, [_i]),
     "nir_profile_report": (_i, [C.c_char_p, _z]),
     "nir_split_f16x2": (_i, [c_fp, _l, _i, _l, _i, C.c_void_p, C.c_void_p, c_st]),
+    "nir_split_f16x2_rtz": (_i, [c_fp, _l, _i, _l, _i, C.c_void_p, C.c_void_p, C.c_void_p, c_st]),
+    "nir_linear_wplanes_f32": (_i, [c_fp, C.c_void_p, C.c_void_p, _l, C.c_void_p, C.c_void_p, _l, c_fp, c_fp, c_fp, C.c_void_p, C.c_void_p, _l, _l, _i, _i,
+                                    _i, c_fp, c_st]),
     "nir_linear_planes_f32": (_i, [C.c_void_p, C.c_void_p, _l, c_ip, _l, _l, _i, _i, C.c_void_p, C.c_void_p, _l, c_fp, c_fp, _l, _l, _i, _i, _i, c_st]),
     "nir_sanitize_ids": (_i, [c_ip, _l, c_ip, _l, _l, c_ip, c_ip, C.c_void_p, c_st]),
     "nir_flag_publish": (_i, [C.c_void_p, C.c_void_p, c_st]),
@@ -211,6 +218,8 @@
     "nir_cars_encode_folded_workspace_bytes": (_z, [_l, _i, C.POINTER(CarsEncoderWeights)]),
     "nir_cars_encode_folded": (_i, [c_ip, c_ip, _l, _i, C.c_void_p, _i, _l, C.POINTER(CarsEncoderWeights), C.c_void_p, _z,
                                     c_fp, c_fp, C.c_void_p, c_st]),
+    "nir_cars_session_plane_bytes": (_z, [C.POINTER(CarsSessionWeights), C.POINTER(C.c_size_t)]),
+    "nir_cars_session_pack_planes": (_i, [C.POINTER(CarsSessionWeights), C.c_void_p, _z, C.c_void_p, c_st]),
     "nir_cars_session_workspace_bytes": (_z, [_i, _i, _i, C.POINTER(CarsSessionWeights)]),
     "nir_linear_wgrad_f32": (_i, [c_fp, _l, c_fp, _l, c_ip, c_fp, _i, c_fp, _l, _l, _i, _i, c_st]),
     "nir_colsum_f32": (_i, [c_fp, _l, _l, _i, c_fp, c_st]),
diff --git a/context_attentive_ir_amd/multitask/cars.py b/context_attentive_ir_amd/multitask/cars.py
--- a/context_attentive_ir_amd/multitask/cars.py
+++ b/context_attentive_ir_amd/multitask/cars.py
@@ -106,6 +106,7 @@
         self.fuse_decoder_argmax = True
         self.fold_decoder_step = True
         self.fold_decoder_query = True
+        self.session_weight_planes = True
         self.fold_budget_bytes = 64 << 30
         self.compute_dtype = getattr(args, "compute_dtype", "f32")
         self._fq, self._fd = lib.PackCache(retain=1), lib.PackCache(retain=1)
@@ -208,8 +209,22 @@
                 b1 = int(b0 and y0 < 32768.0 and float(pk.keep["mo1_w"].abs().max()) < 32768.0)
                 b2 = int("click0_w" in pk.keep and float(pk.keep["click0_w"].abs().max()) < 32768.0)
                 pk.struct.rank_bounded = b0 | (b1 << 1) | (b2 << 2) | (b3 << 3)
+            if self.session_weight_planes and pk.struct.rank_bounded:
+                offs = (lib.C.c_size_t * 5)()
+                nbytes = L.nir_cars_session_plane_bytes(pk.ref(), offs)
+                dev = next(iter(pk.keep.values())).device
+                if nbytes and dev.type == "cuda":
+                    buf, flag = torch.empty(nbytes, dtype=torch.uint8, device=dev), torch.zeros(1, dtype=torch.int32, device=dev)
+                    lib.check(L.nir_cars_session_pack_planes(pk.ref(), lib.ptr(buf), nbytes, lib.ptr(flag), lib.stream()), "nir_cars_session_pack_planes")
+                    if int(flag.item()) == 0:
+                        pk.keep["weight_planes"] = buf
+                        for i, (stem, (wname, bit)) in enumerate(lib.SESSION_PLANE_LAYERS.items()):
+                            if wname in pk.keep and (pk.struct.rank_bounded & bit):
+                                rows, k = pk.keep[wname].shape
+                                setattr(pk.struct, stem + "1", buf.data_ptr() + offs[i])
+                                setattr(pk.struct, stem + "2", buf.data_ptr() + offs[i] + rows * ((k + 7) // 8 * 8) * 2)
             return pk
-        return self._ps.get([p for m in self._session_modules() for p in m.parameters()], build)
+        return self._ps.get([p for m in self._session_modules() for p in m.parameters()] + [self.session_weight_planes], build)
 
     def _decoder_weights(self):
         def build():
diff --git a/include/neuroir_hip.h b/include/neuroir_hip.h
--- a/include/neuroir_hip.h
+++ b/include/neuroir_hip.h
@@ -34,6 +34,12 @@
 int nir_linear_planes_f32(const void* a1, const void* a2, int64_t lda, const int64_t* ids, int64_t rows_per_seq, int64_t seq_stride, int EP,
                           int taps, const void* w1, const void* w2, int64_t ldw, const float* bias, float* c, int64_t ldc, int64_t M, int N,
                           int K, int act, nir_stream_t stream);
+
+int nir_split_f16x2_rtz(const float* x, int64_t rows, int cols, int64_t ld, int cols_pad, void* p1, void* p2, int* err_flag, nir_stream_t stream);
+
+int nir_linear_wplanes_f32(const float* a, const void* a1, const void* a2, int64_t lda, const void* w1, const void* w2, int64_t ldw,
+                           const float* bias, const float* bias2, float* c, void* c1, void* c2, int64_t ldc, int64_t M, int N, int K,
+                           int act, const float* add, nir_stream_t stream);
 
 int nir_sanitize_ids(const int64_t* a, int64_t na, const int64_t* b, int64_t nb, int64_t V, int64_t* out_a, int64_t* out_b,
                      int* err_flag, nir_stream_t stream);
@@ -286,6 +292,7 @@
     int q_on, d_on, rank_on;
     int rank_bounded;
     const void *sq_whh_frag, *sd_whh_frag;
+    const void *click0_w1, *click0_w2, *sq_wih1, *sq_wih2, *sd_wih1, *sd_wih2, *mo0_w1, *mo0_w2, *mo1_w1, *mo1_w2;
 } nir_cars_session_weights;
 typedef struct {
     float* inner_q;
@@ -297,6 +304,8 @@
 int nir_lstm_step_pack_whh_frag(const float* w_hh, int H, void* frag, int* err_flag, nir_stream_t stream);
 size_t nir_cars_session_pack_floats(const nir_cars_session_weights* w , size_t* wrank_floats , size_t* ut_floats );
 int nir_cars_session_pack(const nir_cars_session_weights* w , float* wrank, float* attn_ut, nir_stream_t stream);
+size_t nir_cars_session_plane_bytes(const nir_cars_session_weights* w , size_t* offsets );
+int nir_cars_session_pack_planes(const nir_cars_session_weights* w , void* buffer, size_t buffer_bytes, int* err_flag, nir_stream_t stream);
 size_t nir_cars_session_workspace_bytes(int B, int S, int N, const nir_cars_session_weights* w );
 int nir_cars_rank_session(const float* pooled_q, const float* pooled_docs, const float* labels, int B, int S, int N,
                           const nir_cars_session_weights* w , void* workspace, size_t workspace_bytes,
```
